# Grandediw/Unmanned_Aerial_Vehicles

Hardware: AMD Instinct MI355X
Metric: GP predictions/sec (mean+var) at N_train=65536, D=9 (higher is better)
Workload: dtype f32; 1 GPU; C3: N_train=65536, D=9, P=3, batched predict mean+var over 10000 query points per GPU per step (horizon 20 x 500 rollouts), fp32 predict on an fp64 factor; n_train=65536, features=9, outputs=3, parallelism=query-sharded x1, model replicated (every rank fits redundantly)

## Files before the change

include/gpk.h:

```cpp
#ifndef GPK_H
#define GPK_H

#include <stddef.h>
#include <stdint.h>

#ifdef __cplusplus
extern "C" {
#endif

typedef struct gpk_context* gpk_handle;

#define GPK_API __attribute__((visibility("default")))

enum { GPK_F32 = 0, GPK_F64 = 1 };
enum { GPK_OK = 0, GPK_NOT_PD = 1, GPK_BAD_ARG = 2, GPK_HIP_ERROR = 3 };
enum { GPK_TILE = 128, GPK_MAX_D = 64, GPK_MAX_D_PREDICT = 16, GPK_MAX_P = 16, GPK_MAX_BATCH = 8 };

GPK_API int gpk_create(gpk_handle* h, int device);
GPK_API void gpk_destroy(gpk_handle h);
GPK_API const char* gpk_last_error(gpk_handle h);
#define GPK_OWN_STREAM ((void*)(intptr_t)-1)
GPK_API int gpk_set_stream(gpk_handle h, void* stream);
GPK_API int gpk_synchronize(gpk_handle h);
GPK_API int64_t gpk_padded(int64_t n);

GPK_API int gpk_set_option(gpk_handle h, const char* name, int value);
GPK_API int gpk_set_option_str(gpk_handle h, const char* name, const char* value);
enum { GPK_TIMED_K5 = 1, GPK_TIMED_GRAM = 2, GPK_TIMED_GRAD = 3, GPK_TIMED_POTRF = 4, GPK_TIMED_COV = 5, GPK_TIMED_JAC = 6,
       GPK_TIMED_SPARSE_STATS = 7, GPK_TIMED_SPARSE_PASS = 8 };
GPK_API int gpk_timing(gpk_handle h, int enable);
GPK_API int gpk_kernel_times(gpk_handle h, int tag, double* ms, int max_n, int* n_out);

GPK_API int gpk_batch_begin(gpk_handle h, int count);
GPK_API int gpk_batch_buffer(gpk_handle h, const void* base, int64_t stride_bytes);
GPK_API int gpk_batch_end(gpk_handle h);
GPK_API const char* gpk_version(void);

GPK_API int gpk_gram(gpk_handle h, int dtype, const void* X, int64_t N, int D, const double* ls,
             double sf2, double diag_add, void* K, int64_t ldk);

GPK_API int gpk_gram_rows(gpk_handle h, int dtype, const void* X, int64_t N, int D, const double* ls, double sf2,
                  double diag_add, int64_t row0, int64_t nrows, void* Kslab, int64_t ldk);

GPK_API int gpk_cross_gram_t(gpk_handle h, int dtype, const void* X, int64_t N, const void* Xq,
                     int64_t M, int D, const double* ls, double sf2, void* B, int64_t ldb);

GPK_API int gpk_potrf(gpk_handle h, double* A, int64_t Np, int64_t lda, double* winv, int* info);

GPK_API int gpk_leaf_inverses(gpk_handle h, const double* L, int64_t Np, int64_t ldl, double* winv);

GPK_API int gpk_factor_to_f32(gpk_handle h, const double* L, int64_t Np, int64_t ldl, const double* winv,
                      float* Lf, int64_t ldlf, float* winvf);

GPK_API int gpk_potrs(gpk_handle h, const double* L, int64_t Np, int64_t ldl, const double* winv,
              const double* Y, int64_t N, int P, double* alpha);

GPK_API int gpk_potrs_inv(gpk_handle h, const double* W, int64_t Np, int64_t ldw, const double* Y, int64_t N,
                  int P, double* alpha);

GPK_API int gpk_trsm_lower_left(gpk_handle h, int dtype, const void* L, int64_t Np, int64_t ldl,
                        const void* winv, void* B, int64_t Mp, int64_t ldb);
GPK_API int gpk_colsumsq(gpk_handle h, int dtype, const void* B, int64_t Np, int64_t Mp, int64_t ldb,
                 double* out);

GPK_API int gpk_predict_mean(gpk_handle h, int dtype, const void* X, const void* alpha, int64_t N, int D,
                     int P, const double* ls, double sf2, const double* y_mean,
                     const double* y_std, const void* Xq, int64_t M, void* mean);

#define GPK_HOST_MAX_M 4096
GPK_API int gpk_predict_host(gpk_handle h, const double* X, const double* alpha, int64_t N, int D, int P,
                     const double* ls, double sf2, const double* y_mean, const double* y_std,
                     const double* W, int64_t Np, int64_t ldw, double kss, double floor_,
                     const double* Xq_host, int64_t M, double* mean_host, double* var_host);

GPK_API int gpk_predict_host_multi(gpk_handle h, int B, const double* const* X, const double* const* alpha, int64_t N, int D,
                           const double* ls, const double* sf2, const double* y_mean, const double* y_std,
                           const double* const* W, int64_t Np, int64_t ldw, const double* kss, double floor_,
                           const double* Xq_host, int64_t M, double* mean_host, double* var_host);

GPK_API int gpk_predict_mean_mfma(gpk_handle h, const float* X, const float* alpha, int64_t N, int D, int P,
                          const double* ls, double sf2, const double* center, const double* y_mean,
                          const double* y_std, const float* Xq, int64_t M, float* mean);

GPK_API int gpk_split3(gpk_handle h, const float* src, int64_t rows, int64_t cols, int64_t ld, void* dst);
GPK_API int gpk_predict_var_inv_split(gpk_handle h, const float* X, int64_t N, int D, const double* ls, double sf2,
                              const void* W3, int64_t Np, const float* Xq, int64_t M, double kss, double floor_,
                              float* work, void* work3, double* var);

GPK_API int gpk_split2_rows(gpk_handle h, const float* W, int64_t n, int64_t ld, float* scales, void* dst);
GPK_API int gpk_split2_rows_f64(gpk_handle h, const double* W, int64_t n, int64_t ld, float* scales, void* dst);
GPK_API int gpk_split2_rows_f64_absmax(gpk_handle h, const double* W, int64_t n, int64_t ld, float* scales, void* dst);
GPK_API int gpk_predict_var_inv_split2(gpk_handle h, const float* X, int64_t N, int D, const double* ls, double sf2,
                                       const void* W2, const float* w_scales, int64_t Np, const float* Xq, int64_t M,
                                       double kss, double floor_, void* work2, double* var);

GPK_API int gpk_predict_mean_var_split2(gpk_handle h, const float* X, const float* alpha, int64_t N, int D, int P,
                                        const double* ls, double sf2, const double* center, const double* y_mean,
                                        const double* y_std, const void* W2, const float* w_scales, int64_t Np,
                                        const float* Xq, int64_t M, double kss, double floor_, void* work2,
                                        float* mean_tmp, double recheck_below, unsigned* low_count, double* out);
GPK_API int gpk_pack_mean_var(gpk_handle h, int dtype, const void* mean, const double* var, int64_t M, int P,
                              const double* y_std, double* out);

GPK_API int gpk_predict_mean_multi(gpk_handle h, int dtype, const void* X, const void* alpha, int64_t N, int D,
                           int B, const double* ls, const double* sf2, const double* y_mean,
                           const double* y_std, const void* Xq, int64_t M, void* mean);

GPK_API int gpk_predict_var(gpk_handle h, int dtype, const void* X, int64_t N, int D, const double* ls,
                    double sf2, const void* L, int64_t Np, int64_t ldl, const void* winv,
                    const void* Xq, int64_t M, double kss, double floor, void* work,
                    double* var);

GPK_API int gpk_trtri(gpk_handle h, const double* L, int64_t Np, int64_t ldl, const double* winv, double* W,
              int64_t ldw, double* work);
GPK_API int gpk_trtri_absmax(gpk_handle h, const double* L, int64_t Np, int64_t ldl, const double* winv, double* W,
              int64_t ldw, double* work, float* block_absmax);
GPK_API int gpk_tril_to_f32(gpk_handle h, const double* A, int64_t Np, int64_t lda, float* Af, int64_t ldaf);
GPK_API int gpk_predict_var_inv(gpk_handle h, int dtype, const void* X, int64_t N, int D, const double* ls,
                        double sf2, const void* W, int64_t Np, int64_t ldw, const void* Xq, int64_t M,
                        double kss, double floor, void* work, double* var);

GPK_API int gpk_predict_cov_inv(gpk_handle h, int dtype, const void* X, int64_t N, int D, const double* ls, double sf2,
                                const void* W, int64_t Np, int64_t ldw, const void* Xq, int64_t M, double noise, void* work,
                                double* cov, int64_t ldc);
GPK_API int gpk_predict_cov(gpk_handle h, int dtype, const void* X, int64_t N, int D, const double* ls, double sf2,
                            const void* L, int64_t Np, int64_t ldl, const void* winv, const void* Xq, int64_t M, double noise,
                            void* work, double* cov, int64_t ldc);
GPK_API int gpk_predict_host_cov(gpk_handle h, const double* X, const double* alpha, int64_t N, int D, int P,
                                 const double* ls, double sf2, const double* y_mean, const double* y_std, const double* W,
                                 int64_t Np, int64_t ldw, double noise, const double* Xq_host, int64_t M, double* mean_host,
                                 double* cov_host);
GPK_API int gpk_predict_host_multi_cov(gpk_handle h, int B, const double* const* X, const double* const* alpha, int64_t N,
                                       int D, const double* ls, const double* sf2, const double* y_mean, const double* y_std,
                                       const double* const* W, int64_t Np, int64_t ldw, const double* noise,
                                       const double* Xq_host, int64_t M, double* mean_host, double* cov_host);
GPK_API int gpk_predict_batched_cov(gpk_handle h, const double* Xq, int64_t M, double* mean, double* cov);

GPK_API int gpk_predict_mean_grad(gpk_handle h, const double* X, const double* alpha, int64_t N, int D, int P, const double* ls,
                                  double sf2, const double* y_std, const double* Xq, int64_t M, double* dmean);
GPK_API int gpk_predict_var_grad_inv(gpk_handle h, const double* X, int64_t N, int D, const double* ls, double sf2,
                                     const double* W, int64_t Np, int64_t ldw, const double* Xq, int64_t M, double kss,
                                     double floor, double* work, double* var, double* dvar);
GPK_API int gpk_predict_host_grad(gpk_handle h, const double* X, const double* alpha, int64_t N, int D, int P, const double* ls,
                                  double sf2, const double* y_mean, const double* y_std, const double* W, int64_t Np,
                                  int64_t ldw, double kss, double floor, const double* Xq_host, int64_t M, double* mean_host,
                                  double* var_host, double* dmean_host, double* dvar_host);
GPK_API int gpk_predict_model_grad(gpk_handle h, const double* Xq, int64_t M, double* mean, double* var, double* dmean,
                                   double* dvar, int var_includes_noise);
GPK_API int gpk_predict_host_multi_grad(gpk_handle h, int B, const double* const* X, const double* const* alpha, int64_t N,
                                        int D, const double* ls, const double* sf2, const double* y_mean, const double* y_std,
                                        const double* const* W, int64_t Np, int64_t ldw, const double* kss, double floor,
                                        const double* Xq_host, int64_t M, double* mean_host, double* var_host,
                                        double* dmean_host, double* dvar_host);
GPK_API int gpk_predict_mean_grad_multi(gpk_handle h, const double* X, const double* alpha, int64_t N, int D, int B,
                                        const double* ls, const double* sf2, const double* y_std, const double* Xq, int64_t M,
                                        double* dmean);
GPK_API int gpk_predict_batched_grad(gpk_handle h, const double* Xq, int64_t M, double* mean, double* var, double* dmean,
                                     double* dvar, int var_includes_noise);

GPK_API int gpk_lml_terms(gpk_handle h, const double* L, int64_t N, int64_t ldl, const double* Y,
                  const double* alpha, int P, double* terms);

GPK_API int gpk_potri(gpk_handle h, const double* L, int64_t Np, int64_t ldl, const double* winv,
              double* Kinv, int64_t ldk, double* work);
GPK_API int gpk_wtw(gpk_handle h, const double* W, int64_t Np, int64_t ldw, double* Kinv, int64_t ldk);
GPK_API int gpk_lml_grad(gpk_handle h, const double* X, int64_t N, int D, const double* ls, double sf2,
                 double noise, const double* alpha, int P, const double* Kinv, int64_t ldk,
                 double* grad);

GPK_API int gpk_rbf_kernel_grad(gpk_handle h, const double* X1, int64_t n1, const double* X2, int64_t n2, int D,
                        const double* ls, double sf2, double* K, double* Q, int64_t ld);

GPK_API int gpk_lml_eval(gpk_handle h, const double* X, int64_t N, int D, const double* ls, double sf2, double diag_add,
                 double noise, const double* Yn, int P, double* K, int64_t Np, double* winv, double* W, double* work,
                 double* alpha, double* Kinv, double* terms, double* grad, int* info);

GPK_API int gpk_fit(gpk_handle h, const double* X, int64_t N, int D, const double* Y, int P, const double* ls, int n_ls,
            double sf2, double noise, double jitter, int normalize_y);
GPK_API int gpk_predict(gpk_handle h, const void* Xq, int64_t M, void* mean, void* var, int dtype, int var_includes_noise);
GPK_API int gpk_lml(gpk_handle h, const double* theta, int n_theta, double* lml, double* grad);
GPK_API int gpk_export(gpk_handle h, int64_t* N, int* D, int* P, double* L, double* alpha, double* y_mean, double* y_std,
               double* lml);
GPK_API int gpk_import(gpk_handle h, const double* X, int64_t N, int D, const double* L, const double* alpha, int P,
               const double* ls, int n_ls, double sf2, double noise, const double* y_mean, const double* y_std);
GPK_API int gpk_model_release(gpk_handle h);
GPK_API int gpk_predict_model_cov(gpk_handle h, const double* Xq, int64_t M, double* mean, double* cov);

GPK_API int gpk_fit_batched(gpk_handle h, int B, const double* X, int64_t N, int D, const double* Y, const double* ls, int n_ls,
                    const double* sf2, const double* noise, double jitter, int normalize_y, int* info);
GPK_API int gpk_predict_batched(gpk_handle h, const double* Xq, int64_t M, double* mean, double* var, int var_includes_noise);
GPK_API int gpk_lml_batched(gpk_handle h, const double* thetas, int n_theta, double* lml, double* grad);

GPK_API size_t gpk_greedy_select_bytes(int64_t n, int64_t m_max);
GPK_API int gpk_greedy_select(gpk_handle h, const double* X, int64_t n, int D, const double* ls, int n_ls, double sf2,
                              int64_t m_max, double min_var, double tol, void* work, int64_t* idx, double* trace, double* dmax,
                              int64_t* selected);
GPK_API int gpk_sparse_select(gpk_handle h, const double* X, int64_t n, int64_t m_max, double min_var, double tol, int64_t* idx,
                              double* trace, double* dmax, int64_t* selected);
GPK_API int gpk_sparse_accumulate(gpk_handle h, const double* X, const double* Yn, int64_t n, const double* Z, int64_t m, int D,
                                  int P, const double* ls, double sf2, double* S, int64_t ld);
GPK_API int gpk_sparse_grad_pass(gpk_handle h, const double* X, const double* Yn, int64_t n, const double* Z, int64_t m, int D,
                                 int P, const double* ls, double sf2, const double* Cm, int64_t ldc, double* sums);
GPK_API int gpk_sparse_zgrad_pass(gpk_handle h, const double* X, const double* Yn, int64_t n, const double* Z, int64_t m, int D,
                                  int P, const double* ls, double sf2, const double* Cm, int64_t ldc, double* R);
GPK_API int gpk_sparse_begin(gpk_handle h, const double* Z, int64_t m, int D, int P, const double* ls, int n_ls, double sf2,
                             double noise, double jitter, double jitter_uu, const double* y_mean, const double* y_std);
GPK_API int gpk_sparse_hold(gpk_handle h, const double* X, const double* Y, int64_t n);
GPK_API int gpk_sparse_eval(gpk_handle h, const double* ls, int n_ls, double sf2, double noise, double* bound, double* grad,
                            int* info);
GPK_API int gpk_sparse_eval_z(gpk_handle h, const double* Z, const double* ls, int n_ls, double sf2, double noise, double* bound,
                              double* grad, double* gradZ, int* info);
GPK_API int gpk_sparse_update(gpk_handle h, const double* X, const double* Y, int64_t n);
GPK_API int gpk_sparse_finalize(gpk_handle h, int* info);
GPK_API int gpk_sparse_predict(gpk_handle h, const double* Xq, int64_t M, double* mean, double* var, int var_includes_noise);
GPK_API int gpk_sparse_predict_grad(gpk_handle h, const double* Xq, int64_t M, double* mean, double* var, double* dmean,
                                    double* dvar, int var_includes_noise);
GPK_API int gpk_sparse_predict_cov(gpk_handle h, const double* Xq, int64_t M, double* mean, double* cov);

GPK_API int gpk_sparse_predict_multi(gpk_handle h, int B, const gpk_handle* models, const double* Xq, int64_t M, double* mean,
                                     double* var, int var_includes_noise);
GPK_API int gpk_sparse_predict_multi_grad(gpk_handle h, int B, const gpk_handle* models, const double* Xq, int64_t M, double* mean,
                                          double* var, double* dmean, double* dvar, int var_includes_noise);
GPK_API int gpk_sparse_predict_multi_cov(gpk_handle h, int B, const gpk_handle* models, const double* Xq, int64_t M, double* mean,
                                         double* cov);
GPK_API int gpk_sparse_bound(gpk_handle h, double* bound, int64_t* n_rows);
GPK_API int gpk_sparse_export(gpk_handle h, int64_t* m, int* D, int* P, int* n_ls, double* Z, double* G, double* g, double* yy,
                              int64_t* n_rows, double* ls, double* hyper, double* y_mean, double* y_std);
GPK_API int gpk_sparse_import(gpk_handle h, const double* Z, int64_t m, int D, int P, const double* ls, int n_ls, double sf2,
                              double noise, double jitter, double jitter_uu, const double* y_mean, const double* y_std,
                              const double* G, const double* g, const double* yy, int64_t n_rows);

GPK_API int gpk_gemm_tiles(gpk_handle h, int dtype, int ta, int tb, const void* A, int64_t lda, const void* B,
                   int64_t ldb, void* C, int64_t ldc, int64_t m, int64_t n, int64_t k, double alpha,
                   double beta, int lower_only);

#ifdef __cplusplus
}
#endif
#endif
```

unmanned_aerial_vehicles_amd/_lib.py:

```python
import ctypes as C
import os

import numpy as np

from ._build import LIB_PATH

GPK_F32, GPK_F64 = 0, 1
GPK_OK, GPK_NOT_PD, GPK_BAD_ARG, GPK_HIP_ERROR = 0, 1, 2, 3
GPK_TILE, GPK_MAX_D, GPK_MAX_P = 128, 64, 16
GPK_HOST_MAX_M = 4096
GPK_TIMED_K5, GPK_TIMED_GRAM, GPK_TIMED_GRAD, GPK_TIMED_POTRF = 1, 2, 3, 4
GPK_TIMED_COV = 5
GPK_TIMED_JAC = 6
GPK_TIMED_SPARSE_STATS, GPK_TIMED_SPARSE_PASS = 7, 8

_vp, _i64, _int, _dbl = C.c_void_p, C.c_int64, C.c_int, C.c_double
_dp = C.POINTER(C.c_double)

SIGNATURES = {
    "gpk_create": (_int, [C.POINTER(_vp), _int]),
    "gpk_destroy": (None, [_vp]),
    "gpk_last_error": (C.c_char_p, [_vp]),
    "gpk_set_stream": (_int, [_vp, _vp]),
    "gpk_synchronize": (_int, [_vp]),
    "gpk_padded": (_i64, [_i64]),
    "gpk_fit": (_int, [_vp, _dp, _i64, _int, _dp, _int, _dp, _int, _dbl, _dbl, _dbl, _int]),
    "gpk_predict": (_int, [_vp, _vp, _i64, _vp, _vp, _int, _int]),
    "gpk_lml": (_int, [_vp, _dp, _int, _dp, _dp]),
    "gpk_fit_batched": (_int, [_vp, _int, _dp, _i64, _int, _dp, _dp, _int, _dp, _dp, _dbl, _int, C.POINTER(C.c_int)]),
    "gpk_predict_batched": (_int, [_vp, _dp, _i64, _dp, _dp, _int]),
    "gpk_lml_batched": (_int, [_vp, _dp, _int, _dp, _dp]),
    "gpk_export": (_int, [_vp, C.POINTER(_i64), C.POINTER(_int), C.POINTER(_int), _dp, _dp, _dp, _dp, _dp]),
    "gpk_import": (_int, [_vp, _dp, _i64, _int, _dp, _dp, _int, _dp, _int, _dbl, _dbl, _dp, _dp]),
    "gpk_model_release": (_int, [_vp]),
    "gpk_split2_rows": (_int, [_vp, _vp, _i64, _i64, _vp, _vp]),
    "gpk_split2_rows_f64": (_int, [_vp, _vp, _i64, _i64, _vp, _vp]),
    "gpk_split2_rows_f64_absmax": (_int, [_vp, _vp, _i64, _i64, _vp, _vp]),
    "gpk_predict_var_inv_split2": (_int, [_vp, _vp, _i64, _int, _dp, _dbl, _vp, _vp, _i64, _vp, _i64, _dbl, _dbl, _vp, _vp]),
    "gpk_predict_mean_var_split2": (_int, [_vp, _vp, _vp, _i64, _int, _int, _dp, _dbl, _dp, _dp, _dp, _vp, _vp, _i64, _vp, _i64,
                                           _dbl, _dbl, _vp, _vp, _dbl, _vp, _vp]),
    "gpk_pack_mean_var": (_int, [_vp, _int, _vp, _vp, _i64, _int, _dp, _vp]),
    "gpk_set_option": (_int, [_vp, C.c_char_p, _int]),
    "gpk_set_option_str": (_int, [_vp, C.c_char_p, C.c_char_p]),
    "gpk_timing": (_int, [_vp, _int]),
    "gpk_kernel_times": (_int, [_vp, _int, _dp, _int, C.POINTER(_int)]),
    "gpk_batch_begin": (_int, [_vp, _int]),
    "gpk_batch_buffer": (_int, [_vp, _vp, _i64]),
    "gpk_batch_end": (_int, [_vp]),
    "gpk_version": (C.c_char_p, []),
    "gpk_gram": (_int, [_vp, _int, _vp, _i64, _int, _dp, _dbl, _dbl, _vp, _i64]),
    "gpk_gram_rows": (_int, [_vp, _int, _vp, _i64, _int, _dp, _dbl, _dbl, _i64, _i64, _vp, _i64]),
    "gpk_cross_gram_t": (_int, [_vp, _int, _vp, _i64, _vp, _i64, _int, _dp, _dbl, _vp, _i64]),
    "gpk_rbf_kernel_grad": (_int, [_vp, _vp, _i64, _vp, _i64, _int, _dp, _dbl, _vp, _vp, _i64]),
    "gpk_potrf": (_int, [_vp, _vp, _i64, _i64, _vp, C.POINTER(_int)]),
    "gpk_leaf_inverses": (_int, [_vp, _vp, _i64, _i64, _vp]),
    "gpk_factor_to_f32": (_int, [_vp, _vp, _i64, _i64, _vp, _vp, _i64, _vp]),
    "gpk_potrs": (_int, [_vp, _vp, _i64, _i64, _vp, _vp, _i64, _int, _vp]),
    "gpk_potrs_inv": (_int, [_vp, _vp, _i64, _i64, _vp, _i64, _int, _vp]),
    "gpk_wtw": (_int, [_vp, _vp, _i64, _i64, _vp, _i64]),
    "gpk_trsm_lower_left": (_int, [_vp, _int, _vp, _i64, _i64, _vp, _vp, _i64, _i64]),
    "gpk_colsumsq": (_int, [_vp, _int, _vp, _i64, _i64, _i64, _vp]),
    "gpk_predict_mean": (_int, [_vp, _int, _vp, _vp, _i64, _int, _int, _dp, _dbl, _dp, _dp, _vp, _i64, _vp]),
    "gpk_split3": (_int, [_vp, _vp, _i64, _i64, _i64, _vp]),
    "gpk_predict_var_inv_split": (_int, [_vp, _vp, _i64, _int, _dp, _dbl, _vp, _i64, _vp, _i64, _dbl, _dbl, _vp, _vp, _vp]),
    "gpk_predict_host": (_int, [_vp, _vp, _vp, _i64, _int, _int, _vp, _dbl, _vp, _vp, _vp, _i64, _i64, _dbl, _dbl, _vp,
                                _i64, _vp, _vp]),
    "gpk_predict_host_multi": (_int, [_vp, _int, _vp, _vp, _i64, _int, _vp, _vp, _vp, _vp, _vp, _i64, _i64, _vp, _dbl, _vp,
                                      _i64, _vp, _vp]),
    "gpk_predict_mean_mfma": (_int, [_vp, _vp, _vp, _i64, _int, _int, _dp, _dbl, _dp, _dp, _dp, _vp, _i64, _vp]),
    "gpk_predict_mean_multi": (_int, [_vp, _int, _vp, _vp, _i64, _int, _int, _dp, _dp, _dp, _dp, _vp, _i64, _vp]),
    "gpk_predict_var": (_int, [_vp, _int, _vp, _i64, _int, _dp, _dbl, _vp, _i64, _i64, _vp, _vp, _i64, _dbl,
                               _dbl, _vp, _vp]),
    "gpk_trtri": (_int, [_vp, _vp, _i64, _i64, _vp, _vp, _i64, _vp]),
    "gpk_trtri_absmax": (_int, [_vp, _vp, _i64, _i64, _vp, _vp, _i64, _vp, _vp]),
    "gpk_tril_to_f32": (_int, [_vp, _vp, _i64, _i64, _vp, _i64]),
    "gpk_predict_var_inv": (_int, [_vp, _int, _vp, _i64, _int, _dp, _dbl, _vp, _i64, _i64, _vp, _i64, _dbl, _dbl,
                                   _vp, _vp]),
    "gpk_predict_cov_inv": (_int, [_vp, _int, _vp, _i64, _int, _dp, _dbl, _vp, _i64, _i64, _vp, _i64, _dbl, _vp, _vp,
                                   _i64]),
    "gpk_predict_cov": (_int, [_vp, _int, _vp, _i64, _int, _dp, _dbl, _vp, _i64, _i64, _vp, _vp, _i64, _dbl, _vp, _vp,
                               _i64]),
    "gpk_predict_host_cov": (_int, [_vp, _vp, _vp, _i64, _int, _int, _vp, _dbl, _vp, _vp, _vp, _i64, _i64, _dbl, _vp, _i64,
                                    _vp, _vp]),
    "gpk_predict_model_cov": (_int, [_vp, _dp, _i64, _dp, _dp]),
    "gpk_predict_host_multi_cov": (_int, [_vp, _int, _vp, _vp, _i64, _int, _vp, _vp, _vp, _vp, _vp, _i64, _i64, _vp, _vp, _i64,
                                          _vp, _vp]),
    "gpk_predict_batched_cov": (_int, [_vp, _dp, _i64, _dp, _dp]),
    "gpk_predict_mean_grad": (_int, [_vp, _vp, _vp, _i64, _int, _int, _dp, _dbl, _dp, _vp, _i64, _vp]),
    "gpk_predict_var_grad_inv": (_int, [_vp, _vp, _i64, _int, _dp, _dbl, _vp, _i64, _i64, _vp, _i64, _dbl, _dbl, _vp, _vp, _vp]),
    "gpk_predict_host_grad": (_int, [_vp, _vp, _vp, _i64, _int, _int, _vp, _dbl, _vp, _vp, _vp, _i64, _i64, _dbl, _dbl, _vp,
                                     _i64, _vp, _vp, _vp, _vp]),
    "gpk_predict_model_grad": (_int, [_vp, _dp, _i64, _dp, _dp, _dp, _dp, _int]),
    "gpk_predict_host_multi_grad": (_int, [_vp, _int, _vp, _vp, _i64, _int, _vp, _vp, _vp, _vp, _vp, _i64, _i64, _vp, _dbl, _vp,
                                           _i64, _vp, _vp, _vp, _vp]),
    "gpk_predict_mean_grad_multi": (_int, [_vp, _vp, _vp, _i64, _int, _int, _dp, _dp, _dp, _vp, _i64, _vp]),
    "gpk_predict_batched_grad": (_int, [_vp, _dp, _i64, _dp, _dp, _dp, _dp, _int]),
    "gpk_lml_terms": (_int, [_vp, _vp, _i64, _i64, _vp, _vp, _int, _dp]),
    "gpk_potri": (_int, [_vp, _vp, _i64, _i64, _vp, _vp, _i64, _vp]),
    "gpk_lml_grad": (_int, [_vp, _vp, _i64, _int, _dp, _dbl, _dbl, _vp, _int, _vp, _i64, _dp]),
    "gpk_lml_eval": (_int, [_vp, _vp, _i64, _int, _dp, _dbl, _dbl, _dbl, _vp, _int, _vp, _i64, _vp, _vp, _vp, _vp, _vp, _dp, _dp,
                            C.POINTER(C.c_int)]),
    "gpk_sparse_accumulate": (_int, [_vp, _vp, _vp, _i64, _vp, _i64, _int, _int, _dp, _dbl, _vp, _i64]),
    "gpk_sparse_grad_pass": (_int, [_vp, _vp, _vp, _i64, _vp, _i64, _int, _int, _dp, _dbl, _vp, _i64, _vp]),
    "gpk_sparse_zgrad_pass": (_int, [_vp, _vp, _vp, _i64, _vp, _i64, _int, _int, _dp, _dbl, _vp, _i64, _vp]),
    "gpk_sparse_hold": (_int, [_vp, _dp, _dp, _i64]),
    "gpk_sparse_eval": (_int, [_vp, _dp, _int, _dbl, _dbl, _dp, _dp, C.POINTER(_int)]),
    "gpk_sparse_eval_z": (_int, [_vp, _dp, _dp, _int, _dbl, _dbl, _dp, _dp, _dp, C.POINTER(_int)]),
    "gpk_greedy_select_bytes": (C.c_size_t, [_i64, _i64]),
    "gpk_greedy_select": (_int, [_vp, _vp, _i64, _int, _dp, _int, _dbl, _i64, _dbl, _dbl, _vp, _vp, _vp, _vp, _vp]),
    "gpk_sparse_select": (_int, [_vp, _dp, _i64, _i64, _dbl, _dbl, C.POINTER(_i64), _dp, _dp, C.POINTER(_i64)]),
    "gpk_sparse_begin": (_int, [_vp, _dp, _i64, _int, _int, _dp, _int, _dbl, _dbl, _dbl, _dbl, _dp, _dp]),
    "gpk_sparse_update": (_int, [_vp, _dp, _dp, _i64]),
    "gpk_sparse_finalize": (_int, [_vp, C.POINTER(_int)]),
    "gpk_sparse_predict": (_int, [_vp, _dp, _i64, _dp, _dp, _int]),
    "gpk_sparse_predict_grad": (_int, [_vp, _dp, _i64, _dp, _dp, _dp, _dp, _int]),
    "gpk_sparse_predict_cov": (_int, [_vp, _dp, _i64, _dp, _dp]),
    "gpk_sparse_predict_multi": (_int, [_vp, _int, C.POINTER(_vp), _dp, _i64, _dp, _dp, _int]),
    "gpk_sparse_predict_multi_grad": (_int, [_vp, _int, C.POINTER(_vp), _dp, _i64, _dp, _dp, _dp, _dp, _int]),
    "gpk_sparse_predict_multi_cov": (_int, [_vp, _int, C.POINTER(_vp), _dp, _i64, _dp, _dp]),
    "gpk_sparse_bound": (_int, [_vp, _dp, C.POINTER(_i64)]),
    "gpk_sparse_export": (_int, [_vp, C.POINTER(_i64), C.POINTER(_int), C.POINTER(_int), C.POINTER(_int), _dp, _dp, _dp, _dp,
                                 C.POINTER(_i64), _dp, _dp, _dp, _dp]),
    "gpk_sparse_import": (_int, [_vp, _dp, _i64, _int, _int, _dp, _int, _dbl, _dbl, _dbl, _dbl, _dp, _dp, _dp, _dp, _dp, _i64]),
    "gpk_gemm_tiles": (_int, [_vp, _int, _int, _int, _vp, _i64, _vp, _i64, _vp, _i64, _i64, _i64, _i64, _dbl,
                              _dbl, _int]),
}

_lib = None


class GPKError(RuntimeError):
    def __init__(self, code, message):
        super().__init__(f"libgpk error {code}: {message}")
        self.code = code


class NotPositiveDefinite(np.linalg.LinAlgError):
    """Raised where the reference's LAPACK call raises `numpy.linalg.LinAlgError`
    (scipy.linalg.cholesky at sklearn/gaussian_process/_gpr.py:349)."""


def load():
    global _lib
    if _lib is not None:
        return _lib
    try:
        import torch
    except ImportError:
        pass
    path = os.environ.get("GPK_LIBRARY") or LIB_PATH
    if not os.path.exists(path):
        raise RuntimeError(
            f"{path} not found: build it with `python -c 'import __graft_entry__ as g; g.build()'` "
            "(there is no CPU fallback for the GP kernels)")
    lib = C.CDLL(path)
    for name, (res, args) in SIGNATURES.items():
        fn = getattr(lib, name)
        fn.restype = res
        fn.argtypes = args
    _lib = lib
    return lib


def dptr(a):
    a = np.ascontiguousarray(a, dtype=np.float64)
    return a, a.ctypes.data_as(_dp)
```

unmanned_aerial_vehicles_amd/csrc/gpk_api.hip:

```cpp
#include <cstdlib>

#include "gpk_internal.h"

extern "C" const char* gpk_version(void) { return "gpk 0.1 (gfx950)"; }

extern "C" int64_t gpk_padded(int64_t n) { return (n + GPK_TILE - 1) / GPK_TILE * GPK_TILE; }

extern "C" int gpk_create(gpk_handle* out, int device) {
  if (!out) return GPK_BAD_ARG;
  *out = nullptr;
  int count = 0;
  if (hipGetDeviceCount(&count) != hipSuccess || count <= 0 || device < 0 || device >= count) return GPK_HIP_ERROR;
  if (hipSetDevice(device) != hipSuccess) return GPK_HIP_ERROR;
  gpk_context* h = new gpk_context();
  h->device = device;
  if (hipStreamCreateWithFlags(&h->own_stream, hipStreamNonBlocking) != hipSuccess ||
      hipMalloc((void**)&h->d_info, GPK_MAX_BATCH * sizeof(int)) != hipSuccess ||

      hipMalloc((void**)&h->d_count, 2 * GPK_SMALL_MAX_MODELS * sizeof(unsigned)) != hipSuccess ||
      hipMemset(h->d_count, 0, 2 * GPK_SMALL_MAX_MODELS * sizeof(unsigned)) != hipSuccess ||
      hipHostMalloc((void**)&h->h_small, 4096, hipHostMallocMapped | hipHostMallocCoherent) != hipSuccess ||
      hipHostGetDevicePointer((void**)&h->d_small, h->h_small, 0) != hipSuccess) {
    delete h;
    return GPK_HIP_ERROR;
  }
  h->stream = h->own_stream;
  *out = h;
  return GPK_OK;
}

extern "C" void gpk_destroy(gpk_handle h) {
  if (!h) return;
  (void)hipSetDevice(h->device);
  (void)hipStreamSynchronize(h->stream);
  gpk_model_free(h);
  if (h->scratch) (void)hipFree(h->scratch);
  if (h->d_info) (void)hipFree(h->d_info);
  if (h->d_count) (void)hipFree(h->d_count);
  if (h->d_cov_count) (void)hipFree(h->d_cov_count);
  if (h->d_ptile) (void)hipFree(h->d_ptile);
  if (h->h_small) (void)hipHostFree(h->h_small);
  if (h->serve_dev) (void)hipFree(h->serve_dev);
  if (h->serve_host) (void)hipHostFree(h->serve_host);
  for (auto& t : h->timed) {
    if (t.e0) (void)hipEventDestroy(t.e0);
    if (t.e1) (void)hipEventDestroy(t.e1);
  }
  if (h->own_stream) (void)hipStreamDestroy(h->own_stream);
  delete h;
}

extern "C" const char* gpk_last_error(gpk_handle h) { return h ? h->err.c_str() : "null handle"; }

extern "C" int gpk_set_stream(gpk_handle h, void* stream) {
  if (!h) return GPK_BAD_ARG;
  hipStream_t want = (stream == GPK_OWN_STREAM) ? h->own_stream : (hipStream_t)stream;
  GPK_CHECK_HIP(h, hipSetDevice(h->device));
  if (want == h->stream) return GPK_OK;
  GPK_CHECK_HIP(h, hipStreamSynchronize(h->stream));
  h->stream = want;
  h->user_stream = (stream != GPK_OWN_STREAM);
  return GPK_OK;
}

extern "C" int gpk_set_option(gpk_handle h, const char* name, int value) {
  if (!h) return GPK_BAD_ARG;
  GPK_REQUIRE(h, name, "set_option: null name");
  const std::string n(name);
  if (n == "k5_split2_tile") h->k5_split2_tile = (value >= 0 && value <= 2) ? value : 0;
  else if (n == "small_path") h->small_path = value;
  else if (n == "trsm256") h->trsm256 = value;
  else if (n == "trtri_levels") h->trtri_levels = value;
  else if (n == "gemm_small_tiles") h->gemm_small_tiles = value;
  else if (n == "gemm_tiny_tiles") h->gemm_tiny_tiles = value;
  else if (n == "gemm_balanced") h->gemm_balanced = value;
  else if (n == "gemm_balanced_max_tiles") h->gemm_balanced_max_tiles = value;
  else if (n == "k3_stream_min_np") h->k3_stream_min_np = value;
  else if (n == "gemm_log") h->gemm_log = value;
  else if (n == "gram_log") h->gram_log = value;
  else if (n == "debug_fill") h->debug_fill = value ? 1 : 0;
  else if (n == "sparse_panel") h->sparse_panel = value <= 0 ? 0 : value > (1 << 20) ? (1 << 20) : value;
  else if (n == "sparse_slabs") h->sparse_slabs = value <= 0 ? 0 : value > 64 ? 64 : value;
  else if (n == "ptile") h->ptile = value;
  else if (n == "ptile_max_np") h->ptile_max_np = value;
  else if (n == "ptile_prog_max_nt") h->ptile_prog_max_nt = value;
  else if (n == "ptile_inv_max_np") h->ptile_inv_max_np = value;
  else if (n == "ptile_single_max_nt") h->ptile_single_max_nt = value;
  else if (n == "ptile_sr") h->ptile_sr = value;
  else if (n == "ptile_sr_max_nt") h->ptile_sr_max_nt = value;
  else if (n == "ptile_prog_rows") h->ptile_prog_rows = value >= 8 ? 8 : value >= 1 ? value : 1;
  else { h->err = "bad argument: unknown option " + n; return GPK_BAD_ARG; }
  return GPK_OK;
}

extern "C" int gpk_set_option_str(gpk_handle h, const char* name, const char* value) {
  if (!h) return GPK_BAD_ARG;
  GPK_REQUIRE(h, name, "set_option_str: null name");
  const std::string n(name);
  if (n == "ptile_trace_path") h->ptile_trace_request = value ? value : "";
  else { h->err = "bad argument: unknown option " + n; return GPK_BAD_ARG; }
  return GPK_OK;
}

extern "C" int gpk_timing(gpk_handle h, int enable) {
  if (!h) return GPK_BAD_ARG;
  if (enable && h->timed.empty()) {
    GPK_CHECK_HIP(h, hipSetDevice(h->device));
    h->timed.resize(GPK_TIMING_RING);
    for (auto& t : h->timed) {
      GPK_CHECK_HIP(h, hipEventCreate(&t.e0));
      GPK_CHECK_HIP(h, hipEventCreate(&t.e1));
    }
  }
  h->timing = enable ? 1 : 0;
  h->timed_count = 0;
  return GPK_OK;
}

extern "C" int gpk_kernel_times(gpk_handle h, int tag, double* ms, int max_n, int* n_out) {
  if (!h) return GPK_BAD_ARG;
  GPK_REQUIRE(h, ms && n_out && max_n >= 1, "kernel_times: null pointer");
  *n_out = 0;
  if (h->timed.empty()) return GPK_OK;
  GPK_CHECK_HIP(h, hipStreamSynchronize(h->stream));
  const long long have = h->timed_count < GPK_TIMING_RING ? h->timed_count : GPK_TIMING_RING;
  for (long long i = h->timed_count - have; i < h->timed_count && *n_out < max_n; ++i) {
    const auto& t = h->timed[(size_t)(i % GPK_TIMING_RING)];
    if (t.tag != tag) continue;
    float f = 0.f;
    GPK_CHECK_HIP(h, hipEventElapsedTime(&f, t.e0, t.e1));
    ms[(*n_out)++] = (double)f;
  }
  return GPK_OK;
}

extern "C" int gpk_batch_begin(gpk_handle h, int count) {
  if (!h) return GPK_BAD_ARG;
  GPK_REQUIRE(h, count >= 1 && count <= GPK_MAX_BATCH, "batch_begin: count must be in [1, 8]");
  GPK_REQUIRE(h, h->batch == 1 && h->bbufs.empty(), "batch_begin: a batch is already open");
  h->batch = count;
  return GPK_OK;
}

extern "C" int gpk_batch_buffer(gpk_handle h, const void* base, int64_t stride_bytes) {
  if (!h) return GPK_BAD_ARG;
  GPK_REQUIRE(h, base && stride_bytes > 0 && stride_bytes % 16 == 0, "batch_buffer: stride must be a positive multiple of 16");
  h->bbufs.push_back({(const char*)base, (long long)stride_bytes});
  return GPK_OK;
}

extern "C" int gpk_batch_end(gpk_handle h) {
  if (!h) return GPK_BAD_ARG;
  h->batch = 1;
  h->bbufs.clear();
  return GPK_OK;
}

extern "C" int gpk_synchronize(gpk_handle h) {
  if (!h) return GPK_BAD_ARG;
  GPK_CHECK_HIP(h, hipStreamSynchronize(h->stream));
  return GPK_OK;
}

int gpk_scratch(gpk_handle h, size_t bytes, void** out) {
  if (bytes > h->scratch_bytes) {
    GPK_CHECK_HIP(h, hipSetDevice(h->device));
    GPK_CHECK_HIP(h, hipStreamSynchronize(h->stream));
    if (h->scratch) GPK_CHECK_HIP(h, hipFree(h->scratch));
    h->scratch = nullptr;
    h->scratch_bytes = 0;
    const size_t want = (bytes + (1u << 20) - 1) & ~(size_t)((1u << 20) - 1);
    GPK_CHECK_HIP(h, hipMalloc(&h->scratch, want));
    h->scratch_bytes = want;
  }
  if (h->debug_fill && bytes > 0) GPK_CHECK_HIP(h, hipMemsetAsync(h->scratch, 0xFF, bytes, h->stream));
  *out = h->scratch;
  return GPK_OK;
}

extern "C" int gpk_predict_var(gpk_handle h, int dtype, const void* X, int64_t N, int D, const double* ls,
                               double sf2, const void* L, int64_t Np, int64_t ldl, const void* winv, const void* Xq,
                               int64_t M, double kss, double floor_, void* work, double* var) {
  if (!h) return GPK_BAD_ARG;
  GPK_REQUIRE(h, X && L && winv && Xq && work && var, "predict_var: null pointer");
  GPK_REQUIRE(h, N >= 1 && M >= 1 && Np == gpk_padded(N), "predict_var: Np must equal gpk_padded(N)");
  const int64_t Mp = gpk_padded(M);
  GPK_TRY(gpk_cross_gram_t(h, dtype, X, N, Xq, M, D, ls, sf2, work, Mp));
  GPK_TRY(gpk_trsm_lower_left(h, dtype, L, Np, ldl, winv, work, Mp, Mp));
  GPK_TRY(gpk_colsumsq(h, dtype, work, Np, Mp, Mp, var));
  return gpk_var_finalize(h, var, M, kss, floor_, var);
}

extern "C" int gpk_predict_var_inv(gpk_handle h, int dtype, const void* X, int64_t N, int D, const double* ls,
                                   double sf2, const void* W, int64_t Np, int64_t ldw, const void* Xq, int64_t M,
                                   double kss, double floor_, void* work, double* var) {
  if (!h) return GPK_BAD_ARG;
  GPK_REQUIRE(h, X && W && Xq && work && var, "predict_var_inv: null pointer");
  GPK_REQUIRE(h, N >= 1 && M >= 1 && Np == gpk_padded(N) && ldw >= Np, "predict_var_inv: Np must equal gpk_padded(N)");
  GPK_REQUIRE(h, dtype == GPK_F32 || dtype == GPK_F64, "predict_var_inv: bad dtype");
  const int64_t Mp = gpk_padded(M);
  GPK_TRY(gpk_cross_gram_t(h, dtype, Xq, M, X, N, D, ls, sf2, work, Np));
  GemmArgs g = gemm_args(W, ldw, 0, work, Np, 0, nullptr, Mp, (int)Np, (int)Mp, (int)Np, 1.0, 0.0);
  g.ke0 = GPK_TILE;
  g.ke_row = GPK_TILE;
  g.epilogue = 1;
  g.k_super = 1;
  g.heavy_first = 1;
  const int ntm = (int)(Np / gpk_gemm_tile(h, g));
  void* partial = nullptr;
  GPK_TRY(gpk_scratch(h, (size_t)ntm * Mp * sizeof(double), &partial));
  g.C = partial;
  gpk_time_begin(h, GPK_TIMED_K5);
  const int rc_gemm = gpk_gemm(h, dtype, g);
  gpk_time_end(h);
  GPK_TRY(rc_gemm);
  return gpk_colsum_finalize(h, (const double*)partial, ntm, Mp, M, kss, floor_, var);
}

extern "C" int gpk_gemm_tiles(gpk_handle h, int dtype, int ta, int tb, const void* A, int64_t lda, const void* B,
                              int64_t ldb, void* C, int64_t ldc, int64_t m, int64_t n, int64_t k, double alpha,
                              double beta, int lower_only) {
  if (!h) return GPK_BAD_ARG;
  GPK_REQUIRE(h, A && B && C, "gemm_tiles: null pointer");
  GPK_REQUIRE(h, dtype == GPK_F32 || dtype == GPK_F64, "gemm_tiles: bad dtype");
  GPK_REQUIRE(h, m < (1ll << 31) && n < (1ll << 31) && k < (1ll << 31), "gemm_tiles: size too large");
  GemmArgs g = gemm_args(A, lda, ta ? 1 : 0, B, ldb, tb ? 1 : 0, C, ldc, (int)m, (int)n, (int)k, alpha, beta);
  g.lower_only = lower_only ? 1 : 0;
  return gpk_gemm(h, dtype, g);
}
```

unmanned_aerial_vehicles_amd/csrc/gpk_gram.hip:

```cpp
#include <cstdlib>

#include "gpk_internal.h"
#include "gpk_math.h"

namespace {

struct LsArr { double v[GPK_MAX_D]; };
struct PArr { double v[GPK_MAX_P]; };
struct Ls16 { double v[16]; };

__device__ __forceinline__ double exp_neg(double x) { return gpk_exp_neg(x); }
__device__ __forceinline__ float exp_neg(float x) {
  const float L2E_HI = 1.44269502162933349609375f, L2E_LO = 1.925963033500011e-08f;
  const float hi = x * L2E_HI;
  const float lo = __builtin_fmaf(x, L2E_HI, -hi) + x * L2E_LO;
  const float e = __builtin_amdgcn_exp2f(hi);
  return __builtin_fmaf(e, lo * 0.693147180559945f, e);
}

__device__ __forceinline__ double fma_t(double a, double b, double c) { return __builtin_fma(a, b, c); }
__device__ __forceinline__ float fma_t(float a, float b, float c) { return __builtin_fmaf(a, b, c); }

template <typename T> struct Vec16;
template <> struct Vec16<double> { typedef double2 type; static constexpr int N = 2; };
template <> struct Vec16<float> { typedef float4 type; static constexpr int N = 4; };

__device__ __forceinline__ void st16(double* p, double a, double b, bool nt) {
  typedef double dv2 __attribute__((ext_vector_type(2)));
  dv2 v = {a, b};
  if (nt) __builtin_nontemporal_store(v, reinterpret_cast<dv2*>(p));
  else *reinterpret_cast<dv2*>(p) = v;
}
__device__ __forceinline__ void st16(float* p, float a, float b, float c, float d, bool nt) {
  typedef float fv4 __attribute__((ext_vector_type(4)));
  fv4 v = {a, b, c, d};
  if (nt) __builtin_nontemporal_store(v, reinterpret_cast<fv4*>(p));
  else *reinterpret_cast<fv4*>(p) = v;
}
__device__ __forceinline__ void store_row4(double* p, int tx, const double (&v)[4], bool nt) {
  st16(p + 2 * tx, v[0], v[1], nt);
  st16(p + 32 + 2 * tx, v[2], v[3], nt);
}
__device__ __forceinline__ void store_row4(float* p, int tx, const float (&v)[4], bool nt) {
  st16(p + 4 * tx, v[0], v[1], v[2], v[3], nt);
}

constexpr int TS = 64;

template <typename T> __device__ __forceinline__ int colof(int tx, int c);
template <> __device__ __forceinline__ int colof<double>(int tx, int c) { return (c >> 1) * 32 + 2 * tx + (c & 1); }
template <> __device__ __forceinline__ int colof<float>(int tx, int c) { return 4 * tx + c; }
constexpr int DCH = 16;

template <typename T>
__device__ __forceinline__ void stage_x(const T* __restrict__ X, long long n, int D, long long r0, int d0,
                                        int dc, const LsArr& ls, T* lds, int tid) {
  for (int e = tid; e < TS * dc; e += 256) {
    const int i = e / dc, d = e - i * dc;
    const long long gi = r0 + i;
    T v = T(0);
    if (gi < n) v = X[gi * D + d0 + d] / T(ls.v[d0 + d]);
    lds[d * TS + i] = v;
  }
}

template <typename T>
__device__ __forceinline__ void accum_d2(const T* xi, const T* xj, int dc, int ty, int tx, T (&d2)[4][4]) {
  for (int d = 0; d < dc; ++d) {
    T a[4], b[4];
#pragma unroll
    for (int r = 0; r < 4; ++r) a[r] = xi[d * TS + 4 * ty + r];
#pragma unroll
    for (int c = 0; c < 4; ++c) b[c] = xj[d * TS + colof<T>(tx, c)];
#pragma unroll
    for (int r = 0; r < 4; ++r)
#pragma unroll
      for (int c = 0; c < 4; ++c) {
        const T df = a[r] - b[c];
        d2[r][c] = fma_t(df, df, d2[r][c]);
      }
  }
}

template <typename T, bool NT>
__global__ __launch_bounds__(256) void gram_sym_kernel(const T* __restrict__ X, long long N, int D, LsArr ls,
                                                       T sf2, T diag_add, T* __restrict__ K, long long ldk) {
  __shared__ __attribute__((aligned(16))) T xi[DCH * TS];
  __shared__ __attribute__((aligned(16))) T xj[DCH * TS];
  __shared__ __attribute__((aligned(16))) T tb[TS * (TS + 1)];
  const int tid = threadIdx.x, tx = tid & 15, ty = tid >> 4;

  const long long id = blockIdx.x;
  long long ti = (long long)((__builtin_sqrt(8.0 * (double)id + 1.0) - 1.0) * 0.5);
  while ((ti + 1) * (ti + 2) / 2 <= id) ++ti;
  while (ti * (ti + 1) / 2 > id) --ti;
  const long long tj = id - ti * (ti + 1) / 2;
  const long long i0 = ti * TS, j0 = tj * TS;

  T d2[4][4];
#pragma unroll
  for (int r = 0; r < 4; ++r)
#pragma unroll
    for (int c = 0; c < 4; ++c) d2[r][c] = T(0);

  for (int dbase = 0; dbase < D; dbase += DCH) {
    const int dc = min(DCH, D - dbase);
    if (dbase) __syncthreads();
    stage_x<T>(X, N, D, i0, dbase, dc, ls, xi, tid);
    stage_x<T>(X, N, D, j0, dbase, dc, ls, xj, tid);
    __syncthreads();
    accum_d2<T>(xi, xj, dc, ty, tx, d2);
  }

  T v[4][4];
#pragma unroll
  for (int r = 0; r < 4; ++r) {
    const long long gi = i0 + 4 * ty + r;
#pragma unroll
    for (int c = 0; c < 4; ++c) {
      const long long gj = j0 + colof<T>(tx, c);
      T val = sf2 * exp_neg(T(-0.5) * d2[r][c]);
      if (gi == gj) val = sf2 + diag_add;
      if (gi >= N || gj >= N) val = (gi == gj) ? T(1) : T(0);
      v[r][c] = val;
    }
    store_row4(K + gi * ldk + j0, tx, v[r], NT);
  }
  if (ti == tj) return;

#pragma unroll
  for (int r = 0; r < 4; ++r)
#pragma unroll
    for (int c = 0; c < 4; ++c) tb[(4 * ty + r) * (TS + 1) + colof<T>(tx, c)] = v[r][c];
  __syncthreads();
  constexpr int VEC = Vec16<T>::N;
  constexpr int LPR = TS / VEC;
  constexpr int RPG = TS / (256 / LPR);
  const int lp = tid % LPR, g = tid / LPR;
#pragma unroll
  for (int rr = 0; rr < RPG; ++rr) {
    const int jj = g * RPG + rr;
    T w[VEC];
#pragma unroll
    for (int e = 0; e < VEC; ++e) w[e] = tb[(VEC * lp + e) * (TS + 1) + jj];
    T* dst = K + (j0 + jj) * ldk + i0 + VEC * lp;
    if constexpr (VEC == 2) st16(dst, w[0], w[1], NT);
    else st16(dst, w[0], w[1], w[2], w[3], NT);
  }
}

template <typename T, bool NT, int GS>
__global__ __launch_bounds__(256) void gram_strip_kernel(const T* __restrict__ X, long long N, int D, LsArr ls,
                                                         T sf2, T diag_add, T* __restrict__ K, long long ldk) {
  __shared__ __attribute__((aligned(16))) T xi[DCH * TS];
  __shared__ __attribute__((aligned(16))) T xj[DCH * TS];
  __shared__ __attribute__((aligned(16))) T tb[TS * (TS + 1)];
  const int tid = threadIdx.x, tx = tid & 15, ty = tid >> 4;
  const long long id = blockIdx.x;
  long long q = (long long)((__builtin_sqrt(1.0 + 8.0 * (double)id / GS) - 1.0) * 0.5);
  while (GS * (q + 1) * (q + 2) / 2 <= id) ++q;
  while (GS * q * (q + 1) / 2 > id) --q;
  const long long rem_id = id - GS * q * (q + 1) / 2;
  const long long ti = GS * q + rem_id / (q + 1);
  const long long g = rem_id % (q + 1);
  const long long i0 = ti * TS;
  const long long tj0 = g * GS, tj1 = min(ti, tj0 + GS - 1);

  stage_x<T>(X, N, D, i0, 0, D, ls, xi, tid);
  stage_x<T>(X, N, D, tj0 * TS, 0, D, ls, xj, tid);
  constexpr int NPF = (TS * DCH + 255) / 256;
  T pf[NPF];
  __syncthreads();
  for (long long tj = tj0; tj <= tj1; ++tj) {
    const long long j0 = tj * TS;
    const bool more = tj < tj1;
    if (more) {
#pragma unroll
      for (int p = 0; p < NPF; ++p) {
        const int e = tid + 256 * p;
        const int i = e / D, d = e - i * D;
        const long long gi = j0 + TS + i;
        pf[p] = (e < TS * D && gi < N) ? X[gi * D + d] / T(ls.v[d]) : T(0);
      }
    }
    T d2[4][4];
#pragma unroll
    for (int r = 0; r < 4; ++r)
#pragma unroll
      for (int c = 0; c < 4; ++c) d2[r][c] = T(0);
    accum_d2<T>(xi, xj, D, ty, tx, d2);
    T v[4][4];
#pragma unroll
    for (int r = 0; r < 4; ++r) {
      const long long gi = i0 + 4 * ty + r;
#pragma unroll
      for (int c = 0; c < 4; ++c) {
        const long long gj = j0 + colof<T>(tx, c);
        T val = sf2 * exp_neg(T(-0.5) * d2[r][c]);
        if (gi == gj) val = sf2 + diag_add;
        if (gi >= N || gj >= N) val = (gi == gj) ? T(1) : T(0);
        v[r][c] = val;
      }
      store_row4(K + gi * ldk + j0, tx, v[r], NT);
    }
    if (ti != tj) {
#pragma unroll
      for (int r = 0; r < 4; ++r)
#pragma unroll
        for (int c = 0; c < 4; ++c) tb[(4 * ty + r) * (TS + 1) + colof<T>(tx, c)] = v[r][c];
    }
    __syncthreads();
    if (ti != tj) {
      constexpr int VEC = Vec16<T>::N;
      constexpr int LPR = TS / VEC;
      constexpr int RPG = TS / (256 / LPR);
      const int lp = tid % LPR, gg = tid / LPR;
#pragma unroll
      for (int rr = 0; rr < RPG; ++rr) {
        const int jj = gg * RPG + rr;
        T w[VEC];
#pragma unroll
        for (int e = 0; e < VEC; ++e) w[e] = tb[(VEC * lp + e) * (TS + 1) + jj];
        T* dst = K + (j0 + jj) * ldk + i0 + VEC * lp;
        if constexpr (VEC == 2) st16(dst, w[0], w[1], NT);
        else st16(dst, w[0], w[1], w[2], w[3], NT);
      }
    }
    if (more) {
#pragma unroll
      for (int p = 0; p < NPF; ++p) {
        const int e = tid + 256 * p;
        if (e < TS * D) { const int i = e / D, d = e - i * D; xj[d * TS + i] = pf[p]; }
      }
    }
    __syncthreads();
  }
}

template <typename T>
__global__ __launch_bounds__(256) void cross_t_kernel(const T* __restrict__ X, long long N,
                                                      const T* __restrict__ Xq, long long M, int D, LsArr ls,
                                                      T sf2, T* __restrict__ B, long long ldb) {
  __shared__ __attribute__((aligned(16))) T xi[DCH * TS];
  __shared__ __attribute__((aligned(16))) T xj[DCH * TS];
  const int tid = threadIdx.x, tx = tid & 15, ty = tid >> 4;
  const long long i0 = (long long)blockIdx.y * TS, j0 = (long long)blockIdx.x * TS;
  T d2[4][4];
#pragma unroll
  for (int r = 0; r < 4; ++r)
#pragma unroll
    for (int c = 0; c < 4; ++c) d2[r][c] = T(0);
  for (int dbase = 0; dbase < D; dbase += DCH) {
    const int dc = min(DCH, D - dbase);
    if (dbase) __syncthreads();
    stage_x<T>(X, N, D, i0, dbase, dc, ls, xi, tid);
    stage_x<T>(Xq, M, D, j0, dbase, dc, ls, xj, tid);
    __syncthreads();
    accum_d2<T>(xi, xj, dc, ty, tx, d2);
  }
#pragma unroll
  for (int r = 0; r < 4; ++r) {
    const long long gi = i0 + 4 * ty + r;
    T v[4];
#pragma unroll
    for (int c = 0; c < 4; ++c) {
      const long long gj = j0 + colof<T>(tx, c);
      T val = sf2 * exp_neg(T(-0.5) * d2[r][c]);
      if (gi >= N || gj >= M) val = T(0);
      v[c] = val;
    }
    store_row4(B + gi * ldb + j0, tx, v, false);
  }
}

typedef _Float16 h8_t __attribute__((ext_vector_type(8)));
typedef unsigned int u4_t __attribute__((ext_vector_type(4)));
constexpr int CS2_QS = 4;
template <int DD>
__global__ __launch_bounds__(256) void cross_split2_kernel(const float* __restrict__ Xq, long long M,
                                                           const float* __restrict__ X, long long N, int D, LsArr ls,
                                                           float sf2, float scale, u4_t* __restrict__ dst, long long Np) {
  __shared__ __attribute__((aligned(16))) float xs[DD][128];
  const int tid = threadIdx.x, lane = tid & 63, wave = tid >> 6;
  const long long j0 = (long long)blockIdx.x * 128;
  for (int e = tid; e < 128 * DD; e += 256) {
    const int d = e >> 7, i = e & 127;
    const long long gj = j0 + i;
    xs[d][i] = (d < D && gj < N) ? X[gj * D + d] / (float)ls.v[d] : 0.f;
  }
  __syncthreads();
  const int r = lane & 31, hh = lane >> 5;
  const long long KB = Np >> 4, Mp = (M + 127) / 128 * 128;
#pragma unroll 1
  for (int qs = 0; qs < CS2_QS; ++qs) {
  const long long q0 = ((long long)blockIdx.y * CS2_QS + qs) * 64;
  if (q0 >= Mp) break;
  const long long qblk = (q0 >> 5) + (wave >> 1), q = qblk * 32 + r;
  float xq[DD];
#pragma unroll
  for (int d = 0; d < DD; ++d) xq[d] = (q < M ? Xq[q * DD + d] : 0.f) / (float)ls.v[d];
#pragma unroll
  for (int t = 0; t < 4; ++t) {
    const int kb = 4 * (wave & 1) + t, kbase = 16 * kb + 8 * hh;
    float d2[8];
#pragma unroll
    for (int i = 0; i < 8; ++i) d2[i] = 0.f;
#pragma unroll
    for (int d = 0; d < DD; ++d) {
      const float4 lo = *reinterpret_cast<const float4*>(&xs[d][kbase]), hi = *reinterpret_cast<const float4*>(&xs[d][kbase + 4]);
      const float b[8] = {lo.x, lo.y, lo.z, lo.w, hi.x, hi.y, hi.z, hi.w};
#pragma unroll
      for (int i = 0; i < 8; ++i) { const float df = xq[d] - b[i]; d2[i] = __builtin_fmaf(df, df, d2[i]); }
    }
    h8_t p0, p1;
#pragma unroll
    for (int i = 0; i < 8; ++i) {
      float val = sf2 * exp_neg(-0.5f * d2[i]);
      if (q >= M || j0 + kbase + i >= N) val = 0.f;
      const float x = val * scale;
      const _Float16 h0 = (_Float16)x;
      p0[i] = h0;
      p1[i] = (_Float16)(x - (float)h0);
    }
    u4_t* o = dst + ((qblk * KB + (j0 >> 4) + kb) * 2) * 64 + lane;
    o[0] = __builtin_bit_cast(u4_t, p0);
    o[64] = __builtin_bit_cast(u4_t, p1);
  }
  }
}

constexpr int PM_DMAX = 16, PM_PMAX = 16, PM_TJ = 128, PM_QPT = 2, PM_RS = PM_DMAX + PM_PMAX;

template <typename T> struct Quad;
template <> struct Quad<float> { typedef float4 type; };
template <> struct Quad<double> { typedef double4 type; };

template <typename T, int D4, int P4>
__global__ __launch_bounds__(256) void predict_mean_kernel(const T* __restrict__ X, const T* __restrict__ alpha,
                                                           long long N, int D, int P, Ls16 ls,
                                                           const T* __restrict__ Xq, long long M,
                                                           long long chunk, T* __restrict__ partial) {
  __shared__ __attribute__((aligned(16))) T rows[PM_TJ * PM_RS];
  typedef typename Quad<T>::type Q4;
  const int tid = threadIdx.x;
  constexpr int DD = 4 * D4, PP = 4 * P4;
  T xq[PM_QPT][DD];
  T acc[PM_QPT][PP];
  long long qm[PM_QPT];
#pragma unroll
  for (int q = 0; q < PM_QPT; ++q) {
    qm[q] = ((long long)blockIdx.x * PM_QPT + q) * 256 + tid;
#pragma unroll
    for (int d = 0; d < DD; ++d) {
      xq[q][d] = T(0);
      if (d < D && qm[q] < M) xq[q][d] = Xq[qm[q] * D + d] / T(ls.v[d]);
    }
#pragma unroll
    for (int p = 0; p < PP; ++p) acc[q][p] = T(0);
  }
  constexpr bool TWO_LEVEL = sizeof(T) == 4;
  T tot[PM_QPT][PP];
#pragma unroll
  for (int q = 0; q < PM_QPT; ++q)
#pragma unroll
    for (int p = 0; p < PP; ++p) tot[q][p] = T(0);
  const long long n0 = (long long)blockIdx.y * chunk;
  const long long n1 = min(N, n0 + chunk);
  for (long long jb = n0; jb < n1; jb += PM_TJ) {
    const int nj = (int)min((long long)PM_TJ, n1 - jb);
    if constexpr (TWO_LEVEL) {
#pragma unroll
      for (int q = 0; q < PM_QPT; ++q)
#pragma unroll
        for (int p = 0; p < PP; ++p) { tot[q][p] += acc[q][p]; acc[q][p] = T(0); }
    }
    __syncthreads();
    for (int e = tid; e < nj * (DD + PP); e += 256) {
      const int j = e / (DD + PP), c = e - j * (DD + PP);
      T v = T(0);
      if (c < DD) { if (c < D) v = X[(jb + j) * D + c] / T(ls.v[c]); }
      else if (c - DD < P) v = alpha[(jb + j) * P + (c - DD)];
      rows[j * PM_RS + (c < DD ? c : PM_DMAX + (c - DD))] = v;
    }
    __syncthreads();
#pragma unroll 2
    for (int j = 0; j < nj; ++j) {
      const Q4* row = reinterpret_cast<const Q4*>(rows + j * PM_RS);
      T xt[DD], al[PP];
#pragma unroll
      for (int g = 0; g < D4; ++g) {
        const Q4 v = row[g];
        xt[4 * g] = v.x; xt[4 * g + 1] = v.y; xt[4 * g + 2] = v.z; xt[4 * g + 3] = v.w;
      }
#pragma unroll
      for (int g = 0; g < P4; ++g) {
        const Q4 v = row[PM_DMAX / 4 + g];
        al[4 * g] = v.x; al[4 * g + 1] = v.y; al[4 * g + 2] = v.z; al[4 * g + 3] = v.w;
      }
#pragma unroll
      for (int q = 0; q < PM_QPT; ++q) {
        T d2 = T(0);
#pragma unroll
        for (int d = 0; d < DD; ++d) {
          const T df = xq[q][d] - xt[d];
          d2 = fma_t(df, df, d2);
        }
        const T e = exp_neg(T(-0.5) * d2);
#pragma unroll
        for (int p = 0; p < PP; ++p) acc[q][p] = fma_t(e, al[p], acc[q][p]);
      }
    }
  }
#pragma unroll
  for (int q = 0; q < PM_QPT; ++q) {
    if (qm[q] < M) {
#pragma unroll
      for (int p = 0; p < PP; ++p)
        if (p < P) partial[((long long)blockIdx.y * M + qm[q]) * P + p] = TWO_LEVEL ? tot[q][p] + acc[q][p] : acc[q][p];
    }
  }
}

template <typename T>
using pm_fn = void (*)(const T*, const T*, long long, int, int, Ls16, const T*, long long, long long, T*);
template <typename T, int D4>
pm_fn<T> pm_pick_p(int p4) {
  switch (p4) {
    case 1: return predict_mean_kernel<T, D4, 1>;
    case 2: return predict_mean_kernel<T, D4, 2>;
    case 3: return predict_mean_kernel<T, D4, 3>;
    default: return predict_mean_kernel<T, D4, 4>;
  }
}
template <typename T>
pm_fn<T> pm_pick(int d4, int p4) {
  switch (d4) {
    case 1: return pm_pick_p<T, 1>(p4);
    case 2: return pm_pick_p<T, 2>(p4);
    case 3: return pm_pick_p<T, 3>(p4);
    default: return pm_pick_p<T, 4>(p4);
  }
}

template <typename T, int D4, int B4>
__global__ __launch_bounds__(256) void predict_mean_multi_kernel(const T* __restrict__ X,
                                                                 const T* __restrict__ alpha, long long N, int D,
                                                                 int B, const double* __restrict__ w_dev,
                                                                 const T* __restrict__ Xq, long long M,
                                                                 long long chunk, T* __restrict__ partial) {
  __shared__ __attribute__((aligned(16))) T rows[PM_TJ * PM_RS];
  __shared__ __attribute__((aligned(16))) T wl[4 * B4 * 4 * D4];
  typedef typename Quad<T>::type Q4;
  const int tid = threadIdx.x;
  constexpr int DD = 4 * D4, BB = 4 * B4;
  for (int e = tid; e < BB * DD; e += 256) {
    const int b = e / DD, d = e - b * DD;
    wl[e] = (b < B && d < D) ? T(w_dev[b * D + d]) : T(0);
  }
  T xq[PM_QPT][DD];
  T acc[PM_QPT][BB];
  long long qm[PM_QPT];
#pragma unroll
  for (int q = 0; q < PM_QPT; ++q) {
    qm[q] = ((long long)blockIdx.x * PM_QPT + q) * 256 + tid;
#pragma unroll
    for (int d = 0; d < DD; ++d) {
      xq[q][d] = T(0);
      if (d < D && qm[q] < M) xq[q][d] = Xq[qm[q] * D + d];
    }
#pragma unroll
    for (int b = 0; b < BB; ++b) acc[q][b] = T(0);
  }
  const long long n0 = (long long)blockIdx.y * chunk;
  const long long n1 = min(N, n0 + chunk);
  for (long long jb = n0; jb < n1; jb += PM_TJ) {
    const int nj = (int)min((long long)PM_TJ, n1 - jb);
    __syncthreads();
    for (int e = tid; e < PM_TJ * (DD + BB); e += 256) {
      const int j = e / (DD + BB), c = e - j * (DD + BB);
      T v = T(0);
      if (j < nj) {
        if (c < DD) { if (c < D) v = X[(jb + j) * D + c]; }
        else if (c - DD < B) v = alpha[(jb + j) * B + (c - DD)];
      }
      rows[j * PM_RS + (c < DD ? c : PM_DMAX + (c - DD))] = v;
    }
    __syncthreads();
#pragma unroll 2
    for (int j = 0; j < PM_TJ; ++j) {
      const Q4* row = reinterpret_cast<const Q4*>(rows + j * PM_RS);
      T xt[DD], al[BB];
#pragma unroll
      for (int g = 0; g < D4; ++g) {
        const Q4 v = row[g];
        xt[4 * g] = v.x; xt[4 * g + 1] = v.y; xt[4 * g + 2] = v.z; xt[4 * g + 3] = v.w;
      }
#pragma unroll
      for (int g = 0; g < B4; ++g) {
        const Q4 v = row[PM_DMAX / 4 + g];
        al[4 * g] = v.x; al[4 * g + 1] = v.y; al[4 * g + 2] = v.z; al[4 * g + 3] = v.w;
      }
#pragma unroll
      for (int q = 0; q < PM_QPT; ++q) {
        T sq[DD];
#pragma unroll
        for (int d = 0; d < DD; ++d) { const T df = xq[q][d] - xt[d]; sq[d] = df * df; }
#pragma unroll
        for (int b = 0; b < BB; ++b) {
          T d2 = T(0);
#pragma unroll
          for (int d = 0; d < DD; ++d) d2 = fma_t(sq[d], wl[b * DD + d], d2);
          acc[q][b] = fma_t(exp_neg(T(-0.5) * d2), al[b], acc[q][b]);
        }
      }
    }
  }
#pragma unroll
  for (int q = 0; q < PM_QPT; ++q) {
    if (qm[q] < M) {
#pragma unroll
      for (int b = 0; b < BB; ++b)
        if (b < B) partial[((long long)blockIdx.y * M + qm[q]) * B + b] = acc[q][b];
    }
  }
}

template <typename T>
__global__ void mean_reduce_multi_kernel(const T* __restrict__ partial, int S, long long M, int B, PArr sf2,
                                         PArr ymean, PArr ystd, T* __restrict__ mean) {
  const long long e = (long long)blockIdx.x * blockDim.x + threadIdx.x;
  if (e >= M * B) return;
  const int b = (int)(e % B);
  T s = T(0);
  for (int k = 0; k < S; ++k) s += partial[(long long)k * M * B + e];
  mean[e] = T(ymean.v[b]) + T(ystd.v[b]) * (T(sf2.v[b]) * s);
}

template <typename T>
using pmm_fn = void (*)(const T*, const T*, long long, int, int, const double*, const T*, long long, long long, T*);
template <typename T, int D4>
pmm_fn<T> pmm_pick_b(int b4) {
  return b4 <= 1 ? predict_mean_multi_kernel<T, D4, 1> : predict_mean_multi_kernel<T, D4, 2>;
}
template <typename T>
pmm_fn<T> pmm_pick(int d4, int b4) {
  switch (d4) {
    case 1: return pmm_pick_b<T, 1>(b4);
    case 2: return pmm_pick_b<T, 2>(b4);
    case 3: return pmm_pick_b<T, 3>(b4);
    default: return pmm_pick_b<T, 4>(b4);
  }
}

template <typename T>
__global__ void mean_reduce_kernel(const T* __restrict__ partial, int S, long long M, int P, T sf2, PArr ymean,
                                   PArr ystd, T* __restrict__ mean) {
  const long long e = (long long)blockIdx.x * blockDim.x + threadIdx.x;
  if (e >= M * P) return;
  const int p = (int)(e % P);
  double s = 0.0;
  for (int k = 0; k < S; ++k) s += (double)partial[(long long)k * M * P + e];
  mean[e] = T(ymean.v[p]) + T(ystd.v[p]) * (sf2 * T(s));
}

template <typename T>
__global__ __launch_bounds__(256) void colsumsq_kernel(const T* __restrict__ B, long long rows_per, long long Np,
                                                       long long ldb, double* __restrict__ partial, long long Mp) {
  const int c = threadIdx.x & 127, hh = threadIdx.x >> 7;
  const long long m = (long long)blockIdx.x * 128 + c;
  const long long r0 = (long long)blockIdx.y * rows_per, r1 = min(Np, r0 + rows_per);
  double s0 = 0.0, s1 = 0.0;
  long long r = r0 + hh;
  for (; r + 2 < r1; r += 4) {
    const double a = (double)B[r * ldb + m], b = (double)B[(r + 2) * ldb + m];
    s0 = __builtin_fma(a, a, s0);
    s1 = __builtin_fma(b, b, s1);
  }
  if (r < r1) { const double a = (double)B[r * ldb + m]; s0 = __builtin_fma(a, a, s0); }
  partial[((long long)blockIdx.y * 2 + hh) * Mp + m] = s0 + s1;
}
__global__ void colsum_reduce_kernel(const double* __restrict__ partial, int S, long long Mp,
                                     double* __restrict__ out) {
  const long long m = (long long)blockIdx.x * blockDim.x + threadIdx.x;
  if (m >= Mp) return;
  double s = 0.0;
  for (int k = 0; k < S; ++k) s += partial[(long long)k * Mp + m];
  out[m] = s;
}
__global__ void colsum_finalize_kernel(const double* __restrict__ partial, int S, long long Mp, long long M, double kss,
                                       double floor_, double* __restrict__ var) {
  const long long m = (long long)blockIdx.x * blockDim.x + threadIdx.x;
  if (m >= M) return;
  double s = 0.0;
  for (int k = 0; k < S; ++k) s += partial[(long long)k * Mp + m];
  var[m] = fmax(kss - s, floor_);
}
__global__ void colsum_finalize_packed_kernel(const double* __restrict__ partial, int S, long long Mp, long long M, double kss,
                                              double floor_, const float* __restrict__ mean, int P, PArr ystd,
                                              double recheck_below, unsigned* __restrict__ low_count,
                                              double* __restrict__ out) {
  const long long m = (long long)blockIdx.x * blockDim.x + threadIdx.x;
  if (m >= M) return;
  double s = 0.0;
  for (int k = 0; k < S; ++k) s += partial[(long long)k * Mp + m];
  const double v = fmax(kss - s, floor_);
  if (low_count && v < recheck_below) atomicAdd(low_count, 1u);
  double* o = out + m * 2 * P;
  for (int p = 0; p < P; ++p) { o[p] = (double)mean[m * P + p]; o[P + p] = v * ystd.v[p] * ystd.v[p]; }
}
template <typename T>
__global__ void pack_mean_var_kernel(const T* __restrict__ mean, const double* __restrict__ var, long long M, int P, PArr ystd,
                                     double* __restrict__ out) {
  const long long m = (long long)blockIdx.x * blockDim.x + threadIdx.x;
  if (m >= M) return;
  double* o = out + m * 2 * P;
  const double v = var[m];
  for (int p = 0; p < P; ++p) { o[p] = (double)mean[m * P + p]; o[P + p] = v * ystd.v[p] * ystd.v[p]; }
}
__global__ void var_finalize_kernel(const double* ss, long long M, double kss, double floor_, double* var) {
  const long long m = (long long)blockIdx.x * blockDim.x + threadIdx.x;
  if (m >= M) return;
  var[m] = fmax(kss - ss[m], floor_);
}

int fill_ls(gpk_handle h, const double* ls, int D, LsArr& out) {
  GPK_REQUIRE(h, D >= 1 && D <= GPK_MAX_D, "D must be in [1, 64]");
  GPK_REQUIRE(h, ls != nullptr, "length-scale array is null");
  for (int d = 0; d < GPK_MAX_D; ++d) out.v[d] = 1.0;
  for (int d = 0; d < D; ++d) {
    GPK_REQUIRE(h, ls[d] > 0.0, "length-scales must be positive");
    out.v[d] = ls[d];
  }
  return GPK_OK;
}

}

extern "C" int gpk_gram(gpk_handle h, int dtype, const void* X, int64_t N, int D, const double* ls, double sf2,
                        double diag_add, void* K, int64_t ldk) {
  if (!h) return GPK_BAD_ARG;
  GPK_REQUIRE(h, N >= 1 && X && K, "gram: null pointer or N < 1");
  const int64_t Np = gpk_padded(N);
  GPK_REQUIRE(h, dtype == GPK_F32 || dtype == GPK_F64, "gram: bad dtype");
  GPK_REQUIRE(h, ldk >= Np && ldk % (dtype == GPK_F32 ? 4 : 2) == 0,
              "gram: ldk must be >= gpk_padded(N) and a multiple of 2 (fp64) / 4 (fp32)");
  LsArr l;
  GPK_TRY(fill_ls(h, ls, D, l));
  const int64_t nt = Np / TS;
  const int64_t tiles = nt * (nt + 1) / 2;
  GPK_REQUIRE(h, tiles < (1ll << 31), "gram: N too large");
  const bool stream_nt = Np >= 16384;
  GPK_REQUIRE(h, ((uintptr_t)K % 16) == 0, "gram: K must be 16-byte aligned");
  const dim3 block(256);
  const bool strip = D <= DCH;
  auto count = [&](int gs) { long long c = 0; for (long long r = 0; r < nt; ++r) c += r / gs + 1; return c; };
  const int gs = count(8) >= 1024 ? 8 : count(2) >= 512 ? 2 : 1;
  const long long nstrips = count(gs);
  const dim3 grid((unsigned)(strip ? nstrips : tiles));
#define GPK_GRAM_LAUNCH(T, NT)                                                                              \
  do {                                                                                                      \
    if (strip && gs == 8)                                                                                   \
      hipLaunchKernelGGL((gram_strip_kernel<T, NT, 8>), grid, block, 0, h->stream, (const T*)X, (long long)N, D, l, \
                         (T)sf2, (T)diag_add, (T*)K, (long long)ldk);                                       \
    else if (strip && gs == 2)                                                                              \
      hipLaunchKernelGGL((gram_strip_kernel<T, NT, 2>), grid, block, 0, h->stream, (const T*)X, (long long)N, D, l, \
                         (T)sf2, (T)diag_add, (T*)K, (long long)ldk);                                       \
    else if (strip)                                                                                         \
      hipLaunchKernelGGL((gram_strip_kernel<T, NT, 1>), grid, block, 0, h->stream, (const T*)X, (long long)N, D, l, \
                         (T)sf2, (T)diag_add, (T*)K, (long long)ldk);                                       \
    else                                                                                                    \
      hipLaunchKernelGGL((gram_sym_kernel<T, NT>), grid, block, 0, h->stream, (const T*)X, (long long)N, D, l,  \
                         (T)sf2, (T)diag_add, (T*)K, (long long)ldk);                                       \
  } while (0)
  if (h->gram_log)
    fprintf(stderr, "GPKGRAM %s %lld %lld %d %s gs%d nt%lld grid%u\n", dtype == GPK_F64 ? "f64" : "f32", (long long)N, (long long)Np, D,
            strip ? "strip" : "sym", strip ? gs : 0, (long long)nt, grid.x);
  gpk_time_begin(h, GPK_TIMED_GRAM);
  if (dtype == GPK_F64) { if (stream_nt) GPK_GRAM_LAUNCH(double, true); else GPK_GRAM_LAUNCH(double, false); }
  else { if (stream_nt) GPK_GRAM_LAUNCH(float, true); else GPK_GRAM_LAUNCH(float, false); }
  gpk_time_end(h);
#undef GPK_GRAM_LAUNCH
  GPK_LAUNCH_CHECK(h);
  return GPK_OK;
}

int gpk_cross_split2(gpk_handle h, const float* Xq, int64_t M, const float* X, int64_t N, int D, const double* ls,
                     double sf2, double scale, void* dst) {
  GPK_REQUIRE(h, Xq && X && dst && M >= 1 && N >= 1 && D >= 1 && D <= DCH, "cross_split2: bad argument");
  const int64_t Np = gpk_padded(N), Mp = gpk_padded(M);
  LsArr l;
  GPK_TRY(fill_ls(h, ls, D, l));
  GPK_REQUIRE(h, Mp / 64 < 65536, "cross_split2: at most 2^22 queries per call");
  const dim3 grid((unsigned)(Np / 128), (unsigned)((Mp / 64 + CS2_QS - 1) / CS2_QS));
#define GPK_CS2(DD) case DD: hipLaunchKernelGGL(cross_split2_kernel<DD>, grid, dim3(256), 0, h->stream, Xq, (long long)M, X, (long long)N, D, \
                                                l, (float)sf2, (float)scale, (u4_t*)dst, (long long)Np); break
  switch (D) {
    GPK_CS2(1); GPK_CS2(2); GPK_CS2(3); GPK_CS2(4); GPK_CS2(5); GPK_CS2(6); GPK_CS2(7); GPK_CS2(8);
    GPK_CS2(9); GPK_CS2(10); GPK_CS2(11); GPK_CS2(12); GPK_CS2(13); GPK_CS2(14); GPK_CS2(15); GPK_CS2(16);
  }
#undef GPK_CS2
  GPK_LAUNCH_CHECK(h);
  return GPK_OK;
}

extern "C" int gpk_cross_gram_t(gpk_handle h, int dtype, const void* X, int64_t N, const void* Xq, int64_t M,
                                int D, const double* ls, double sf2, void* B, int64_t ldb) {
  if (!h) return GPK_BAD_ARG;
  GPK_REQUIRE(h, N >= 1 && M >= 1 && X && Xq && B, "cross_gram: null pointer or empty input");
  const int64_t Np = gpk_padded(N), Mp = gpk_padded(M);
  GPK_REQUIRE(h, ldb >= Mp && ldb % 4 == 0, "cross_gram: ldb must be >= gpk_padded(M)");
  GPK_REQUIRE(h, dtype == GPK_F32 || dtype == GPK_F64, "cross_gram: bad dtype");
  LsArr l;
  GPK_TRY(fill_ls(h, ls, D, l));
  dim3 grid((unsigned)(Mp / TS), (unsigned)(Np / TS));
  GPK_REQUIRE(h, Np / TS < 65536, "cross_gram: N too large");
  if (dtype == GPK_F64)
    hipLaunchKernelGGL(cross_t_kernel<double>, grid, dim3(256), 0, h->stream, (const double*)X, (long long)N,
                       (const double*)Xq, (long long)M, D, l, sf2, (double*)B, (long long)ldb);
  else
    hipLaunchKernelGGL(cross_t_kernel<float>, grid, dim3(256), 0, h->stream, (const float*)X, (long long)N,
                       (const float*)Xq, (long long)M, D, l, (float)sf2, (float*)B, (long long)ldb);
  GPK_LAUNCH_CHECK(h);
  return GPK_OK;
}

namespace {
template <typename T>
__global__ void slab_diag_kernel(T* __restrict__ K, long long ldk, long long row0, long long nrows_p, long long N,
                                 long long Np, T dval) {
  const long long r = (long long)blockIdx.x * 256 + threadIdx.x;
  if (r >= nrows_p) return;
  const long long i = row0 + r;
  if (i < Np) K[r * ldk + i] = i < N ? dval : T(1);
}
}

extern "C" int gpk_gram_rows(gpk_handle h, int dtype, const void* X, int64_t N, int D, const double* ls, double sf2,
                             double diag_add, int64_t row0, int64_t nrows, void* Kslab, int64_t ldk) {
  if (!h) return GPK_BAD_ARG;
  GPK_REQUIRE(h, X && Kslab && N >= 1, "gram_rows: null pointer or empty input");
  const int64_t Np = gpk_padded(N), nrp = gpk_padded(nrows);
  GPK_REQUIRE(h, row0 >= 0 && row0 % GPK_TILE == 0 && nrows >= 1 && row0 + nrp <= Np,
              "gram_rows: row0 must be a multiple of 128 and the slab must lie inside the padded matrix");
  GPK_REQUIRE(h, ldk >= Np && ldk % 4 == 0, "gram_rows: ldk must be >= gpk_padded(N)");
  GPK_REQUIRE(h, dtype == GPK_F32 || dtype == GPK_F64, "gram_rows: bad dtype");
  const size_t es = dtype == GPK_F64 ? 8 : 4;
  const int64_t valid = row0 >= N ? 0 : (N - row0 < nrp ? N - row0 : nrp);
  if (valid > 0) {
    GPK_TRY(gpk_cross_gram_t(h, dtype, (const char*)X + (size_t)row0 * D * es, valid, X, N, D, ls, sf2, Kslab, ldk));
    if (gpk_padded(valid) < nrp)
      GPK_CHECK_HIP(h, hipMemsetAsync((char*)Kslab + (size_t)gpk_padded(valid) * ldk * es, 0,
                                      (size_t)(nrp - gpk_padded(valid)) * ldk * es, h->stream));
  } else {
    GPK_CHECK_HIP(h, hipMemsetAsync(Kslab, 0, (size_t)nrp * ldk * es, h->stream));
  }
  const unsigned nb = (unsigned)((nrp + 255) / 256);
  if (dtype == GPK_F64)
    hipLaunchKernelGGL(slab_diag_kernel<double>, dim3(nb), dim3(256), 0, h->stream, (double*)Kslab, (long long)ldk,
                       (long long)row0, (long long)nrp, (long long)N, (long long)Np, sf2 + diag_add);
  else
    hipLaunchKernelGGL(slab_diag_kernel<float>, dim3(nb), dim3(256), 0, h->stream, (float*)Kslab, (long long)ldk,
                       (long long)row0, (long long)nrp, (long long)N, (long long)Np, (float)sf2 + (float)diag_add);
  GPK_LAUNCH_CHECK(h);
  return GPK_OK;
}

extern "C" int gpk_predict_mean(gpk_handle h, int dtype, const void* X, const void* alpha, int64_t N, int D, int P,
                                const double* ls, double sf2, const double* y_mean, const double* y_std,
                                const void* Xq, int64_t M, void* mean) {
  if (!h) return GPK_BAD_ARG;
  GPK_REQUIRE(h, X && alpha && Xq && mean && y_mean && y_std, "predict_mean: null pointer");
  GPK_REQUIRE(h, N >= 1 && M >= 1, "predict_mean: empty input");
  GPK_REQUIRE(h, D >= 1 && D <= PM_DMAX, "predict_mean: D must be in [1, 16]");
  GPK_REQUIRE(h, P >= 1 && P <= PM_PMAX, "predict_mean: P must be in [1, 16]");
  GPK_REQUIRE(h, dtype == GPK_F32 || dtype == GPK_F64, "predict_mean: bad dtype");
  LsArr l;
  GPK_TRY(fill_ls(h, ls, D, l));
  PArr ym{}, ys{};
  for (int p = 0; p < P; ++p) { ym.v[p] = y_mean[p]; ys.v[p] = y_std[p]; }
  Ls16 l16;
  for (int d = 0; d < 16; ++d) l16.v[d] = l.v[d];
  const int64_t nqb = (M + 256 * PM_QPT - 1) / (256 * PM_QPT);
  const int64_t gran = (M <= 512 && N <= 16384) ? 32 : PM_TJ;
  int64_t S = (2048 + nqb - 1) / nqb;
  if (dtype == GPK_F32 && S < (N + 2047) / 2048) S = (N + 2047) / 2048;
  const int64_t maxS = (N + gran - 1) / gran;
  if (S > maxS) S = maxS;
  if (S < 1) S = 1;
  if (S > 65535) S = 65535;
  int64_t chunk = (N + S - 1) / S;
  chunk = (chunk + gran - 1) / gran * gran;
  S = (N + chunk - 1) / chunk;
  const size_t es = dtype == GPK_F64 ? 8 : 4;
  void* partial = nullptr;
  GPK_TRY(gpk_scratch(h, (size_t)S * M * P * es, &partial));
  dim3 grid((unsigned)nqb, (unsigned)S);
  const int64_t tot = M * P;
  const int d4 = (D + 3) / 4, p4 = (P + 3) / 4;
  if (h->gram_log)
    fprintf(stderr, "GPKMEAN %s %lld %lld %d P%d d%d p%d gran%lld s%lld chunk%lld\n", dtype == GPK_F64 ? "f64" : "f32", (long long)N,
            (long long)M, D, P, d4, p4, (long long)gran, (long long)S, (long long)chunk);
  if (dtype == GPK_F64) {
    hipLaunchKernelGGL(pm_pick<double>(d4, p4), grid, dim3(256), 0, h->stream, (const double*)X,
                       (const double*)alpha, (long long)N, D, P, l16, (const double*)Xq, (long long)M,
                       (long long)chunk, (double*)partial);
    GPK_LAUNCH_CHECK(h);
    hipLaunchKernelGGL(mean_reduce_kernel<double>, dim3((unsigned)((tot + 255) / 256)), dim3(256), 0, h->stream,
                       (const double*)partial, (int)S, (long long)M, P, sf2, ym, ys, (double*)mean);
  } else {
    hipLaunchKernelGGL(pm_pick<float>(d4, p4), grid, dim3(256), 0, h->stream, (const float*)X,
                       (const float*)alpha, (long long)N, D, P, l16, (const float*)Xq, (long long)M,
                       (long long)chunk, (float*)partial);
    GPK_LAUNCH_CHECK(h);
    hipLaunchKernelGGL(mean_reduce_kernel<float>, dim3((unsigned)((tot + 255) / 256)), dim3(256), 0, h->stream,
                       (const float*)partial, (int)S, (long long)M, P, (float)sf2, ym, ys, (float*)mean);
  }
  GPK_LAUNCH_CHECK(h);
  return GPK_OK;
}

extern "C" int gpk_predict_mean_multi(gpk_handle h, int dtype, const void* X, const void* alpha, int64_t N, int D,
                                      int B, const double* ls, const double* sf2, const double* y_mean,
                                      const double* y_std, const void* Xq, int64_t M, void* mean) {
  if (!h) return GPK_BAD_ARG;
  GPK_REQUIRE(h, X && alpha && Xq && mean && ls && sf2 && y_mean && y_std, "predict_mean_multi: null pointer");
  GPK_REQUIRE(h, N >= 1 && M >= 1, "predict_mean_multi: empty input");
  GPK_REQUIRE(h, D >= 1 && D <= PM_DMAX, "predict_mean_multi: D must be in [1, 16]");
  GPK_REQUIRE(h, B >= 1 && B <= 8, "predict_mean_multi: B must be in [1, 8]");
  GPK_REQUIRE(h, dtype == GPK_F32 || dtype == GPK_F64, "predict_mean_multi: bad dtype");
  PArr ym{}, ys{}, sf{};
  double w[8 * PM_DMAX];
  for (int b = 0; b < B; ++b) {
    ym.v[b] = y_mean[b]; ys.v[b] = y_std[b]; sf.v[b] = sf2[b];
    for (int d = 0; d < D; ++d) {
      GPK_REQUIRE(h, ls[b * D + d] > 0.0, "predict_mean_multi: length-scales must be positive");
      w[b * D + d] = 1.0 / (ls[b * D + d] * ls[b * D + d]);
    }
  }
  const int64_t nqb = (M + 256 * PM_QPT - 1) / (256 * PM_QPT);
  int64_t S = (2048 + nqb - 1) / nqb;
  const int64_t maxS = (N + PM_TJ - 1) / PM_TJ;
  if (S > maxS) S = maxS;
  if (S < 1) S = 1;
  if (S > 65535) S = 65535;
  int64_t chunk = (N + S - 1) / S;
  chunk = (chunk + PM_TJ - 1) / PM_TJ * PM_TJ;
  S = (N + chunk - 1) / chunk;
  const size_t es = dtype == GPK_F64 ? 8 : 4;
  const size_t wbytes = 8 * PM_DMAX * sizeof(double);
  void* ws = nullptr;
  GPK_TRY(gpk_scratch(h, wbytes + (size_t)S * M * B * es, &ws));
  double* w_dev = (double*)ws;
  void* partial = (char*)ws + wbytes;
  GPK_CHECK_HIP(h, hipStreamSynchronize(h->stream));
  memcpy(h->h_small, w, (size_t)B * D * sizeof(double));
  GPK_CHECK_HIP(h, hipMemcpyAsync(w_dev, h->h_small, (size_t)B * D * sizeof(double), hipMemcpyHostToDevice, h->stream));
  dim3 grid((unsigned)nqb, (unsigned)S);
  const int64_t tot = M * B;
  const int d4 = (D + 3) / 4, b4 = (B + 3) / 4;
  if (h->gram_log)
    fprintf(stderr, "GPKMEAN %s %lld %lld %d B%d d%d p%d gran%d s%lld chunk%lld\n", dtype == GPK_F64 ? "f64" : "f32", (long long)N,
            (long long)M, D, B, d4, b4 <= 1 ? 1 : 2, PM_TJ, (long long)S, (long long)chunk);
  if (dtype == GPK_F64) {
    hipLaunchKernelGGL(pmm_pick<double>(d4, b4), grid, dim3(256), 0, h->stream, (const double*)X,
                       (const double*)alpha, (long long)N, D, B, (const double*)w_dev, (const double*)Xq,
                       (long long)M, (long long)chunk, (double*)partial);
    GPK_LAUNCH_CHECK(h);
    hipLaunchKernelGGL(mean_reduce_multi_kernel<double>, dim3((unsigned)((tot + 255) / 256)), dim3(256), 0, h->stream,
                       (const double*)partial, (int)S, (long long)M, B, sf, ym, ys, (double*)mean);
  } else {
    hipLaunchKernelGGL(pmm_pick<float>(d4, b4), grid, dim3(256), 0, h->stream, (const float*)X,
                       (const float*)alpha, (long long)N, D, B, (const double*)w_dev, (const float*)Xq,
                       (long long)M, (long long)chunk, (float*)partial);
    GPK_LAUNCH_CHECK(h);
    hipLaunchKernelGGL(mean_reduce_multi_kernel<float>, dim3((unsigned)((tot + 255) / 256)), dim3(256), 0, h->stream,
                       (const float*)partial, (int)S, (long long)M, B, sf, ym, ys, (float*)mean);
  }
  GPK_LAUNCH_CHECK(h);
  return GPK_OK;
}

extern "C" int gpk_colsumsq(gpk_handle h, int dtype, const void* B, int64_t Np, int64_t Mp, int64_t ldb,
                            double* out) {
  if (!h) return GPK_BAD_ARG;
  GPK_REQUIRE(h, B && out, "colsumsq: null pointer");
  GPK_REQUIRE(h, Np > 0 && Mp > 0 && Mp % 128 == 0 && ldb >= Mp, "colsumsq: Mp must be a multiple of 128");
  GPK_REQUIRE(h, dtype == GPK_F32 || dtype == GPK_F64, "colsumsq: bad dtype");
  const int64_t nmb = Mp / 128;
  int64_t S = (2048 + nmb - 1) / nmb;
  if (S > Np / 64) S = Np / 64;
  if (S < 1) S = 1;
  if (S > 32768) S = 32768;
  const int64_t rows_per = (Np + S - 1) / S;
  S = (Np + rows_per - 1) / rows_per;
  void* partial = nullptr;
  GPK_TRY(gpk_scratch(h, (size_t)2 * S * Mp * sizeof(double), &partial));
  dim3 grid((unsigned)nmb, (unsigned)S);
  if (dtype == GPK_F64)
    hipLaunchKernelGGL(colsumsq_kernel<double>, grid, dim3(256), 0, h->stream, (const double*)B,
                       (long long)rows_per, (long long)Np, (long long)ldb, (double*)partial, (long long)Mp);
  else
    hipLaunchKernelGGL(colsumsq_kernel<float>, grid, dim3(256), 0, h->stream, (const float*)B, (long long)rows_per,
                       (long long)Np, (long long)ldb, (double*)partial, (long long)Mp);
  GPK_LAUNCH_CHECK(h);
  hipLaunchKernelGGL(colsum_reduce_kernel, dim3((unsigned)((Mp + 255) / 256)), dim3(256), 0, h->stream,
                     (const double*)partial, (int)(2 * S), (long long)Mp, out);
  GPK_LAUNCH_CHECK(h);
  return GPK_OK;
}

int gpk_colsum_finalize(gpk_handle h, const double* partial, int S, int64_t Mp, int64_t M, double kss, double floor_,
                        double* var) {
  hipLaunchKernelGGL(colsum_finalize_kernel, dim3((unsigned)((M + 255) / 256)), dim3(256), 0, h->stream, partial, S,
                     (long long)Mp, (long long)M, kss, floor_, var);
  GPK_LAUNCH_CHECK(h);
  return GPK_OK;
}
int gpk_colsum_finalize_packed(gpk_handle h, const double* partial, int S, int64_t Mp, int64_t M, double kss, double floor_,
                               const float* mean, int P, const double* y_std, double recheck_below, unsigned* low_count,
                               double* out) {
  PArr ys{};
  for (int p = 0; p < P; ++p) ys.v[p] = y_std[p];
  hipLaunchKernelGGL(colsum_finalize_packed_kernel, dim3((unsigned)((M + 255) / 256)), dim3(256), 0, h->stream, partial, S,
                     (long long)Mp, (long long)M, kss, floor_, mean, P, ys, recheck_below, low_count, out);
  GPK_LAUNCH_CHECK(h);
  return GPK_OK;
}
extern "C" int gpk_pack_mean_var(gpk_handle h, int dtype, const void* mean, const double* var, int64_t M, int P,
                                 const double* y_std, double* out) {
  if (!h) return GPK_BAD_ARG;
  GPK_REQUIRE(h, mean && var && y_std && out && M >= 1 && P >= 1 && P <= GPK_MAX_P, "pack_mean_var: bad argument");
  GPK_REQUIRE(h, dtype == GPK_F32 || dtype == GPK_F64, "pack_mean_var: bad dtype");
  PArr ys{};
  for (int p = 0; p < P; ++p) ys.v[p] = y_std[p];
  const dim3 grid((unsigned)((M + 255) / 256));
  if (dtype == GPK_F32)
    hipLaunchKernelGGL(pack_mean_var_kernel<float>, grid, dim3(256), 0, h->stream, (const float*)mean, var, (long long)M, P, ys, out);
  else
    hipLaunchKernelGGL(pack_mean_var_kernel<double>, grid, dim3(256), 0, h->stream, (const double*)mean, var, (long long)M, P, ys, out);
  GPK_LAUNCH_CHECK(h);
  return GPK_OK;
}
int gpk_colsum_reduce(gpk_handle h, const double* partial, int S, int64_t Mp, double* out) {
  hipLaunchKernelGGL(colsum_reduce_kernel, dim3((unsigned)((Mp + 255) / 256)), dim3(256), 0, h->stream, partial, S,
                     (long long)Mp, out);
  GPK_LAUNCH_CHECK(h);
  return GPK_OK;
}

int gpk_var_finalize(gpk_handle h, const double* ss, int64_t M, double kss, double floor_, double* var) {
  hipLaunchKernelGGL(var_finalize_kernel, dim3((unsigned)((M + 255) / 256)), dim3(256), 0, h->stream, ss,
                     (long long)M, kss, floor_, var);
  GPK_LAUNCH_CHECK(h);
  return GPK_OK;
}
```

unmanned_aerial_vehicles_amd/csrc/gpk_internal.h:

```cpp
#pragma once
#include <hip/hip_runtime.h>

#include <cstdint>
#include <cstdio>
#include <cstring>
#include <string>
#include <vector>

#include "../../include/gpk.h"

struct gpk_model;
struct gpk_bmodel;
struct gpk_sparse;

struct gpk_context {
  int device = 0;
  gpk_model* model = nullptr;
  gpk_bmodel* bmodel = nullptr;
  gpk_sparse* sparse = nullptr;
  hipStream_t stream = nullptr;
  hipStream_t own_stream = nullptr;
  bool user_stream = false;
  std::string err;
  void* scratch = nullptr;
  size_t scratch_bytes = 0;
  int* d_info = nullptr;
  double* h_small = nullptr;
  double* d_small = nullptr;
  unsigned* d_count = nullptr;
  unsigned* d_cov_count = nullptr;
  void* serve_dev = nullptr;
  size_t serve_dev_bytes = 0;
  void* serve_host = nullptr;
  size_t serve_host_bytes = 0;
  int gemm_small_tiles = 1024;
  int gemm_tiny_tiles = 320;
  int gemm_balanced = 1;
  long long gemm_balanced_max_tiles = 32768;
  int cus = 0;
  int trtri_levels = 1;
  int trsm256 = 1;
  int small_path = 1;
  int k3_stream_min_np = 512;
  int k5_split2_tile = 0;
  int ptile = 1;
  int ptile_max_np = 24576;
  int ptile_prog_max_nt = 128;
  int ptile_inv_max_np = 4608;
  int ptile_prog_rows = 8;
  int* d_ptile = nullptr;
  int ptile_slots = 512;
  int ptile_sr = 1, ptile_sr_max_nt = 36;
  int ptile_single_max_nt = 96;
  int ptile_launches = 0;
  std::string ptile_trace_request;
  std::string ptile_trace_path;
  long long ptile_trace_n = 0;
  int sparse_panel = 0;
  int sparse_slabs = 0;
  int debug_fill = 0;
  int gemm_log = 0;
  int gram_log = 0;
  struct TimedLaunch { hipEvent_t e0 = nullptr, e1 = nullptr; int tag = 0; };
  int timing = 0;
  std::vector<TimedLaunch> timed;
  long long timed_count = 0;
  struct BatchBuf { const char* base; long long stride; };
  int batch = 1;
  std::vector<BatchBuf> bbufs;
};

#define GPK_CHECK_HIP(h, call)                                                          \
  do {                                                                                  \
    hipError_t e_ = (call);                                                             \
    if (e_ != hipSuccess) {                                                             \
      (h)->err = std::string(#call) + ": " + hipGetErrorString(e_);                     \
      return GPK_HIP_ERROR;                                                             \
    }                                                                                   \
  } while (0)

#define GPK_REQUIRE(h, cond, msg)                                                       \
  do {                                                                                  \
    if (!(cond)) {                                                                      \
      (h)->err = std::string("bad argument: ") + (msg);                                 \
      return GPK_BAD_ARG;                                                               \
    }                                                                                   \
  } while (0)

#define GPK_LAUNCH_CHECK(h)                                                             \
  do {                                                                                  \
    hipError_t e_ = hipGetLastError();                                                  \
    if (e_ != hipSuccess) {                                                             \
      (h)->err = std::string("kernel launch: ") + hipGetErrorString(e_);                \
      return GPK_HIP_ERROR;                                                             \
    }                                                                                   \
  } while (0)

#define GPK_TRY(expr)                                                                   \
  do {                                                                                  \
    int rc_ = (expr);                                                                   \
    if (rc_ != GPK_OK) return rc_;                                                      \
  } while (0)

int gpk_scratch(gpk_handle h, size_t bytes, void** out);

constexpr size_t GPK_PTILE_CTRL_INTS = 16 + 8 * 512 + 1024 + 10 * 8 * 512;
int gpk_potrf_ptile(gpk_handle h, double* A, int64_t Np, int64_t lda, double* winv, int row0, int* used, double* wt = nullptr,
                    double* wband = nullptr, int64_t ldw = 0, int zero_info = 0);
int gpk_potrf_ptile_check(gpk_handle h, int gave_up = -1);
void gpk_model_free(gpk_handle h);
void gpk_bmodel_free(gpk_handle h);
void gpk_sparse_free(gpk_handle h);
int gpk_potrf_enqueue(gpk_handle h, double* A, int64_t Np, int64_t lda, double* winv);
int gpk_potrf_finish(gpk_handle h, const int* hinfo_all, int* info, int gave_up = -1);
constexpr int GPK_STATUS_OFF = 480;
int gpk_tril_block_absmax_f64_enqueue(gpk_handle h, const double* W, int64_t n, int64_t ld, unsigned* out);
int gpk_potrf_trtri_enqueue(gpk_handle h, double* A, int64_t Np, int64_t lda, double* winv, double* W, int64_t ldw, double* wt,
                            int* used);
int gpk_lml_terms_enqueue(gpk_handle h, const double* L, int64_t N, int64_t ldl, const double* Y, const double* alpha, int P,
                          double* dout, int with_status = 0);
int gpk_lml_grad_enqueue(gpk_handle h, const double* X, int64_t N, int D, const double* ls, double sf2, const double* alpha,
                         int P, const double* Kinv, int64_t ldk, double* dout);
int gpk_lml_chain_batched(gpk_handle h, int B, const double* X, int64_t N, int D, const double* ls , const double* sf2,
                          const double* noise, const double* Yn, int64_t Ne, double* K, int64_t Np, double* winv, double* W,
                          double* T, size_t tsz, double* alpha, double* Kinv, double* terms, double* grads, int* info);

constexpr int GPK_TIMING_RING = 64;
inline void gpk_time_begin(gpk_handle h, int tag) {
  if (!h->timing) return;
  auto& t = h->timed[(size_t)(h->timed_count % GPK_TIMING_RING)];
  t.tag = tag;
  (void)hipEventRecord(t.e0, h->stream);
}
inline void gpk_time_end(gpk_handle h) {
  if (!h->timing) return;
  auto& t = h->timed[(size_t)(h->timed_count % GPK_TIMING_RING)];
  (void)hipEventRecord(t.e1, h->stream);
  ++h->timed_count;
}

inline long long gpk_bstride(gpk_handle h, const void* p) {
  if (h->batch <= 1) return 0;
  const char* c = (const char*)p;
  for (const auto& b : h->bbufs)
    if (c >= b.base && c < b.base + b.stride) return b.stride;
  return 0;
}

constexpr int GPK_ZERO_BAND_TILES = 16;

constexpr int GPK_GRAD_W = 17;

struct GemmArgs {
  const void* A;
  const void* B;
  void* C;
  int64_t lda, ldb, ldc;
  int m, n, k;
  int ta, tb;
  double alpha, beta;
  int lower_only;
  int kb0, kb_row, kb_col, ke0, ke_row, ke_col;
  int heavy_first;
  int k_super;
  int epilogue;
  unsigned* amax;
  const void* amax_base;
  const double* cov_q;
  double cov_sf2, cov_noise;
  int cov_d, cov_m;
  const double* grad_x;
  const double* grad_z;
  int grad_n, grad_m, grad_d;
  double grad_ls[16];
  int nbatch;
  long long sA, sB, sC;
};
inline GemmArgs gemm_args(const void* A, int64_t lda, int ta, const void* B, int64_t ldb, int tb,
                          void* C, int64_t ldc, int m, int n, int k, double alpha, double beta) {
  GemmArgs g{};
  g.A = A; g.B = B; g.C = C; g.lda = lda; g.ldb = ldb; g.ldc = ldc;
  g.m = m; g.n = n; g.k = k; g.ta = ta; g.tb = tb; g.alpha = alpha; g.beta = beta;
  g.lower_only = 0; g.kb0 = 0; g.kb_row = 0; g.kb_col = 0; g.ke0 = -1; g.ke_row = 0; g.ke_col = 0; g.epilogue = 0; g.heavy_first = 0; g.k_super = 0;
  g.nbatch = 0; g.sA = 0; g.sB = 0; g.sC = 0; g.amax = nullptr; g.amax_base = nullptr;
  g.cov_q = nullptr; g.cov_sf2 = 0.0; g.cov_noise = 0.0; g.cov_d = 0; g.cov_m = 0;
  return g;
}
int gpk_gemm(gpk_handle h, int dtype, const GemmArgs& g);
int gpk_gemm_tile(gpk_handle h, const GemmArgs& g);

constexpr int GPK_SMALL_MAX_M = 32;
constexpr int64_t GPK_SMALL_MAX_NP = 16384;
constexpr int GPK_SMALL_MAX_MODELS = 8;
constexpr int GPK_SMALL_COV_COUNTERS = GPK_SMALL_MAX_MODELS * 129 + GPK_SMALL_MAX_MODELS;
bool gpk_small_ok(int64_t Np, int D, int P, int64_t M);
enum { GPK_SMALL_PREDICT, GPK_SMALL_COV, GPK_SMALL_GRAD };
size_t gpk_small_work_doubles(int call, int64_t Np, int B, int64_t M, int D, int P, int F = 1);
int gpk_small_predict(gpk_handle h, int B, const double* const* X, const double* const* alpha, int64_t N, int D, int P,
                      const double* ls, const double* sf2, const double* y_mean, const double* y_std,
                      const double* const* W, int64_t Np, int64_t ldw, const double* kss, double floor_,
                      const double* Xq, int64_t M, double* work, double* mean_out, double* var_out);
int gpk_small_cov_multi(gpk_handle h, int B, const double* const* X, const double* const* alpha, int64_t N, int D, int P,
                        const double* ls, const double* sf2, const double* y_mean, const double* y_std, const double* const* W,
                        int64_t Np, int64_t ldw, const double* noise, const double* Xq, int64_t M, double* work,
                        double* mean_out, double* cov_out);
int gpk_small_grad_multi(gpk_handle h, int B, const double* const* X, const double* const* alpha, int64_t N, int D, int P,
                         const double* ls, const double* sf2, const double* y_mean, const double* y_std, const double* const* W,
                         int64_t Np, int64_t ldw, const double* kss, double floor_, const double* Xq, int64_t M, double* work,
                         double* mean_out, double* var_out, double* dmean_out, double* dvar_out);
int gpk_small_two(gpk_handle h, int call, const double* X, const double* alpha, int64_t N, int D, int P, const double* ls,
                  double sf2, const double* y_mean, const double* y_std, const double* W0, const double* W1, int64_t Np,
                  int64_t ldw, double kss, double floor_, double noise, const double* Xq, int64_t M, double* work,
                  double* mean_out, double* var_out, double* dmean_out, double* dvar_out, double* cov_out);
int gpk_small_two_multi(gpk_handle h, int call, int B, const double* const* X, const double* const* alpha, int64_t N, int D, int P,
                        const double* ls, const double* sf2, const double* y_mean, const double* y_std, const double* const* W0,
                        const double* const* W1, int64_t Np, int64_t ldw, const double* kss, double floor_, const double* noise,
                        const double* Xq, int64_t M, double* work, double* mean_out, double* var_out, double* dmean_out,
                        double* dvar_out, double* cov_out);
int gpk_serve_two(gpk_handle h, int call, const double* X, const double* alpha, int64_t N, int D, int P, const double* ls,
                  double sf2, const double* y_mean, const double* y_std, const double* W0, const double* W1, int64_t Np,
                  int64_t ldw, double kss, double floor_, double noise, const double* Xq_host, int64_t M, double* mean_host,
                  double* var_host, double* dmean_host, double* dvar_host, double* cov_host);
int gpk_serve_two_multi(gpk_handle h, int call, int B, const double* const* X, const double* const* alpha, int64_t N, int D, int P,
                        const double* ls, const double* sf2, const double* y_mean, const double* y_std, const double* const* W0,
                        const double* const* W1, int64_t Np, int64_t ldw, const double* kss, double floor_, const double* noise,
                        const double* Xq_host, int64_t M, double* mean_host, double* var_host, double* dmean_host, double* dvar_host,
                        double* cov_host);
int gpk_cov_from_v(gpk_handle h, const double* VA, const double* VB, int64_t rows, const double* Xq, int64_t M, int D,
                   const double* ls, double sf2, double noise, double* cov, int64_t ldc);

int gpk_cross_split2(gpk_handle h, const float* Xq, int64_t M, const float* X, int64_t N, int D, const double* ls,
                     double sf2, double scale, void* dst);
int gpk_var_finalize(gpk_handle h, const double* ss, int64_t M, double kss, double floor_, double* var);
int gpk_colsum_reduce(gpk_handle h, const double* partial, int S, int64_t Mp, double* out);
int gpk_colsum_finalize(gpk_handle h, const double* partial, int S, int64_t Mp, int64_t M, double kss, double floor_,
                        double* var);
int gpk_colsum_finalize_packed(gpk_handle h, const double* partial, int S, int64_t Mp, int64_t M, double kss, double floor_,
                               const float* mean, int P, const double* y_std, double recheck_below, unsigned* low_count,
                               double* out);
```

unmanned_aerial_vehicles_amd/csrc/gpk_k5split.hip:

```cpp
#include <cmath>

#include "gpk_internal.h"

namespace {

typedef __bf16 bf16x8 __attribute__((ext_vector_type(8)));
typedef unsigned int V16 __attribute__((ext_vector_type(4)));
typedef float f16v __attribute__((ext_vector_type(16)));
template <int V> struct IntC { static constexpr int value = V; };

constexpr int ROWB = 384;
constexpr int LROW = 112;
typedef _Float16 f16x8 __attribute__((ext_vector_type(8)));

__device__ __forceinline__ unsigned bf16_rn_bits(float x) {
  const unsigned u = __float_as_uint(x);
  return (u + 0x7fffu + ((u >> 16) & 1u)) & 0xffff0000u;
}
__device__ __forceinline__ void split3(float x, unsigned& h0, unsigned& h1, unsigned& h2) {
  h0 = bf16_rn_bits(x);
  const float r1 = x - __uint_as_float(h0);
  h1 = bf16_rn_bits(r1);
  const float r2 = r1 - __uint_as_float(h1);
  h2 = __float_as_uint(r2);
}

__global__ __launch_bounds__(256) void split3_kernel(const float* __restrict__ src, long long rows, long long cols,
                                                     long long ld, V16* __restrict__ dst) {
  const long long hc = cols / 8;
  const long long e = (long long)blockIdx.x * 256 + threadIdx.x;
  if (e >= rows * hc) return;
  const long long row = e / hc, hb = e - row * hc;
  const float4* s4 = reinterpret_cast<const float4*>(src + row * ld + hb * 8);
  const float4 lo = s4[0], hi = s4[1];
  const float v[8] = {lo.x, lo.y, lo.z, lo.w, hi.x, hi.y, hi.z, hi.w};
  V16 f[3];
#pragma unroll
  for (int j = 0; j < 4; ++j) {
    unsigned a0, a1, a2, b0, b1, b2;
    split3(v[2 * j], a0, a1, a2);
    split3(v[2 * j + 1], b0, b1, b2);
    f[0][j] = (a0 >> 16) | b0;
    f[1][j] = (a1 >> 16) | b1;
    f[2][j] = (a2 >> 16) | (b2 & 0xffff0000u);
  }
  V16* d = dst + (((row >> 2) * (hc >> 1) + (hb >> 1)) * 4 + (row & 3)) * 6 + (hb & 1) * 3;
  d[0] = f[0]; d[1] = f[1]; d[2] = f[2];
}

struct SParams {
  const char* A;
  const char* B;
  double* out;
  long long rsa, rsb;
  long long Mp;
  int ntm, ntn, nst;
};

template <int WR>
__global__ __launch_bounds__(WR * 128, 2) void k5_split_kernel(SParams p) {
  constexpr int TMR = 64 * WR;
  constexpr int SSZ = (TMR + 128) * LROW;
  constexpr int BOFF = TMR * LROW;
  __shared__ __attribute__((aligned(16))) char lds[2 * SSZ];
  constexpr int NT = WR * 128, NCH = (TMR + 128) * 6, NQ = (NCH + NT - 1) / NT;
  constexpr int GSZ = WR == 2 ? 64 : 32;
  constexpr int BH = 1024 / TMR;
  const int tid = threadIdx.x, lane = tid & 63, wave = __builtin_amdgcn_readfirstlane(tid >> 6);
  const int wm = wave >> 1, wn = wave & 1;
  const int row_w = wm * 64, col_w = wn * 64;

  const int ntm = p.ntm * 128 / TMR;
  const int xcd = blockIdx.x & 7, j = blockIdx.x >> 3;
  const int grp = j / GSZ, slot = j - grp * GSZ;
  const int st = grp * 8 + ((grp & 1) ? 7 - xcd : xcd);
  if (st >= p.nst) return;
  const int per = BH * p.ntn, nfull = ntm / BH, hlast = ntm - nfull * BH, total = ntm * p.ntn;
  const int t = st * GSZ + slot;
  if (t >= total) return;
  int tm, tn;
  {
    const int band = min(t / per, nfull);
    const int idx = t - band * per, hh = band < nfull ? BH : hlast;
    tn = idx / hh;
    tm = band * BH + (idx - tn * hh);
  }
  const int band0 = min(st * GSZ / per, nfull), band1 = min(min(st * GSZ + GSZ - 1, total - 1) / per, nfull);
  tm = ntm - 1 - tm;
  const int rhi = (band1 - band0 <= 1) ? ntm - 1 - band0 * BH : tm;
  const int nkt = (rhi + 1) * (TMR / 16);

  const int row0 = tm * TMR, col0 = tn * 128;
  f16v acc[2][2];
#pragma unroll
  for (int a = 0; a < 2; ++a)
#pragma unroll
    for (int b = 0; b < 2; ++b)
#pragma unroll
      for (int i = 0; i < 16; ++i) acc[a][b][i] = 0.f;

  unsigned goff[NQ], lofs[NQ];
  bool isb[NQ], live[NQ];
#pragma unroll
  for (int q = 0; q < NQ; ++q) {
    const int g = tid + NT * q;
    live[q] = __builtin_amdgcn_readfirstlane(g < NCH ? 1 : 0) != 0;
    isb[q] = __builtin_amdgcn_readfirstlane(g >= TMR * 6 ? 1 : 0) != 0;
    const int c = live[q] ? (isb[q] ? g - TMR * 6 : g) : 0, row = c / 6, w = c - row * 6;
    goff[q] = (unsigned)((long long)(row >> 2) * p.rsa + ((row & 3) * 6 + w) * 16);
    lofs[q] = (isb[q] ? BOFF : 0) + row * LROW + w * 16;
  }
  const char* ua = p.A + (long long)(row0 >> 2) * p.rsa;
  const char* ub = p.B + (long long)(col0 >> 2) * p.rsb;
  V16 rr[2][NQ];
  auto fetch = [&](int tile, auto slotc) {
    constexpr int sl = decltype(slotc)::value;
    const long long ko = (long long)min(tile, nkt - 1) * ROWB;
#pragma unroll
    for (int q = 0; q < NQ; ++q) {
      if (NCH % NT != 0 && !live[q]) continue;
      const __amdgpu_buffer_rsrc_t rs =
          __builtin_amdgcn_make_buffer_rsrc(const_cast<char*>((isb[q] ? ub : ua) + ko), 0, 0x7fffffff, 0x00020000);
      rr[sl][q] = __builtin_amdgcn_raw_buffer_load_b128(rs, goff[q], 0, 0);
    }
  };
  auto stage = [&](auto bufc, auto slotc) {
    constexpr int sl = decltype(slotc)::value, bi = decltype(bufc)::value;
    char* buf = lds + bi * SSZ;
#pragma unroll
    for (int q = 0; q < NQ; ++q)
      if (NCH % NT == 0 || live[q]) *reinterpret_cast<V16*>(buf + lofs[q]) = rr[sl][q];
  };
  const int fr = lane & 31, fh = lane >> 5;
  auto mfmas = [&](const bf16x8 (&af)[2][3], const bf16x8 (&bf)[2][3]) {
#pragma unroll
    for (int a = 0; a < 2; ++a)
#pragma unroll
      for (int b = 0; b < 2; ++b) {
        f16v c = acc[a][b];
        c = __builtin_amdgcn_mfma_f32_32x32x16_bf16(af[a][2], bf[b][0], c, 0, 0, 0);
        c = __builtin_amdgcn_mfma_f32_32x32x16_bf16(af[a][0], bf[b][2], c, 0, 0, 0);
        c = __builtin_amdgcn_mfma_f32_32x32x16_bf16(af[a][1], bf[b][1], c, 0, 0, 0);
        c = __builtin_amdgcn_mfma_f32_32x32x16_bf16(af[a][1], bf[b][0], c, 0, 0, 0);
        c = __builtin_amdgcn_mfma_f32_32x32x16_bf16(af[a][0], bf[b][1], c, 0, 0, 0);
        c = __builtin_amdgcn_mfma_f32_32x32x16_bf16(af[a][0], bf[b][0], c, 0, 0, 0);
        acc[a][b] = c;
      }
  };
  auto frags = [&](auto bufc, bf16x8 (&af)[2][3], bf16x8 (&bf)[2][3]) {
    constexpr int bi = decltype(bufc)::value;
#pragma unroll
    for (int a = 0; a < 2; ++a)
#pragma unroll
      for (int s = 0; s < 3; ++s)
        af[a][s] = __builtin_bit_cast(bf16x8, *reinterpret_cast<const V16*>(lds + bi * SSZ + (row_w + 32 * a + fr) * LROW + (fh * 3 + s) * 16));
#pragma unroll
    for (int b = 0; b < 2; ++b)
#pragma unroll
      for (int s = 0; s < 3; ++s)
        bf[b][s] = __builtin_bit_cast(bf16x8, *reinterpret_cast<const V16*>(lds + bi * SSZ + BOFF + (col_w + 32 * b + fr) * LROW + (fh * 3 + s) * 16));
  };
  bf16x8 FA[2][2][3], FB[2][2][3];
  fetch(0, IntC<0>{});
  stage(IntC<0>{}, IntC<0>{});
  fetch(1, IntC<1>{});
  stage(IntC<1>{}, IntC<1>{});
  fetch(2, IntC<0>{});
  fetch(3, IntC<1>{});
  __syncthreads();
  frags(IntC<0>{}, FA[0], FB[0]);
  __syncthreads();
  auto body = [&](int kt, auto ksc) {
    constexpr int cur = decltype(ksc)::value & 1;
    stage(IntC<cur>{}, IntC<cur>{});
    fetch(kt + 4, IntC<cur>{});
    frags(IntC<(cur ^ 1)>{}, FA[cur ^ 1], FB[cur ^ 1]);
    mfmas(FA[cur], FB[cur]);
    constexpr int NMF = 24, NRD = 12;
    __builtin_amdgcn_sched_group_barrier(0x200, NQ, 0);
#pragma unroll
    for (int g = 0; g < NQ; ++g) {
      __builtin_amdgcn_sched_group_barrier(0x008, (NMF + NQ - 1) / NQ, 0);
      __builtin_amdgcn_sched_group_barrier(0x100, (NRD + NQ - 1) / NQ, 0);
      __builtin_amdgcn_sched_group_barrier(0x020, 1, 0);
    }
    __syncthreads();
  };
  for (int kt = 0; kt + 3 < nkt; kt += 4) {
    body(kt, IntC<0>{});
    body(kt + 1, IntC<1>{});
    body(kt + 2, IntC<2>{});
    body(kt + 3, IntC<3>{});
  }

  double* red = reinterpret_cast<double*>(lds);
#pragma unroll
  for (int b = 0; b < 2; ++b) {
    float s = 0.f;
#pragma unroll
    for (int a = 0; a < 2; ++a)
#pragma unroll
      for (int i = 0; i < 16; ++i) { const float v = acc[a][b][i]; s = __builtin_fmaf(v, v, s); }
    s += __shfl_xor(s, 32, 64);
    if (lane < 32) red[wm * 128 + col_w + 32 * b + lane] = (double)s;
  }
  __syncthreads();
  if (tid < 128) {
    double t2 = 0.0;
#pragma unroll
    for (int w = 0; w < WR; ++w) t2 += red[w * 128 + tid];
    p.out[(long long)tm * p.Mp + col0 + tid] = t2;
  }
}

struct DParams {
  const char* A;
  const char* B;
  double* out;
  const float* wscale;
  long long rba, rbb;
  long long Mp;
  float kscale;
  int ntm, ntn, nst;
  int per_pad;
};

template <int AB>
__global__ __launch_bounds__(256, 1) void k5_direct_kernel(DParams p) {
  constexpr int TMR = 128 * AB, GSZ = 32, BH = 1024 / TMR;
  const int tid = threadIdx.x, lane = tid & 63, wave = __builtin_amdgcn_readfirstlane(tid >> 6);
  const int ntm = p.ntm * 128 / TMR;
  const int xcd = blockIdx.x & 7, j = blockIdx.x >> 3;
  const int grp = j / GSZ, slot = j - grp * GSZ;
  const int st = grp * 8 + ((grp & 1) ? 7 - xcd : xcd);
  if (st >= p.nst) return;
  const int nfull = ntm / BH, hlast = ntm - nfull * BH;
  const int t = st * GSZ + slot;
  int tm, tn;
  {
    const int band = min(t / p.per_pad, nfull);
    const int idx = t - band * p.per_pad, hh = band < nfull ? BH : hlast;
    if (idx >= hh * p.ntn) return;
    tn = idx / hh;
    tm = band * BH + (idx - tn * hh);
  }
  tm = ntm - 1 - tm;
  const int row0 = tm * TMR, col0 = tn * 128;
  const int nkt = (row0 + 32 * AB * (wave + 1)) / 16;

  f16v acc[AB][4];
#pragma unroll
  for (int a = 0; a < AB; ++a)
#pragma unroll
    for (int b = 0; b < 4; ++b)
#pragma unroll
      for (int i = 0; i < 16; ++i) acc[a][b][i] = 0.f;

  const unsigned vo = lane * 16;
  const char* ua = p.A + (long long)((row0 >> 5) + AB * wave) * p.rba;
  const char* ub = p.B + (long long)(col0 >> 5) * p.rbb;
  const int rba = (int)p.rba, rbb = (int)p.rbb;
  V16 FA[3][AB][2], FB[3][4][2];
  auto rsrc_at = [&](const char* base, int tile) {
    return __builtin_amdgcn_make_buffer_rsrc(const_cast<char*>(base + (long long)min(tile, nkt - 1) * 2048), 0, 0x7fffffff, 0x00020000);
  };
  auto ldf = [&](const __amdgpu_buffer_rsrc_t rs, int blk_off, V16 (&f)[2]) {
    f[0] = __builtin_amdgcn_raw_buffer_load_b128(rs, vo, blk_off, 0);
    f[1] = __builtin_amdgcn_raw_buffer_load_b128(rs, vo, blk_off + 1024, 0);
  };
  auto fill = [&](int tile, auto slc) {
    constexpr int S = decltype(slc)::value;
    const __amdgpu_buffer_rsrc_t ra = rsrc_at(ua, tile), rb = rsrc_at(ub, tile);
    ldf(ra, 0, FA[S][0]);
#pragma unroll
    for (int b = 0; b < 4; ++b) ldf(rb, b * rbb, FB[S][b]);
#pragma unroll
    for (int a = 1; a < AB; ++a) ldf(ra, a * rba, FA[S][a]);
  };
  auto mm = [&](f16v& c, const V16 (&fa)[2], const V16 (&fb)[2]) {
    const f16x8 a0 = __builtin_bit_cast(f16x8, fa[0]), a1 = __builtin_bit_cast(f16x8, fa[1]);
    const f16x8 b0 = __builtin_bit_cast(f16x8, fb[0]), b1 = __builtin_bit_cast(f16x8, fb[1]);
    c = __builtin_amdgcn_mfma_f32_32x32x16_f16(a1, b0, c, 0, 0, 0);
    c = __builtin_amdgcn_mfma_f32_32x32x16_f16(a0, b1, c, 0, 0, 0);
    c = __builtin_amdgcn_mfma_f32_32x32x16_f16(a0, b0, c, 0, 0, 0);
  };
  fill(0, IntC<0>{});
  fill(1, IntC<1>{});
  fill(2, IntC<2>{});
  auto body = [&](int kt, auto slc) {
    constexpr int S = decltype(slc)::value;
    const __amdgpu_buffer_rsrc_t ra = rsrc_at(ua, kt + 3), rb = rsrc_at(ub, kt + 3);
#pragma unroll
    for (int a = 0; a < AB; ++a) {
#pragma unroll
      for (int b = 0; b < 4; ++b) {
        mm(acc[a][b], FA[S][a], FB[S][b]);
        if (a == AB - 1) ldf(rb, b * rbb, FB[S][b]);
        __builtin_amdgcn_sched_barrier(0);
      }
      ldf(ra, a * rba, FA[S][a]);
      __builtin_amdgcn_sched_barrier(0);
    }
  };
  int kt = 0;
  for (; kt + 3 <= nkt; kt += 3) {
    body(kt, IntC<0>{});
    body(kt + 1, IntC<1>{});
    body(kt + 2, IntC<2>{});
  }
  if (kt < nkt) {
    body(kt, IntC<0>{});
    if (kt + 1 < nkt) body(kt + 1, IntC<1>{});
  }

  __shared__ double red[4 * 128];
  const float alpha = (1.0f / p.wscale[(row0 + 32 * AB * wave) >> 7]) * (1.0f / p.kscale);
#pragma unroll
  for (int b = 0; b < 4; ++b) {
    float s = 0.f;
#pragma unroll
    for (int a = 0; a < AB; ++a)
#pragma unroll
      for (int i = 0; i < 16; ++i) { const float v = alpha * acc[a][b][i]; s = __builtin_fmaf(v, v, s); }
    s += __shfl_xor(s, 32, 64);
    if (lane < 32) red[wave * 128 + 32 * b + lane] = (double)s;
  }
  __syncthreads();
  if (tid < 128) p.out[(long long)tm * p.Mp + col0 + tid] = (red[tid] + red[128 + tid]) + (red[256 + tid] + red[384 + tid]);
}

__global__ __launch_bounds__(256) void split2_kernel(const float* __restrict__ src, long long rows, long long cols,
                                                      long long ld, const float* __restrict__ scales,
                                                      V16* __restrict__ dst) {
  const int lane = threadIdx.x & 63, wave = threadIdx.x >> 6;
  const long long KB = cols >> 4;
  const long long kb = (long long)blockIdx.x * 4 + wave, rb = blockIdx.y;
  if (kb >= KB) return;
  const int r = lane & 31, h = lane >> 5;
  const long long row = rb * 32 + r;
  const float sc = scales[row >> 7];
  const float4* s4 = reinterpret_cast<const float4*>(src + row * ld + kb * 16 + h * 8);
  const float4 lo = s4[0], hi = s4[1];
  const float v[8] = {lo.x, lo.y, lo.z, lo.w, hi.x, hi.y, hi.z, hi.w};
  f16x8 p0, p1;
#pragma unroll
  for (int j = 0; j < 8; ++j) {
    const float x = v[j] * sc;
    const _Float16 h0 = (_Float16)x;
    p0[j] = h0;
    p1[j] = (_Float16)(x - (float)h0);
  }
  V16* d = dst + ((rb * KB + kb) * 2) * 64 + lane;
  d[0] = __builtin_bit_cast(V16, p0);
  d[64] = __builtin_bit_cast(V16, p1);
}

__global__ __launch_bounds__(256) void tril_block_absmax_kernel(const float* __restrict__ A, long long n, long long lda,
                                                                unsigned* __restrict__ out) {
  const long long i = blockIdx.x;
  float m = 0.f;
  for (long long jj = threadIdx.x; jj <= i; jj += 256) m = fmaxf(m, fabsf(A[i * lda + jj]));
  for (int off = 32; off > 0; off >>= 1) m = fmaxf(m, __shfl_xor(m, off, 64));
  if ((threadIdx.x & 63) == 0) atomicMax(out + (i >> 7), __float_as_uint(m));
}
__global__ __launch_bounds__(256) void tril_block_absmax_f64_kernel(const double* __restrict__ A, long long n, long long lda,
                                                                    unsigned* __restrict__ out) {
  const long long i = blockIdx.x;
  float m = 0.f;
  for (long long jj = threadIdx.x; jj <= i; jj += 256) m = fmaxf(m, fabsf((float)A[i * lda + jj]));
  for (int off = 32; off > 0; off >>= 1) m = fmaxf(m, __shfl_xor(m, off, 64));
  if ((threadIdx.x & 63) == 0) atomicMax(out + (i >> 7), __float_as_uint(m));
}
__global__ __launch_bounds__(256) void split2_f64_kernel(const double* __restrict__ src, long long n, long long ld,
                                                          const float* __restrict__ scales, V16* __restrict__ dst) {
  typedef double dv2 __attribute__((ext_vector_type(2)));
  const int lane = threadIdx.x & 63, wave = threadIdx.x >> 6;
  const long long KB = n >> 4;
  const long long kb = (long long)blockIdx.x * 4 + wave, rb = blockIdx.y;
  if (kb >= KB || kb * 16 >= ((rb * 32) / 128 + 1) * 128) return;
  const int r = lane & 31, h = lane >> 5;
  const long long row = rb * 32 + r, col0 = kb * 16 + h * 8;
  const float sc = scales[row >> 7];
  const dv2* s2 = reinterpret_cast<const dv2*>(src + row * ld + col0);
  const dv2 a = s2[0], b = s2[1], c = s2[2], d = s2[3];
  const double v[8] = {a.x, a.y, b.x, b.y, c.x, c.y, d.x, d.y};
  f16x8 p0, p1;
#pragma unroll
  for (int j = 0; j < 8; ++j) {
    const float x = (col0 + j <= row ? (float)v[j] : 0.f) * sc;
    const _Float16 h0 = (_Float16)x;
    p0[j] = h0;
    p1[j] = (_Float16)(x - (float)h0);
  }
  V16* o = dst + ((rb * KB + kb) * 2) * 64 + lane;
  o[0] = __builtin_bit_cast(V16, p0);
  o[64] = __builtin_bit_cast(V16, p1);
}
__global__ void absmax_to_scale_kernel(unsigned* __restrict__ io, int nblk) {
  const int b = blockIdx.x * blockDim.x + threadIdx.x;
  if (b >= nblk) return;
  const unsigned u = io[b];
  const int e = (int)(u >> 23) - 127;
  float s = 1.f;
  if (u != 0u && u < 0x7f800000u) {
    const int se = ((u & 0x7fffffu) == 0u ? 15 : 14) - e;
    s = __uint_as_float((unsigned)(min(max(se, -126), 100) + 127) << 23);
  }
  reinterpret_cast<float*>(io)[b] = s;
}

}

extern "C" int gpk_split3(gpk_handle h, const float* src, int64_t rows, int64_t cols, int64_t ld, void* dst) {
  if (!h) return GPK_BAD_ARG;
  GPK_REQUIRE(h, src && dst, "split3: null pointer");
  GPK_REQUIRE(h, rows >= 4 && rows % 4 == 0 && cols >= 16 && cols % 16 == 0 && ld >= cols && ld % 4 == 0,
              "split3: rows must be a multiple of 4 and cols a multiple of 16");
  GPK_REQUIRE(h, ((uintptr_t)src % 16) == 0 && ((uintptr_t)dst % 16) == 0, "split3: buffers must be 16-byte aligned");
  const long long n = rows * (cols / 8);
  hipLaunchKernelGGL(split3_kernel, dim3((unsigned)((n + 255) / 256)), dim3(256), 0, h->stream, src, (long long)rows,
                     (long long)cols, (long long)ld, (V16*)dst);
  GPK_LAUNCH_CHECK(h);
  return GPK_OK;
}

extern "C" int gpk_split2_rows(gpk_handle h, const float* W, int64_t n, int64_t ld, float* scales, void* dst) {
  if (!h) return GPK_BAD_ARG;
  GPK_REQUIRE(h, W && scales && dst, "split2_rows: null pointer");
  GPK_REQUIRE(h, n >= 128 && n % 128 == 0 && ld >= n && ld % 4 == 0 && n < (1ll << 24), "split2_rows: n must be a multiple of 128");
  GPK_REQUIRE(h, ((uintptr_t)W % 16) == 0 && ((uintptr_t)dst % 16) == 0, "split2_rows: buffers must be 16-byte aligned");
  const int nblk = (int)(n / 128);
  GPK_CHECK_HIP(h, hipMemsetAsync(scales, 0, nblk * sizeof(float), h->stream));
  hipLaunchKernelGGL(tril_block_absmax_kernel, dim3((unsigned)n), dim3(256), 0, h->stream, W, (long long)n, (long long)ld,
                     reinterpret_cast<unsigned*>(scales));
  GPK_LAUNCH_CHECK(h);
  hipLaunchKernelGGL(absmax_to_scale_kernel, dim3((unsigned)((nblk + 255) / 256)), dim3(256), 0, h->stream,
                     reinterpret_cast<unsigned*>(scales), nblk);
  GPK_LAUNCH_CHECK(h);
  hipLaunchKernelGGL(split2_kernel, dim3((unsigned)((n / 16 + 3) / 4), (unsigned)(n / 32)), dim3(256), 0, h->stream, W,
                     (long long)n, (long long)n, (long long)ld, (const float*)scales, (V16*)dst);
  GPK_LAUNCH_CHECK(h);
  return GPK_OK;
}

int gpk_tril_block_absmax_f64_enqueue(gpk_handle h, const double* W, int64_t n, int64_t ld, unsigned* out) {
  GPK_CHECK_HIP(h, hipMemsetAsync(out, 0, (n / 128) * sizeof(unsigned), h->stream));
  hipLaunchKernelGGL(tril_block_absmax_f64_kernel, dim3((unsigned)n), dim3(256), 0, h->stream, W, (long long)n, (long long)ld, out);
  GPK_LAUNCH_CHECK(h);
  return GPK_OK;
}

static int split2_rows_f64_impl(gpk_handle h, const double* W, int64_t n, int64_t ld, float* scales, void* dst, bool have_absmax) {
  GPK_REQUIRE(h, W && scales && dst, "split2_rows_f64: null pointer");
  GPK_REQUIRE(h, n >= 128 && n % 128 == 0 && ld >= n && ld % 2 == 0 && n < (1ll << 24), "split2_rows_f64: n must be a multiple of 128");
  GPK_REQUIRE(h, ((uintptr_t)W % 16) == 0 && ((uintptr_t)dst % 16) == 0, "split2_rows_f64: buffers must be 16-byte aligned");
  const int nblk = (int)(n / 128);
  if (!have_absmax) GPK_TRY(gpk_tril_block_absmax_f64_enqueue(h, W, n, ld, reinterpret_cast<unsigned*>(scales)));
  hipLaunchKernelGGL(absmax_to_scale_kernel, dim3((unsigned)((nblk + 255) / 256)), dim3(256), 0, h->stream,
                     reinterpret_cast<unsigned*>(scales), nblk);
  GPK_LAUNCH_CHECK(h);
  hipLaunchKernelGGL(split2_f64_kernel, dim3((unsigned)((n / 16 + 3) / 4), (unsigned)(n / 32)), dim3(256), 0, h->stream, W,
                     (long long)n, (long long)ld, (const float*)scales, (V16*)dst);
  GPK_LAUNCH_CHECK(h);
  return GPK_OK;
}

extern "C" int gpk_split2_rows_f64(gpk_handle h, const double* W, int64_t n, int64_t ld, float* scales, void* dst) {
  if (!h) return GPK_BAD_ARG;
  return split2_rows_f64_impl(h, W, n, ld, scales, dst, false);
}

extern "C" int gpk_split2_rows_f64_absmax(gpk_handle h, const double* W, int64_t n, int64_t ld, float* scales, void* dst) {
  if (!h) return GPK_BAD_ARG;
  return split2_rows_f64_impl(h, W, n, ld, scales, dst, true);
}

namespace {
int split2_launch(gpk_handle h, const char* who, const float* X, int64_t N, int D, const double* ls, double sf2, const void* W2,
                  const float* w_scales, int64_t Np, const float* Xq, int64_t M, void* work2, void** partial, int* S) {
  GPK_REQUIRE(h, X && W2 && w_scales && Xq && work2, (std::string(who) + ": null pointer").c_str());
  GPK_REQUIRE(h, N >= 1 && M >= 1 && Np == gpk_padded(N), (std::string(who) + ": Np must equal gpk_padded(N)").c_str());
  GPK_REQUIRE(h, h->batch == 1, (std::string(who) + ": not available in batched mode").c_str());
  GPK_REQUIRE(h, sf2 > 0.0 && D >= 1 && D <= 16, (std::string(who) + ": sf2 must be positive and D <= 16").c_str());
  const int64_t Mp = gpk_padded(M);
  const int ntm = (int)(Np / 128), ntn = (int)(Mp / 128);
  GPK_REQUIRE(h, (long long)ntm * ntn < (1ll << 30) && Np * 128 * 4 < (1ll << 31) && Mp / 64 < 65536,
              (std::string(who) + ": size too large").c_str());
  const double k_scale = std::ldexp(1.0, 14 - (int)std::floor(std::log2(sf2)));
  GPK_TRY(gpk_cross_split2(h, Xq, M, X, N, D, ls, sf2, k_scale, work2));
  int ab = 1;
  if (Np % 512 == 0 && (h->k5_split2_tile == 2 || (Np / 512) * (long long)ntn >= 512)) ab = 4;
  else if (Np % 256 == 0 && (Np / 256) * (long long)ntn >= 512) ab = 2;
  if (h->k5_split2_tile == 1) ab = 1;
  const int ntmT = (int)(Np / (128 * ab)), gsz = 32;
  GPK_TRY(gpk_scratch(h, (size_t)ntmT * Mp * sizeof(double), partial));
  DParams p;
  p.A = (const char*)W2; p.B = (const char*)work2; p.out = (double*)*partial; p.wscale = w_scales;
  p.rba = p.rbb = Np * 128;
  p.Mp = Mp;
  p.kscale = (float)k_scale;
  p.ntm = ntm; p.ntn = ntn;
  {
    const int bh = 1024 / (128 * ab), per = bh * ntn, pad = (per + gsz - 1) / gsz * gsz;
    p.per_pad = (pad - per) * 8 <= per ? pad : per;
    const int nfull = ntmT / bh, hlast = ntmT - nfull * bh;
    p.nst = (int)(((long long)nfull * p.per_pad + (long long)hlast * ntn + gsz - 1) / gsz);
  }
  const long long nblocks = (long long)((p.nst + 7) / 8) * 8 * gsz;
  gpk_time_begin(h, GPK_TIMED_K5);
  if (ab == 4) hipLaunchKernelGGL(k5_direct_kernel<4>, dim3((unsigned)nblocks), dim3(256), 0, h->stream, p);
  else if (ab == 2) hipLaunchKernelGGL(k5_direct_kernel<2>, dim3((unsigned)nblocks), dim3(256), 0, h->stream, p);
  else hipLaunchKernelGGL(k5_direct_kernel<1>, dim3((unsigned)nblocks), dim3(256), 0, h->stream, p);
  gpk_time_end(h);
  GPK_LAUNCH_CHECK(h);
  *S = ntmT;
  return GPK_OK;
}
}

extern "C" int gpk_predict_var_inv_split2(gpk_handle h, const float* X, int64_t N, int D, const double* ls, double sf2,
                                          const void* W2, const float* w_scales, int64_t Np, const float* Xq, int64_t M,
                                          double kss, double floor_, void* work2, double* var) {
  if (!h) return GPK_BAD_ARG;
  GPK_REQUIRE(h, var, "predict_var_inv_split2: null pointer");
  void* partial = nullptr;
  int S = 0;
  GPK_TRY(split2_launch(h, "predict_var_inv_split2", X, N, D, ls, sf2, W2, w_scales, Np, Xq, M, work2, &partial, &S));
  return gpk_colsum_finalize(h, (const double*)partial, S, gpk_padded(M), M, kss, floor_, var);
}

extern "C" int gpk_predict_mean_var_split2(gpk_handle h, const float* X, const float* alpha, int64_t N, int D, int P,
                                           const double* ls, double sf2, const double* center, const double* y_mean,
                                           const double* y_std, const void* W2, const float* w_scales, int64_t Np,
                                           const float* Xq, int64_t M, double kss, double floor_, void* work2,
                                           float* mean_tmp, double recheck_below, unsigned* low_count, double* out) {
  if (!h) return GPK_BAD_ARG;
  GPK_REQUIRE(h, alpha && y_mean && y_std && mean_tmp && out && P >= 1 && P <= GPK_MAX_P, "predict_mean_var_split2: bad argument");
  if (center) GPK_TRY(gpk_predict_mean_mfma(h, X, alpha, N, D, P, ls, sf2, center, y_mean, y_std, Xq, M, mean_tmp));
  else GPK_TRY(gpk_predict_mean(h, GPK_F32, X, alpha, N, D, P, ls, sf2, y_mean, y_std, Xq, M, mean_tmp));
  void* partial = nullptr;
  int S = 0;
  GPK_TRY(split2_launch(h, "predict_mean_var_split2", X, N, D, ls, sf2, W2, w_scales, Np, Xq, M, work2, &partial, &S));
  return gpk_colsum_finalize_packed(h, (const double*)partial, S, gpk_padded(M), M, kss, floor_, mean_tmp, P, y_std,
                                    recheck_below, low_count, out);
}

extern "C" int gpk_predict_var_inv_split(gpk_handle h, const float* X, int64_t N, int D, const double* ls, double sf2,
                                         const void* W3, int64_t Np, const float* Xq, int64_t M, double kss,
                                         double floor_, float* work, void* work3, double* var) {
  if (!h) return GPK_BAD_ARG;
  GPK_REQUIRE(h, X && W3 && Xq && work && work3 && var, "predict_var_inv_split: null pointer");
  GPK_REQUIRE(h, N >= 1 && M >= 1 && Np == gpk_padded(N), "predict_var_inv_split: Np must equal gpk_padded(N)");
  GPK_REQUIRE(h, h->batch == 1, "predict_var_inv_split: not available in batched mode");
  const int64_t Mp = gpk_padded(M);
  const int ntm = (int)(Np / 128), ntn = (int)(Mp / 128);
  GPK_REQUIRE(h, (long long)ntm * ntn < (1ll << 30) && Np * 24 * 64 < (1ll << 31), "predict_var_inv_split: size too large");
  GPK_TRY(gpk_cross_gram_t(h, GPK_F32, Xq, M, X, N, D, ls, sf2, work, Np));
  GPK_TRY(gpk_split3(h, work, Mp, Np, Np, work3));
  const int wr = (Np % 256 == 0) ? 4 : 2;
  const int ntmT = (int)(Np / (64 * wr)), gsz = wr == 2 ? 64 : 32;
  void* partial = nullptr;
  GPK_TRY(gpk_scratch(h, (size_t)ntmT * Mp * sizeof(double), &partial));
  SParams p;
  p.A = (const char*)W3; p.B = (const char*)work3; p.out = (double*)partial;
  p.rsa = Np * 24; p.rsb = Np * 24; p.Mp = Mp;
  p.ntm = ntm; p.ntn = ntn;
  p.nst = (int)(((long long)ntmT * ntn + gsz - 1) / gsz);
  const long long nblocks = (long long)((p.nst + 7) / 8) * 8 * gsz;
  gpk_time_begin(h, GPK_TIMED_K5);
  if (wr == 4) hipLaunchKernelGGL(k5_split_kernel<4>, dim3((unsigned)nblocks), dim3(512), 0, h->stream, p);
  else hipLaunchKernelGGL(k5_split_kernel<2>, dim3((unsigned)nblocks), dim3(256), 0, h->stream, p);
  gpk_time_end(h);
  GPK_LAUNCH_CHECK(h);
  return gpk_colsum_finalize(h, (const double*)partial, ntmT, Mp, M, kss, floor_, var);
}
```

unmanned_aerial_vehicles_amd/device.py:

```python
from __future__ import annotations

import ctypes as C
import os
import threading

import numpy as np

from . import _lib
from ._lib import GPK_F32, GPK_F64, GPKError, NotPositiveDefinite

_backends = {}
_backends_lock = threading.Lock()


def _torch():
    import torch
    return torch


class Backend:

    def __init__(self, device_index=0):
        torch = _torch()
        self.lib = _lib.load()
        if not torch.cuda.is_available():
            raise RuntimeError("no HIP device visible: the GP kernels need an MI355X (there is no CPU fallback)")
        self.device_index = int(device_index)
        self.device = torch.device("cuda", self.device_index)
        torch.cuda.set_device(self.device)
        h = C.c_void_p()
        rc = self.lib.gpk_create(C.byref(h), self.device_index)
        if rc != _lib.GPK_OK:
            raise GPKError(rc, "gpk_create failed")
        self.h = h
        self.lock = threading.RLock()
        if os.environ.get("GPK_DEBUG_FILL"):
            self.check(self.lib.gpk_set_option(self.h, b"debug_fill", 1))
        self.bind_stream()
        self.low_count = torch.zeros((1,), dtype=torch.int32, device=self.device)
        self.low_seen = 0

    def bind_stream(self):
        torch = _torch()
        s = torch.cuda.current_stream(self.device).cuda_stream
        self.check(self.lib.gpk_set_stream(self.h, C.c_void_p(s)))

    def check(self, rc):
        if rc == _lib.GPK_OK:
            return
        msg = self.lib.gpk_last_error(self.h).decode()
        if rc == _lib.GPK_NOT_PD:
            raise NotPositiveDefinite(msg)
        raise GPKError(rc, msg)

    def sync(self):
        self.check(self.lib.gpk_synchronize(self.h))

    def set_options(self, **opts):
        for k, v in opts.items():
            if isinstance(v, str):
                self.check(self.lib.gpk_set_option_str(self.h, k.encode(), v.encode()))
            else:
                self.check(self.lib.gpk_set_option(self.h, k.encode(), int(v)))
        return self

    def empty(self, shape, dtype):
        t = _torch().empty(shape, dtype=dtype, device=self.device)
        if os.environ.get("GPK_DEBUG_FILL"):
            t.fill_(float(os.environ["GPK_DEBUG_FILL"]) if t.is_floating_point() else 255)
        return t

    def upload(self, a, dtype=None):
        torch = _torch()
        t = torch.from_numpy(np.ascontiguousarray(a))
        if dtype is not None:
            t = t.to(dtype)
        return t.to(self.device)


def get_backend(device_index=None) -> Backend:
    torch = _torch()
    if isinstance(device_index, Backend):
        return device_index
    if device_index is None:
        device_index = torch.cuda.current_device() if torch.cuda.is_available() else 0
    with _backends_lock:
        b = _backends.get(device_index)
        if b is None:
            b = _backends[device_index] = Backend(device_index)
        return b


_workers = {}


def worker_backends(device_index, n):
    torch = _torch()
    main = get_backend(device_index)
    with _backends_lock:
        pool = _workers.setdefault(main.device_index, [])
        while len(pool) < n:
            pool.append((Backend(main.device_index), torch.cuda.Stream(device=main.device)))
        return pool[:n]


def padded(n):
    return (int(n) + 127) // 128 * 128


def _p(t):
    return C.c_void_p(t.data_ptr())


class DeviceGP:

    VAR_PANEL_BYTES = 6 << 30
    VAR_PANEL_MAX = 16384
    INVERSE_EAGER_NP = 32768
    FUSED_INVERSE_NP = 4608
    MAX_FEATURES = 16

    def __init__(self, X, Yn, backend: Backend | None = None):
        torch = _torch()
        self.be = backend or get_backend()
        X = np.ascontiguousarray(X, dtype=np.float64)
        Yn = np.ascontiguousarray(Yn, dtype=np.float64)
        if X.ndim != 2 or Yn.ndim != 2 or X.shape[0] != Yn.shape[0]:
            raise ValueError("X must be (N, D) and Y (N, P)")
        self.N, self.D = X.shape
        self.P = Yn.shape[1]
        if not (1 <= self.D <= self.MAX_FEATURES):
            raise ValueError(f"D must be in [1, {self.MAX_FEATURES}] on the MI355X path (got {self.D})")
        if not (1 <= self.P <= _lib.GPK_MAX_P):
            raise ValueError(f"P must be in [1, {_lib.GPK_MAX_P}]")
        self.Np = padded(self.N)
        self._Xh = X
        self._xc = X.mean(axis=0)
        self._r2 = {}
        self.X = self.be.upload(X)
        self.Yn = self.be.upload(Yn)
        self.K = None
        self.winv = None
        self.alpha = self.be.empty((self.N, self.P), torch.float64)
        self.factored = False
        self.ls = None
        self.sf2 = None
        self._f32 = None
        self._Winv = {}
        self._host_args = None
        self._amp = self._alpha_sq = None
        self._Kinv = None
        self.replica = False

    def _ensure_K(self):
        torch = _torch()
        if self.K is None:
            self.K = self.be.empty((self.Np, self.Np), torch.float64)
            self.winv = self.be.empty((self.Np, 128), torch.float64)

    def gram(self, ls, sf2, diag_add):
        self._ensure_K()
        ls = np.ascontiguousarray(np.broadcast_to(np.asarray(ls, dtype=np.float64), (self.D,)))
        be = self.be
        with be.lock:
            be.bind_stream()
            be.check(be.lib.gpk_gram(be.h, GPK_F64, _p(self.X), self.N, self.D, ls.ctypes.data_as(_lib._dp),
                                     float(sf2), float(diag_add), _p(self.K), self.Np))
        self.ls, self.sf2 = ls, float(sf2)
        self.factored = False
        self._f32 = None
        self._Winv = {}

    def factorize(self, ls, sf2, diag_add):
        self.gram(ls, sf2, diag_add)
        be = self.be
        info = C.c_int(0)
        with be.lock:
            be.check(be.lib.gpk_potrf(be.h, _p(self.K), self.Np, self.Np, _p(self.winv), C.byref(info)))
        self.factored = True

    def load_factor(self, L, ls, sf2):
        torch = _torch()
        self._ensure_K()
        L = np.asarray(L, dtype=np.float64)
        Kh = torch.eye(self.Np, dtype=torch.float64)
        Kh[: self.N, : self.N] = torch.from_numpy(np.tril(L))
        self.K.copy_(Kh)
        be = self.be
        with be.lock:
            be.bind_stream()
            be.check(be.lib.gpk_leaf_inverses(be.h, _p(self.K), self.Np, self.Np, _p(self.winv)))
        self.ls = np.ascontiguousarray(np.broadcast_to(np.asarray(ls, dtype=np.float64), (self.D,)))
        self.sf2 = float(sf2)
        self.factored = True
        self._f32 = None
        self._Winv = {}

    def solve_alpha(self, method="auto"):
        assert self.factored
        be = self.be
        if method == "auto":
            method = "inverse" if ("f64" in self._Winv or self.Np <= self.INVERSE_EAGER_NP) else "chain"
        if method == "inverse":
            W = self.inverse_factor(False)
            with be.lock:
                be.bind_stream()
                be.check(be.lib.gpk_potrs_inv(be.h, _p(W), self.Np, self.Np, _p(self.Yn), self.N, self.P,
                                              _p(self.alpha)))
        else:
            with be.lock:
                be.bind_stream()
                be.check(be.lib.gpk_potrs(be.h, _p(self.K), self.Np, self.Np, _p(self.winv), _p(self.Yn), self.N,
                                          self.P, _p(self.alpha)))
        self._amp = self._alpha_sq = None
        if self._f32:
            self._f32.pop("alpha", None)

    def set_alpha(self, alpha):
        self.alpha.copy_(self.be.upload(np.asarray(alpha, dtype=np.float64).reshape(self.N, self.P)))
        self._amp = self._alpha_sq = None
        if self._f32:
            self._f32.pop("alpha", None)

    def lml_terms(self):
        be = self.be
        out = np.zeros(1 + self.P)
        with be.lock:
            be.bind_stream()
            be.check(be.lib.gpk_lml_terms(be.h, _p(self.K), self.N, self.Np, _p(self.Yn), _p(self.alpha), self.P,
                                          out.ctypes.data_as(_lib._dp)))
        return out[0], out[1:]

    def lml_grad(self, noise, logdet_weight=None):
        torch = _torch()
        assert self.factored
        if self.D > 16:
            raise ValueError("analytic LML gradients support D <= 16")
        if self._Kinv is None:
            self._Kinv = self.be.empty((self.Np, self.Np), torch.float64)
        W = self.inverse_factor(False)
        be = self.be
        g = np.zeros(self.D + 2)
        ratio = 1.0 if logdet_weight is None else self.P / float(logdet_weight)
        if not ratio > 0.0:
            raise ValueError("logdet_weight must be positive")
        alpha = self.alpha if ratio == 1.0 else self.alpha * float(np.sqrt(ratio))
        with be.lock:
            be.bind_stream()
            be.check(be.lib.gpk_wtw(be.h, _p(W), self.Np, self.Np, _p(self._Kinv), self.Np))
            be.check(be.lib.gpk_lml_grad(be.h, _p(self.X), self.N, self.D, self.ls.ctypes.data_as(_lib._dp),
                                         self.sf2, float(noise), _p(alpha), self.P, _p(self._Kinv), self.Np,
                                         g.ctypes.data_as(_lib._dp)))
        return g if ratio == 1.0 else g / ratio

    def lml_eval(self, ls, sf2, diag_add, noise, eval_gradient=True):
        torch = _torch()
        if eval_gradient and self.D > 16:
            raise ValueError("analytic LML gradients support D <= 16")
        self._ensure_K()
        ls = np.ascontiguousarray(np.broadcast_to(np.asarray(ls, dtype=np.float64), (self.D,)))
        be = self.be
        self._f32 = None
        self._Winv = {}
        self.factored = False
        W = be.empty((self.Np, self.Np), torch.float64)
        work = be.empty(((self.Np // 2 + 128) ** 2,), torch.float64)
        want_kinv = eval_gradient or self.Np <= self.FUSED_INVERSE_NP
        if want_kinv and self._Kinv is None:
            self._Kinv = be.empty((self.Np, self.Np), torch.float64)
        terms = np.zeros(1 + self.P)
        g = np.zeros(self.D + 2) if eval_gradient else None
        info = C.c_int(0)
        with be.lock:
            be.bind_stream()
            self.ls, self.sf2 = ls, float(sf2)
            be.check(be.lib.gpk_lml_eval(
                be.h, _p(self.X), self.N, self.D, ls.ctypes.data_as(_lib._dp), float(sf2), float(diag_add), float(noise),
                _p(self.Yn), self.P, _p(self.K), self.Np, _p(self.winv), _p(W), _p(work), _p(self.alpha),
                _p(self._Kinv) if want_kinv else None, terms.ctypes.data_as(_lib._dp),
                g.ctypes.data_as(_lib._dp) if eval_gradient else None, C.byref(info)))
        self.factored = True
        self._Winv["f64"] = W
        self._amp = self._alpha_sq = None
        return terms[0], terms[1:], g

    def release_grad_buffers(self):
        self._Kinv = None

    def L_host(self):
        return np.tril(self.K[: self.N, : self.N].cpu().numpy())

    def alpha_host(self):
        return self.alpha.cpu().numpy()

    def _f32_data(self):
        torch = _torch()
        if self._f32 is None:
            self._f32 = {}
        if "X" not in self._f32:
            self._f32["X"] = self.X.to(torch.float32)
        if "alpha" not in self._f32:
            self._f32["alpha"] = self.alpha.to(torch.float32)
        return self._f32

    def _f32_factor(self):
        torch = _torch()
        c = self._f32_data()
        if "L" not in c:
            assert self.factored
            be = self.be
            Lf = be.empty((self.Np, self.Np), torch.float32)
            wf = be.empty((self.Np, 128), torch.float32)
            with be.lock:
                be.bind_stream()
                be.check(be.lib.gpk_factor_to_f32(be.h, _p(self.K), self.Np, self.Np, _p(self.winv), _p(Lf),
                                                  self.Np, _p(wf)))
            c["L"], c["winv"] = Lf, wf
        return c

    def _as_queries(self, Xq, tdtype):
        torch = _torch()
        if isinstance(Xq, torch.Tensor):
            q = Xq.to(device=self.be.device, dtype=tdtype).contiguous()
        else:
            q = self.be.upload(np.ascontiguousarray(Xq, dtype=np.float64), tdtype)
        if q.ndim != 2 or q.shape[1] != self.D:
            raise ValueError(f"queries must be (M, {self.D})")
        return q

    def timing(self, enable=True):
        be = self.be
        with be.lock:
            be.bind_stream()
            be.check(be.lib.gpk_timing(be.h, 1 if enable else 0))

    def kernel_times(self, tag, max_n=64):
        be = self.be
        ms = np.zeros(max_n)
        n = C.c_int(0)
        with be.lock:
            be.check(be.lib.gpk_kernel_times(be.h, int(tag), ms.ctypes.data_as(_lib._dp), max_n, C.byref(n)))
        return ms[: n.value].copy()

    MFMA_MEAN_R2_MAX = 64.0

    def mean_kernel_choice(self):
        key = self.ls.tobytes()
        if key not in self._r2:
            u = (self._Xh - self._xc) / self.ls
            self._r2 = {key: 0.5 * np.log2(np.e) * float(np.max(np.einsum("ij,ij->i", u, u)))}
        return "mfma" if (self.P <= 8 and self._r2[key] <= self.MFMA_MEAN_R2_MAX) else "valu"

    def predict_mean_dev(self, Xq, y_mean, y_std, dtype="float64", kernel="auto", _alpha=None, _kernel=None):
        torch = _torch()
        f32 = dtype in ("float32", np.float32, torch.float32)
        if kernel == "auto":
            kernel = self.mean_kernel_choice() if f32 else "valu"
        if kernel not in ("valu", "mfma") or (kernel == "mfma" and not f32):
            raise ValueError("kernel must be 'auto', 'valu' or 'mfma' (mfma: float32 only)")
        tdt = torch.float32 if f32 else torch.float64
        q = self._as_queries(Xq, tdt)
        M = q.shape[0]
        out = self.be.empty((M, self.P), tdt)
        if M == 0:
            return out
        if f32:
            c = self._f32_data()
            Xd, ad = c["X"], c["alpha"]
        else:
            Xd, ad = self.X, (self.alpha if _alpha is None else _alpha)
        ym = np.ascontiguousarray(np.broadcast_to(np.asarray(y_mean, dtype=np.float64), (self.P,)))
        ys = np.ascontiguousarray(np.broadcast_to(np.asarray(y_std, dtype=np.float64), (self.P,)))
        be = self.be
        ls_, sf2_ = (self.ls, self.sf2) if _kernel is None else (np.ascontiguousarray(_kernel[0]), float(_kernel[1]))
        if kernel == "mfma":
            with be.lock:
                be.bind_stream()
                be.check(be.lib.gpk_predict_mean_mfma(be.h, _p(Xd), _p(ad), self.N, self.D, self.P,
                                                      self.ls.ctypes.data_as(_lib._dp), self.sf2,
                                                      self._xc.ctypes.data_as(_lib._dp), ym.ctypes.data_as(_lib._dp),
                                                      ys.ctypes.data_as(_lib._dp), _p(q), M, _p(out)))
            return out
        with be.lock:
            be.bind_stream()
            be.check(be.lib.gpk_predict_mean(be.h, GPK_F32 if f32 else GPK_F64, _p(Xd), _p(ad), self.N, self.D,
                                             self.P, ls_.ctypes.data_as(_lib._dp), sf2_,
                                             ym.ctypes.data_as(_lib._dp), ys.ctypes.data_as(_lib._dp), _p(q), M,
                                             _p(out)))
        return out

    HOST_PATH_MAX_M = 256

    def host_path_ok(self, M, want_var):
        if not (1 <= M <= self.HOST_PATH_MAX_M and self.D <= 16):
            return False
        return (not want_var) or ("f64" in self._Winv) or self.Np <= self.INVERSE_EAGER_NP

    def _host_call_args(self, y_mean, y_std):
        c = self._host_args
        if (c is None or c[0] is not self.X or c[1] is not self.alpha or c[2] is not self.ls or c[3] is not y_mean
                or c[4] is not y_std):
            ym = np.ascontiguousarray(np.broadcast_to(np.asarray(y_mean, dtype=np.float64), (self.P,)))
            ys = np.ascontiguousarray(np.broadcast_to(np.asarray(y_std, dtype=np.float64), (self.P,)))
            c = self._host_args = (self.X, self.alpha, self.ls, y_mean, y_std, ym, ys, self.X.data_ptr(),
                                   self.alpha.data_ptr(), self.ls.ctypes.data, ym.ctypes.data, ys.ctypes.data)
        return c

    def predict_host(self, Xq, y_mean, y_std, kss=None, floor=0.0):
        assert self.factored or kss is None
        Xq = np.ascontiguousarray(Xq, dtype=np.float64)
        M = Xq.shape[0]
        if Xq.ndim != 2 or Xq.shape[1] != self.D:
            raise ValueError(f"queries must be (M, {self.D})")
        mean = np.empty((M, self.P))
        var = np.empty((M,)) if kss is not None else None
        W = self.inverse_factor(False) if kss is not None else None
        be = self.be
        c = self._host_call_args(y_mean, y_std)
        with be.lock:
            be.bind_stream()
            be.check(be.lib.gpk_predict_host(be.h, c[7], c[8], self.N, self.D, self.P, c[9], self.sf2, c[10], c[11],
                                             W.data_ptr() if W is not None else None, self.Np, self.Np,
                                             float(kss) if kss is not None else 0.0, float(floor),
                                             Xq.ctypes.data, M, mean.ctypes.data,
                                             var.ctypes.data if var is not None else None))
        return mean, var

    def inverse_factor(self, f32):
        torch = _torch()
        assert self.factored
        key = "f32" if f32 else "f64"
        if key not in self._Winv:
            be = self.be
            W = self._Winv.get("f64")
            if W is None:
                W = be.empty((self.Np, self.Np), torch.float64)
                work = be.empty(((self.Np // 2 + 128) ** 2,), torch.float64)
                absmax = be.empty((self.Np // 128,), torch.float32)
                with be.lock:
                    be.bind_stream()
                    be.check(be.lib.gpk_trtri_absmax(be.h, _p(self.K), self.Np, self.Np, _p(self.winv), _p(W), self.Np,
                                                     _p(work), _p(absmax)))
                self._Winv["absmax"] = absmax
                del work
            if f32:
                Wf = be.empty((self.Np, self.Np), torch.float32)
                with be.lock:
                    be.bind_stream()
                    be.check(be.lib.gpk_tril_to_f32(be.h, _p(W), self.Np, self.Np, _p(Wf), self.Np))
                self._Winv["f32"] = Wf
            else:
                self._Winv["f64"] = W
        return self._Winv[key]

    def split_inverse_factor(self):
        torch = _torch()
        if "split" not in self._Winv:
            had_f32 = "f32" in self._Winv
            Wf = self.inverse_factor(True)
            be = self.be
            W3 = be.empty((self.Np * self.Np * 6,), torch.uint8)
            with be.lock:
                be.bind_stream()
                be.check(be.lib.gpk_split3(be.h, _p(Wf), self.Np, self.Np, self.Np, _p(W3)))
            self._Winv["split"] = W3
            if not had_f32:
                self._Winv.pop("f32", None)
        return self._Winv["split"]

    def split2_inverse_factor(self):
        torch = _torch()
        if "split2" not in self._Winv:
            be = self.be
            scales = be.empty((self.Np // 128,), torch.float32)
            W2 = be.empty((self.Np * self.Np * 4,), torch.uint8)
            if "f32" in self._Winv:
                with be.lock:
                    be.bind_stream()
                    be.check(be.lib.gpk_split2_rows(be.h, _p(self._Winv["f32"]), self.Np, self.Np, _p(scales), _p(W2)))
            else:
                W = self.inverse_factor(False)
                absmax = self._Winv.pop("absmax", None)
                with be.lock:
                    be.bind_stream()
                    if absmax is not None:
                        scales = absmax
                        be.check(be.lib.gpk_split2_rows_f64_absmax(be.h, _p(W), self.Np, self.Np, _p(scales), _p(W2)))
                    else:
                        be.check(be.lib.gpk_split2_rows_f64(be.h, _p(W), self.Np, self.Np, _p(scales), _p(W2)))
            self._Winv["split2"] = (W2, scales)
        return self._Winv["split2"]

    SERVING_TENSORS = ("X", "alpha", "W2", "w_scales")

    def serving_state(self):
        assert self.factored and not self.replica
        W2, w_scales = self.split2_inverse_factor()
        meta = {"N": self.N, "D": self.D, "P": self.P, "Np": self.Np, "ls": np.asarray(self.ls, dtype=np.float64).tolist(),
                "sf2": float(self.sf2), "shapes": {"X": (self.N, self.D), "alpha": (self.N, self.P),
                                                   "W2": (self.Np * self.Np * 4,), "w_scales": (self.Np // 128,)},
                "dtypes": {"X": "float64", "alpha": "float64", "W2": "uint8", "w_scales": "float32"}}
        return meta, {"X": self.X, "alpha": self.alpha, "W2": W2, "w_scales": w_scales}

    @classmethod
    def from_serving_state(cls, meta, tensors, backend=None):
        torch = _torch()
        self = cls.__new__(cls)
        self.be = backend or get_backend()
        self.N, self.D, self.P, self.Np = int(meta["N"]), int(meta["D"]), int(meta["P"]), int(meta["Np"])
        self.X = tensors["X"]
        self._Xh = self.X.cpu().numpy()
        self._xc = self._Xh.mean(axis=0)
        self._r2 = {}
        self.Yn = None
        self.K = self.winv = None
        self.alpha = tensors["alpha"]
        self.factored = True
        self.ls = np.ascontiguousarray(meta["ls"], dtype=np.float64)
        self.sf2 = float(meta["sf2"])
        self._f32 = None
        self._Winv = {"split2": (tensors["W2"], tensors["w_scales"])}
        self._host_args = None
        self._amp = self._alpha_sq = None
        self._Kinv = None
        self.replica = True
        return self

    FP32_MEAN_ERR_PER_AMP = {"mfma": 7.0e-7, "valu": 1.1e-6}
    FP32_MEAN_TOL = 1e-4
    FP32_BATCH_GATE_ROWS = 1024
    FP32_BATCH_GATE_MARGIN = 1.3
    FP32_VAR_RECHECK_FRACTION = 1e-2

    def _amplification_at(self, q64):
        zeros, ones = np.zeros(self.P), np.ones(self.P)
        sq = getattr(self, "_alpha_sq", None)
        if sq is None:
            sq = self._alpha_sq = self.alpha ** 2
        b = self.predict_mean_dev(q64, zeros, ones, "float64", "valu").abs().amax(dim=0)
        a2 = self.predict_mean_dev(q64, zeros, ones, "float64", "valu", _alpha=sq,
                                   _kernel=(self.ls / np.sqrt(2.0), self.sf2 ** 2)).amax(dim=0).sqrt()
        return float((a2 / b.clamp_min(1e-300)).max())

    def fp32_mean_amplification(self):
        torch = _torch()
        c = getattr(self, "_amp", None)
        if c is not None and c[0] is self.ls:
            return c[1]
        idx = torch.linspace(0, self.N - 1, min(self.N, 1024), device=self.be.device).round().long()
        amp = self._amplification_at(self.X[idx].contiguous())
        self._amp = (self.ls, amp)
        return amp

    def fp32_mean_ok(self, q=None):
        torch = _torch()
        c = self.FP32_MEAN_ERR_PER_AMP[self.mean_kernel_choice()]
        if c * self.fp32_mean_amplification() <= self.FP32_MEAN_TOL:
            return True
        if q is None or len(q) == 0:
            return False
        M = len(q)
        if isinstance(q, torch.Tensor):
            idx = torch.linspace(0, M - 1, min(M, self.FP32_BATCH_GATE_ROWS), device=q.device).round().long()
            qs = q[idx].to(device=self.be.device, dtype=torch.float64).contiguous()
        else:
            idx = np.round(np.linspace(0, M - 1, min(M, self.FP32_BATCH_GATE_ROWS))).astype(np.int64)
            qs = self.be.upload(np.ascontiguousarray(np.asarray(q, dtype=np.float64)[idx]))
        return c * self.FP32_BATCH_GATE_MARGIN * self._amplification_at(qs) <= self.FP32_MEAN_TOL

    def predict_var_dev(self, Xq, kss, floor=0.0, dtype="float64", method="auto"):
        torch = _torch()
        assert self.factored
        f32 = dtype in ("float32", np.float32, torch.float32)
        if method == "auto":
            method = "inverse_split2" if f32 else "inverse"
        if method not in ("solve", "inverse", "inverse_split", "inverse_split2"):
            raise ValueError("method must be 'auto', 'solve', 'inverse', 'inverse_split' or 'inverse_split2'")
        if method in ("inverse_split", "inverse_split2") and not f32:
            raise ValueError("inverse_split / inverse_split2 are fp32 serving forms (bf16x3 / fp16x2 operand splits)")
        tdt = torch.float32 if f32 else torch.float64
        es = 4 if f32 else 8
        code = GPK_F32 if f32 else GPK_F64
        q = self._as_queries(Xq, tdt)
        M = q.shape[0]
        out = self.be.empty((M,), torch.float64)
        if M == 0:
            return out
        Xd = self._f32_data()["X"] if f32 else self.X
        if method == "inverse_split":
            W3 = self.split_inverse_factor()
        elif method == "inverse_split2":
            W2, w_scales = self.split2_inverse_factor()
        elif method == "inverse":
            Wd = self.inverse_factor(f32)
        elif f32:
            c = self._f32_factor()
            Ld, wd = c["L"], c["winv"]
        else:
            Ld, wd = self.K, self.winv
        panel = max(128, min(self.VAR_PANEL_MAX, (self.VAR_PANEL_BYTES // (self.Np * es)) // 128 * 128))
        panel = min(panel, padded(M))
        work = self.be.empty((self.Np * panel,), tdt) if method != "inverse_split2" else None
        work3 = (self.be.empty((self.Np * panel * (6 if method == "inverse_split" else 4),), torch.uint8)
                 if method in ("inverse_split", "inverse_split2") else None)
        var = self.be.empty((panel,), torch.float64)
        be = self.be
        lsp = self.ls.ctypes.data_as(_lib._dp)
        with be.lock:
            be.bind_stream()
            for m0 in range(0, M, panel):
                m1 = min(M, m0 + panel)
                if method == "inverse_split":
                    be.check(be.lib.gpk_predict_var_inv_split(be.h, _p(Xd), self.N, self.D, lsp, self.sf2, _p(W3),
                                                              self.Np, _p(q[m0:m1]), m1 - m0, float(kss), float(floor),
                                                              _p(work), _p(work3), _p(var)))
                elif method == "inverse_split2":
                    be.check(be.lib.gpk_predict_var_inv_split2(be.h, _p(Xd), self.N, self.D, lsp, self.sf2, _p(W2),
                                                               _p(w_scales), self.Np, _p(q[m0:m1]), m1 - m0, float(kss),
                                                               float(floor), _p(work3), _p(var)))
                elif method == "inverse":
                    be.check(be.lib.gpk_predict_var_inv(be.h, code, _p(Xd), self.N, self.D, lsp, self.sf2, _p(Wd),
                                                        self.Np, self.Np, _p(q[m0:m1]), m1 - m0, float(kss),
                                                        float(floor), _p(work), _p(var)))
                else:
                    be.check(be.lib.gpk_predict_var(be.h, code, _p(Xd), self.N, self.D, lsp, self.sf2, _p(Ld),
                                                    self.Np, self.Np, _p(wd), _p(q[m0:m1]), m1 - m0, float(kss),
                                                    float(floor), _p(work), _p(var)))
                out[m0:m1].copy_(var[: m1 - m0])
        return out

    def cov_panel_check(self, M):
        if M > self.VAR_PANEL_MAX:
            raise ValueError(f"return_cov: at most VAR_PANEL_MAX = {self.VAR_PANEL_MAX} queries per call (got {M})")
        need = self.Np * padded(M) * 8
        if need > self.VAR_PANEL_BYTES:
            raise ValueError(f"return_cov: V = L^-1 K*^T would take {need} bytes, more than VAR_PANEL_BYTES = "
                             f"{self.VAR_PANEL_BYTES} (N = {self.N}, M = {M}): pass fewer queries per call")

    def predict_cov_dev(self, Xq, noise, method="auto"):
        torch = _torch()
        assert self.factored
        if method == "auto":
            method = self._fp64_var_method()
        if method not in ("inverse", "solve"):
            raise ValueError("method must be 'auto', 'inverse' or 'solve'")
        if self.replica:
            raise RuntimeError("a serving replica holds no factor: covariances are computed on the rank that fitted the model")
        q = self._as_queries(Xq, torch.float64)
        M = q.shape[0]
        if M == 0:
            return self.be.empty((0, 0), torch.float64)
        self.cov_panel_check(M)
        Mp = padded(M)
        work = self.be.empty((self.Np * Mp,), torch.float64)
        cov = self.be.empty((Mp, Mp), torch.float64)
        be = self.be
        lsp = self.ls.ctypes.data_as(_lib._dp)
        if method == "inverse":
            W = self.inverse_factor(False)
            with be.lock:
                be.bind_stream()
                be.check(be.lib.gpk_predict_cov_inv(be.h, GPK_F64, _p(self.X), self.N, self.D, lsp, self.sf2, _p(W), self.Np,
                                                    self.Np, _p(q), M, float(noise), _p(work), _p(cov), Mp))
        else:
            with be.lock:
                be.bind_stream()
                be.check(be.lib.gpk_predict_cov(be.h, GPK_F64, _p(self.X), self.N, self.D, lsp, self.sf2, _p(self.K), self.Np,
                                                self.Np, _p(self.winv), _p(q), M, float(noise), _p(work), _p(cov), Mp))
        del work
        return cov[:M, :M]

    def predict_cov_host(self, Xq, y_mean, y_std, noise):
        assert self.factored
        Xq = np.ascontiguousarray(Xq, dtype=np.float64)
        if Xq.ndim != 2 or Xq.shape[1] != self.D:
            raise ValueError(f"queries must be (M, {self.D})")
        M = Xq.shape[0]
        mean = np.empty((M, self.P))
        cov = np.empty((M, M))
        W = self.inverse_factor(False)
        be = self.be
        c = self._host_call_args(y_mean, y_std)
        with be.lock:
            be.bind_stream()
            be.check(be.lib.gpk_predict_host_cov(be.h, c[7], c[8], self.N, self.D, self.P, c[9], self.sf2, c[10], c[11],
                                                 W.data_ptr(), self.Np, self.Np, float(noise), Xq.ctypes.data, M,
                                                 mean.ctypes.data, cov.ctypes.data))
        return mean, cov

    def predict_grad_dev(self, Xq, y_std, kss=None, floor=0.0):
        torch = _torch()
        if kss is not None and self.replica:
            raise RuntimeError("a serving replica holds no fp64 inverse factor: variance gradients are computed on the rank "
                               "that fitted the model (the mean Jacobian is served here: kss=None)")
        q = self._as_queries(Xq, torch.float64)
        dmean = self.predict_mean_grad_dev(q, y_std)
        if kss is None:
            return dmean, None, None
        var, dvar = self.predict_var_grad_dev(q, kss, floor)
        return dmean, var, dvar

    def predict_mean_grad_dev(self, Xq, y_std):
        torch = _torch()
        assert self.factored
        q = self._as_queries(Xq, torch.float64)
        M = q.shape[0]
        dmean = self.be.empty((M, self.P, self.D), torch.float64)
        if M == 0:
            return dmean
        ys = np.ascontiguousarray(np.broadcast_to(np.asarray(y_std, dtype=np.float64), (self.P,)))
        be = self.be
        with be.lock:
            be.bind_stream()
            be.check(be.lib.gpk_predict_mean_grad(be.h, _p(self.X), _p(self.alpha), self.N, self.D, self.P,
                                                  self.ls.ctypes.data_as(_lib._dp), self.sf2, ys.ctypes.data_as(_lib._dp),
                                                  _p(q), M, _p(dmean)))
        return dmean

    def predict_var_grad_dev(self, Xq, kss, floor=0.0):
        torch = _torch()
        assert self.factored
        if self.replica:
            raise RuntimeError("a serving replica holds no fp64 inverse factor: variance gradients are computed on the rank "
                               "that fitted the model (the mean Jacobian is served here: kss=None)")
        q = self._as_queries(Xq, torch.float64)
        M = q.shape[0]
        var = self.be.empty((M,), torch.float64)
        dvar = self.be.empty((M, self.D), torch.float64)
        if M == 0:
            return var, dvar
        W = self.inverse_factor(False)
        panel = max(128, min(self.VAR_PANEL_MAX, (self.VAR_PANEL_BYTES // (3 * self.Np * 8)) // 128 * 128))
        panel = min(panel, padded(M))
        work = self.be.empty((3 * self.Np * panel,), torch.float64)
        be = self.be
        lsp = self.ls.ctypes.data_as(_lib._dp)
        with be.lock:
            be.bind_stream()
            for m0 in range(0, M, panel):
                m1 = min(M, m0 + panel)
                be.check(be.lib.gpk_predict_var_grad_inv(be.h, _p(self.X), self.N, self.D, lsp, self.sf2, _p(W), self.Np,
                                                         self.Np, _p(q[m0:m1]), m1 - m0, float(kss), float(floor),
                                                         _p(work), _p(var[m0:m1]), _p(dvar[m0:m1])))
        del work
        return var, dvar

    def predict_grad_host(self, Xq, y_mean, y_std, kss=None, floor=0.0):
        assert self.factored
        Xq = np.ascontiguousarray(Xq, dtype=np.float64)
        if Xq.ndim != 2 or Xq.shape[1] != self.D:
            raise ValueError(f"queries must be (M, {self.D})")
        if kss is not None and self.replica:
            raise RuntimeError("a serving replica holds no fp64 inverse factor: variance gradients are computed on the rank "
                               "that fitted the model (the mean Jacobian is served here: kss=None)")
        M = Xq.shape[0]
        mean = np.empty((M, self.P))
        dmean = np.empty((M, self.P, self.D))
        var = np.empty((M,)) if kss is not None else None
        dvar = np.empty((M, self.D)) if kss is not None else None
        W = self.inverse_factor(False) if kss is not None else None
        be = self.be
        c = self._host_call_args(y_mean, y_std)
        with be.lock:
            be.bind_stream()
            be.check(be.lib.gpk_predict_host_grad(be.h, c[7], c[8], self.N, self.D, self.P, c[9], self.sf2, c[10], c[11],
                                                  W.data_ptr() if W is not None else None, self.Np, self.Np,
                                                  float(kss) if kss is not None else 0.0, float(floor), Xq.ctypes.data, M,
                                                  mean.ctypes.data, var.ctypes.data if var is not None else None,
                                                  dmean.ctypes.data, dvar.ctypes.data if dvar is not None else None))
        return mean, var, dmean, dvar

    def _rows64(self, Xq, q, rows):
        torch = _torch()
        if isinstance(Xq, torch.Tensor):
            return Xq[rows.to(Xq.device)].to(device=self.be.device, dtype=torch.float64).contiguous()
        return self.be.upload(np.ascontiguousarray(np.asarray(Xq, dtype=np.float64)[rows.cpu().numpy()]))

    def _fp64_var_method(self):
        if self.replica:
            raise RuntimeError("a serving replica holds no factor: fp64 variances are computed on the rank that fitted the model")
        return "inverse" if ("f64" in self._Winv or self.Np <= self.INVERSE_EAGER_NP) else "solve"

    def _gate_mean(self, dtype, var_method, gated, q=None, mean_gate=None):
        torch = _torch()
        f32 = dtype in ("float32", np.float32, torch.float32)
        if f32 and gated and not (self.fp32_mean_ok(q) if mean_gate is None else mean_gate):
            return "float64", ("auto" if var_method in ("inverse_split", "inverse_split2") else var_method)
        return ("float32" if f32 else "float64"), var_method

    def predict_gated_dev(self, Xq, y_mean, y_std, kss=None, floor=0.0, dtype="float64", var_method="auto", gated=True,
                          mean_gate=None):
        torch = _torch()
        pd, vm = self._gate_mean(dtype, var_method, gated, Xq, mean_gate)
        q = self._as_queries(Xq, torch.float32 if pd == "float32" else torch.float64)
        mean = self.predict_mean_dev(q, y_mean, y_std, pd)
        if kss is None:
            return mean, None
        var = self.predict_var_dev(q, kss, floor, pd, vm)
        if gated and pd == "float32" and q.shape[0]:
            low = torch.nonzero(var < self.FP32_VAR_RECHECK_FRACTION * kss).ravel()
            if low.numel():
                var[low] = self.predict_var_dev(self._rows64(Xq, q, low), kss, floor, "float64", self._fp64_var_method())
        return mean, var

    def predict_packed_dev(self, Xq, y_mean, y_std, kss, floor=0.0, dtype="float32", var_method="auto", gated=True,
                           mean_gate=None):
        torch = _torch()
        pd, vm = self._gate_mean(dtype, var_method, gated, Xq, mean_gate)
        f32 = pd == "float32"
        if vm == "auto":
            vm = "inverse_split2" if f32 else "inverse"
        q = self._as_queries(Xq, torch.float32 if f32 else torch.float64)
        M = q.shape[0]
        out = self.be.empty((M, 2 * self.P), torch.float64)
        if M == 0:
            return out
        ym = np.ascontiguousarray(np.broadcast_to(np.asarray(y_mean, dtype=np.float64), (self.P,)))
        ys = np.ascontiguousarray(np.broadcast_to(np.asarray(y_std, dtype=np.float64), (self.P,)))
        be = self.be
        if not (f32 and vm == "inverse_split2"):
            mean = self.predict_mean_dev(q, ym, ys, pd)
            var = self.predict_var_dev(q, kss, floor, pd, vm)
            if gated and f32:
                low = torch.nonzero(var < self.FP32_VAR_RECHECK_FRACTION * kss).ravel()
                if low.numel():
                    var[low] = self.predict_var_dev(self._rows64(Xq, q, low), kss, floor, "float64", self._fp64_var_method())
            with be.lock:
                be.bind_stream()
                be.check(be.lib.gpk_pack_mean_var(be.h, GPK_F32 if f32 else GPK_F64, _p(mean), _p(var), M, self.P,
                                                  ys.ctypes.data_as(_lib._dp), _p(out)))
            return out
        c = self._f32_data()
        W2, w_scales = self.split2_inverse_factor()
        center = self._xc.ctypes.data_as(_lib._dp) if self.mean_kernel_choice() == "mfma" else None
        panel = max(128, min(self.VAR_PANEL_MAX, (self.VAR_PANEL_BYTES // (self.Np * 4)) // 128 * 128))
        panel = min(panel, padded(M))
        work2 = be.empty((self.Np * panel * 4,), torch.uint8)
        mean_tmp = be.empty((panel * self.P,), torch.float32)
        thr = self.FP32_VAR_RECHECK_FRACTION * kss if gated else 0.0
        nlow = 0
        with be.lock:
            be.bind_stream()
            try:
                for m0 in range(0, M, panel):
                    m1 = min(M, m0 + panel)
                    be.check(be.lib.gpk_predict_mean_var_split2(
                        be.h, _p(c["X"]), _p(c["alpha"]), self.N, self.D, self.P, self.ls.ctypes.data_as(_lib._dp), self.sf2,
                        center, ym.ctypes.data_as(_lib._dp), ys.ctypes.data_as(_lib._dp), _p(W2), _p(w_scales), self.Np,
                        _p(q[m0:m1]), m1 - m0, float(kss), float(floor), _p(work2), _p(mean_tmp), float(thr),
                        _p(be.low_count) if gated else None, _p(out[m0:m1])))
            finally:
                if gated:
                    seen = int(be.low_count.item()) & 0xFFFFFFFF
                    nlow = (seen - be.low_seen) & 0xFFFFFFFF
                    be.low_seen = seen
        if nlow and not self.replica:
            ys2 = torch.as_tensor(ys ** 2, device=be.device)
            low = torch.nonzero(out[:, self.P] <= thr * float(ys[0] ** 2) * (1.0 + 1e-12)).ravel()
            v64 = self.predict_var_dev(self._rows64(Xq, q, low), kss, floor, "float64", self._fp64_var_method())
            out[low, self.P:] = v64[:, None] * ys2[None, :]
        return out

    def gram_host(self, ls, sf2, diag_add):
        self.gram(ls, sf2, diag_add)
        return self.K[: self.N, : self.N].cpu().numpy()


def prior_cov(X, ls, sf2, noise, device=None):
    torch = _torch()
    be = get_backend(device)
    X = np.ascontiguousarray(X, dtype=np.float64)
    M, D = X.shape
    if M == 0:
        return np.zeros((0, 0))
    if not 1 <= D <= _lib.GPK_MAX_D:
        raise ValueError(f"D must be in [1, {_lib.GPK_MAX_D}]")
    Mp = padded(M)
    ls = np.ascontiguousarray(np.broadcast_to(np.asarray(ls, dtype=np.float64), (D,)))
    q = be.upload(X)
    K = be.empty((Mp, Mp), torch.float64)
    with be.lock:
        be.bind_stream()
        be.check(be.lib.gpk_gram(be.h, GPK_F64, _p(q), M, D, ls.ctypes.data_as(_lib._dp), float(sf2), float(noise), _p(K), Mp))
    return K[:M, :M].cpu().numpy()
```

Before: 101,300 predictions/s.

## Fuse fp32 mean-accuracy gate into the packed predict call on device

Adds a device-side fp64 mean-amplification kernel that reduces across blocks with ticket counters, and a gated split2 predict entry point. The fp32-accuracy gate is now evaluated in the same call as the first panel instead of in a separate host-synchronising check. The low-variance count is published to mapped host memory by the finalize kernel, so the .item() readback is no longer needed. This cuts host round-trips and syncs per predict call, at the cost of more complex atomic-ticket logic and a fallback path if the gate fails.

```diff
diff --git a/include/gpk.h b/include/gpk.h
--- a/include/gpk.h
+++ b/include/gpk.h
@@ -99,6 +99,17 @@
                                         const double* y_std, const void* W2, const float* w_scales, int64_t Np,
                                         const float* Xq, int64_t M, double kss, double floor_, void* work2,
                                         float* mean_tmp, double recheck_below, unsigned* low_count, double* out);
+GPK_API int gpk_mean_amplification(gpk_handle h, const double* X, const double* alpha, int64_t N, int D, int P,
+                                   const double* ls, double sf2, int q_dtype, const void* Xq, int64_t M,
+                                   const int64_t* idx, int64_t R, double* a2);
+GPK_API int gpk_predict_mean_var_split2_gated(gpk_handle h, const float* X, const float* alpha, int64_t N, int D, int P,
+                                              const double* ls, double sf2, const double* center, const double* y_mean,
+                                              const double* y_std, const void* W2, const float* w_scales, int64_t Np,
+                                              const float* Xq, int64_t M, double kss, double floor_, void* work2,
+                                              float* mean_tmp, double recheck_below, double* out, const double* X64,
+                                              const double* alpha64, int gate_dtype, const void* gate_Xq, int64_t gate_M,
+                                              const int64_t* gate_idx, int64_t gate_R, double gate_factor, double gate_tol,
+                                              int* served, double* a2, unsigned* low_total);
 GPK_API int gpk_pack_mean_var(gpk_handle h, int dtype, const void* mean, const double* var, int64_t M, int P,
                               const double* y_std, double* out);
 
diff --git a/unmanned_aerial_vehicles_amd/_lib.py b/unmanned_aerial_vehicles_amd/_lib.py
--- a/unmanned_aerial_vehicles_amd/_lib.py
+++ b/unmanned_aerial_vehicles_amd/_lib.py
@@ -39,6 +39,10 @@
     "gpk_predict_var_inv_split2": (_int, [_vp, _vp, _i64, _int, _dp, _dbl, _vp, _vp, _i64, _vp, _i64, _dbl, _dbl, _vp, _vp]),
     "gpk_predict_mean_var_split2": (_int, [_vp, _vp, _vp, _i64, _int, _int, _dp, _dbl, _dp, _dp, _dp, _vp, _vp, _i64, _vp, _i64,
                                            _dbl, _dbl, _vp, _vp, _dbl, _vp, _vp]),
+    "gpk_mean_amplification": (_int, [_vp, _vp, _vp, _i64, _int, _int, _dp, _dbl, _int, _vp, _i64, _vp, _i64, _dp]),
+    "gpk_predict_mean_var_split2_gated": (_int, [_vp, _vp, _vp, _i64, _int, _int, _dp, _dbl, _dp, _dp, _dp, _vp, _vp, _i64, _vp,
+                                                 _i64, _dbl, _dbl, _vp, _vp, _dbl, _vp, _vp, _vp, _int, _vp, _i64, _vp, _i64,
+                                                 _dbl, _dbl, C.POINTER(_int), _dp, C.POINTER(C.c_uint)]),
     "gpk_pack_mean_var": (_int, [_vp, _int, _vp, _vp, _i64, _int, _dp, _vp]),
     "gpk_set_option": (_int, [_vp, C.c_char_p, _int]),
     "gpk_set_option_str": (_int, [_vp, C.c_char_p, C.c_char_p]),
diff --git a/unmanned_aerial_vehicles_amd/csrc/gpk_api.hip b/unmanned_aerial_vehicles_amd/csrc/gpk_api.hip
--- a/unmanned_aerial_vehicles_amd/csrc/gpk_api.hip
+++ b/unmanned_aerial_vehicles_amd/csrc/gpk_api.hip
@@ -17,14 +17,15 @@
   if (hipStreamCreateWithFlags(&h->own_stream, hipStreamNonBlocking) != hipSuccess ||
       hipMalloc((void**)&h->d_info, GPK_MAX_BATCH * sizeof(int)) != hipSuccess ||
 
-      hipMalloc((void**)&h->d_count, 2 * GPK_SMALL_MAX_MODELS * sizeof(unsigned)) != hipSuccess ||
-      hipMemset(h->d_count, 0, 2 * GPK_SMALL_MAX_MODELS * sizeof(unsigned)) != hipSuccess ||
+      hipMalloc((void**)&h->d_count, GPK_COUNT_WORDS * sizeof(unsigned)) != hipSuccess ||
+      hipMemset(h->d_count, 0, GPK_COUNT_WORDS * sizeof(unsigned)) != hipSuccess ||
       hipHostMalloc((void**)&h->h_small, 4096, hipHostMallocMapped | hipHostMallocCoherent) != hipSuccess ||
       hipHostGetDevicePointer((void**)&h->d_small, h->h_small, 0) != hipSuccess) {
     delete h;
     return GPK_HIP_ERROR;
   }
   h->stream = h->own_stream;
+  memset(h->h_small + GPK_SERVE_LOW_OFF, 0, sizeof(double));
   *out = h;
   return GPK_OK;
 }
@@ -46,6 +47,7 @@
     if (t.e0) (void)hipEventDestroy(t.e0);
     if (t.e1) (void)hipEventDestroy(t.e1);
   }
+  if (h->gate_event) (void)hipEventDestroy(h->gate_event);
   if (h->own_stream) (void)hipStreamDestroy(h->own_stream);
   delete h;
 }
diff --git a/unmanned_aerial_vehicles_amd/csrc/gpk_gram.hip b/unmanned_aerial_vehicles_amd/csrc/gpk_gram.hip
--- a/unmanned_aerial_vehicles_amd/csrc/gpk_gram.hip
+++ b/unmanned_aerial_vehicles_amd/csrc/gpk_gram.hip
@@ -563,6 +563,140 @@
   mean[e] = T(ymean.v[p]) + T(ystd.v[p]) * (sf2 * T(s));
 }
 
+__device__ __forceinline__ bool amp_last_of(unsigned* counter, unsigned count, int tid) {
+  __shared__ int is_last;
+  __syncthreads();
+  if (tid == 0) {
+    const unsigned t = __hip_atomic_fetch_add(counter, 1u, __ATOMIC_ACQ_REL, __HIP_MEMORY_SCOPE_AGENT);
+    is_last = (t == count - 1);
+    if (is_last) __hip_atomic_store(counter, 0u, __ATOMIC_RELAXED, __HIP_MEMORY_SCOPE_AGENT);
+  }
+  __syncthreads();
+  return is_last != 0;
+}
+
+template <int D4, int P4>
+__global__ __launch_bounds__(256) void mean_amp_kernel(const double* __restrict__ X, const double* __restrict__ alpha,
+                                                       long long N, int D, int P, Ls16 ls, double sf2,
+                                                       const void* __restrict__ Xq, int q_f32, long long M,
+                                                       const long long* __restrict__ idx, int R, long long chunk,
+                                                       double* __restrict__ partial, double* __restrict__ blockmax,
+                                                       unsigned* __restrict__ tickets, unsigned* __restrict__ top_ticket,
+                                                       double* __restrict__ a2_out) {
+  __shared__ __attribute__((aligned(16))) double rows[PM_TJ * PM_RS];
+  constexpr int DD = 4 * D4, PP = 4 * P4;
+  const int tid = threadIdx.x;
+  const int r = blockIdx.x * 256 + tid;
+  const long long Rp = (long long)gridDim.x * 256;
+  double xq[DD], a1[PP], a2[PP];
+  {
+    long long m = r < R ? (idx ? idx[r] : (long long)r) : 0;
+    m = min(max(m, 0ll), M - 1);
+#pragma unroll
+    for (int d = 0; d < DD; ++d) {
+      xq[d] = 0.0;
+      if (d < D && r < R)
+        xq[d] = (q_f32 ? (double)static_cast<const float*>(Xq)[m * D + d] : static_cast<const double*>(Xq)[m * D + d]) / ls.v[d];
+    }
+  }
+#pragma unroll
+  for (int p = 0; p < PP; ++p) { a1[p] = 0.0; a2[p] = 0.0; }
+  const long long n0 = (long long)blockIdx.y * chunk;
+  const long long n1 = min(N, n0 + chunk);
+  for (long long jb = n0; jb < n1; jb += PM_TJ) {
+    const int nj = (int)min((long long)PM_TJ, n1 - jb);
+    __syncthreads();
+    for (int e = tid; e < nj * (DD + PP); e += 256) {
+      const int j = e / (DD + PP), c = e - j * (DD + PP);
+      double v = 0.0;
+      if (c < DD) { if (c < D) v = X[(jb + j) * D + c] / ls.v[c]; }
+      else if (c - DD < P) v = alpha[(jb + j) * P + (c - DD)];
+      rows[j * PM_RS + (c < DD ? c : PM_DMAX + (c - DD))] = v;
+    }
+    __syncthreads();
+#pragma unroll 2
+    for (int j = 0; j < nj; ++j) {
+      const double4* row = reinterpret_cast<const double4*>(rows + j * PM_RS);
+      double xt[DD], al[PP];
+#pragma unroll
+      for (int g = 0; g < D4; ++g) {
+        const double4 v = row[g];
+        xt[4 * g] = v.x; xt[4 * g + 1] = v.y; xt[4 * g + 2] = v.z; xt[4 * g + 3] = v.w;
+      }
+#pragma unroll
+      for (int g = 0; g < P4; ++g) {
+        const double4 v = row[PM_DMAX / 4 + g];
+        al[4 * g] = v.x; al[4 * g + 1] = v.y; al[4 * g + 2] = v.z; al[4 * g + 3] = v.w;
+      }
+      double d2 = 0.0;
+#pragma unroll
+      for (int d = 0; d < DD; ++d) {
+        const double df = xq[d] - xt[d];
+        d2 = __builtin_fma(df, df, d2);
+      }
+      const double e = exp_neg(-0.5 * d2);
+#pragma unroll
+      for (int p = 0; p < PP; ++p) {
+        const double t = e * al[p];
+        a1[p] += t;
+        a2[p] = __builtin_fma(t, t, a2[p]);
+      }
+    }
+  }
+#pragma unroll
+  for (int p = 0; p < PP; ++p)
+    if (p < P) {
+      partial[(((long long)blockIdx.y * 2) * P + p) * Rp + r] = r < R ? a1[p] : 0.0;
+      partial[(((long long)blockIdx.y * 2 + 1) * P + p) * Rp + r] = r < R ? a2[p] : 0.0;
+    }
+  if (!amp_last_of(tickets + blockIdx.x, gridDim.y, tid)) return;
+  double* red = rows;
+  const int lane = tid & 63, wave = tid >> 6;
+  for (int w = 0; w < 2 * P; ++w) {
+    double s = 0.0;
+    for (unsigned k = 0; k < gridDim.y; ++k) s += partial[((long long)k * 2 * P + w) * Rp + r];
+    s = w < P ? fabs(sf2 * s) : sf2 * sf2 * s;
+    for (int off = 32; off > 0; off >>= 1) s = fmax(s, __shfl_xor(s, off, 64));
+    if (lane == 0) red[w * 4 + wave] = s;
+  }
+  __syncthreads();
+  if (tid < 2 * P) blockmax[(long long)blockIdx.x * 2 * P + tid] = fmax(fmax(red[tid * 4], red[tid * 4 + 1]), fmax(red[tid * 4 + 2], red[tid * 4 + 3]));
+  if (!amp_last_of(top_ticket, gridDim.x, tid)) return;
+  if (tid == 0) {
+    double best = 0.0;
+    for (int p = 0; p < P; ++p) {
+      double m1 = 0.0, m2 = 0.0;
+      for (unsigned b = 0; b < gridDim.x; ++b) {
+        m1 = fmax(m1, blockmax[(long long)b * 2 * P + p]);
+        m2 = fmax(m2, blockmax[(long long)b * 2 * P + P + p]);
+      }
+      const double a = sqrt(m2) / fmax(m1, 1e-300);
+      best = (a > best || a != a) ? a : best;
+    }
+    *a2_out = best;
+  }
+}
+
+using amp_fn = void (*)(const double*, const double*, long long, int, int, Ls16, double, const void*, int, long long,
+                        const long long*, int, long long, double*, double*, unsigned*, unsigned*, double*);
+template <int D4>
+amp_fn amp_pick_p(int p4) {
+  switch (p4) {
+    case 1: return mean_amp_kernel<D4, 1>;
+    case 2: return mean_amp_kernel<D4, 2>;
+    case 3: return mean_amp_kernel<D4, 3>;
+    default: return mean_amp_kernel<D4, 4>;
+  }
+}
+amp_fn amp_pick(int d4, int p4) {
+  switch (d4) {
+    case 1: return amp_pick_p<1>(p4);
+    case 2: return amp_pick_p<2>(p4);
+    case 3: return amp_pick_p<3>(p4);
+    default: return amp_pick_p<4>(p4);
+  }
+}
+
 template <typename T>
 __global__ __launch_bounds__(256) void colsumsq_kernel(const T* __restrict__ B, long long rows_per, long long Np,
                                                        long long ldb, double* __restrict__ partial, long long Mp) {
@@ -598,15 +732,19 @@
 __global__ void colsum_finalize_packed_kernel(const double* __restrict__ partial, int S, long long Mp, long long M, double kss,
                                               double floor_, const float* __restrict__ mean, int P, PArr ystd,
                                               double recheck_below, unsigned* __restrict__ low_count,
-                                              double* __restrict__ out) {
+                                              double* __restrict__ out, unsigned* __restrict__ ticket,
+                                              unsigned* __restrict__ published) {
   const long long m = (long long)blockIdx.x * blockDim.x + threadIdx.x;
-  if (m >= M) return;
-  double s = 0.0;
-  for (int k = 0; k < S; ++k) s += partial[(long long)k * Mp + m];
-  const double v = fmax(kss - s, floor_);
-  if (low_count && v < recheck_below) atomicAdd(low_count, 1u);
-  double* o = out + m * 2 * P;
-  for (int p = 0; p < P; ++p) { o[p] = (double)mean[m * P + p]; o[P + p] = v * ystd.v[p] * ystd.v[p]; }
+  if (m < M) {
+    double s = 0.0;
+    for (int k = 0; k < S; ++k) s += partial[(long long)k * Mp + m];
+    const double v = fmax(kss - s, floor_);
+    if (low_count && v < recheck_below) atomicAdd(low_count, 1u);
+    double* o = out + m * 2 * P;
+    for (int p = 0; p < P; ++p) { o[p] = (double)mean[m * P + p]; o[P + p] = v * ystd.v[p] * ystd.v[p]; }
+  }
+  if (ticket && amp_last_of(ticket, gridDim.x, threadIdx.x) && threadIdx.x == 0)
+    *published = __hip_atomic_load(low_count, __ATOMIC_RELAXED, __HIP_MEMORY_SCOPE_AGENT);
 }
 template <typename T>
 __global__ void pack_mean_var_kernel(const T* __restrict__ mean, const double* __restrict__ var, long long M, int P, PArr ystd,
@@ -880,6 +1018,49 @@
   return GPK_OK;
 }
 
+int gpk_mean_amp_enqueue(gpk_handle h, const double* X, const double* alpha, int64_t N, int D, int P, const double* ls,
+                         double sf2, int q_dtype, const void* Xq, int64_t M, const int64_t* idx, int64_t R, double* d_out) {
+  GPK_REQUIRE(h, X && alpha && Xq && ls && d_out, "mean_amplification: null pointer");
+  GPK_REQUIRE(h, N >= 1 && M >= 1 && R >= 1 && R <= GPK_GATE_MAX_ROWS, "mean_amplification: 1 <= R <= 1024 rows");
+  GPK_REQUIRE(h, idx || R <= M, "mean_amplification: more rows than the batch holds");
+  GPK_REQUIRE(h, D >= 1 && D <= PM_DMAX && P >= 1 && P <= PM_PMAX, "mean_amplification: D and P must be in [1, 16]");
+  GPK_REQUIRE(h, q_dtype == GPK_F32 || q_dtype == GPK_F64, "mean_amplification: bad dtype");
+  GPK_REQUIRE(h, h->batch == 1, "mean_amplification: not available in batched mode");
+  LsArr l;
+  GPK_TRY(fill_ls(h, ls, D, l));
+  Ls16 l16;
+  for (int d = 0; d < 16; ++d) l16.v[d] = l.v[d];
+  const int64_t nqb = (R + 255) / 256;
+  int64_t S = (512 + nqb - 1) / nqb;
+  if (S > 256) S = 256;
+  const int64_t maxS = (N + PM_TJ - 1) / PM_TJ;
+  if (S > maxS) S = maxS;
+  int64_t chunk = (N + S - 1) / S;
+  chunk = (chunk + PM_TJ - 1) / PM_TJ * PM_TJ;
+  S = (N + chunk - 1) / chunk;
+  const size_t nshare = (size_t)S * 2 * P * nqb * 256;
+  void* ws = nullptr;
+  GPK_TRY(gpk_scratch(h, (nshare + (size_t)nqb * 2 * P) * sizeof(double), &ws));
+  double* partial = (double*)ws;
+  hipLaunchKernelGGL(amp_pick((D + 3) / 4, (P + 3) / 4), dim3((unsigned)nqb, (unsigned)S), dim3(256), 0, h->stream, X, alpha,
+                     (long long)N, D, P, l16, sf2, Xq, q_dtype == GPK_F32 ? 1 : 0, (long long)M, (const long long*)idx, (int)R,
+                     (long long)chunk, partial, partial + nshare, h->d_count + GPK_SERVE_GATE_TICKETS,
+                     h->d_count + GPK_SERVE_GATE_TOP, d_out);
+  GPK_LAUNCH_CHECK(h);
+  return GPK_OK;
+}
+
+extern "C" int gpk_mean_amplification(gpk_handle h, const double* X, const double* alpha, int64_t N, int D, int P,
+                                      const double* ls, double sf2, int q_dtype, const void* Xq, int64_t M,
+                                      const int64_t* idx, int64_t R, double* a2) {
+  if (!h) return GPK_BAD_ARG;
+  GPK_REQUIRE(h, a2, "mean_amplification: null pointer");
+  GPK_TRY(gpk_mean_amp_enqueue(h, X, alpha, N, D, P, ls, sf2, q_dtype, Xq, M, idx, R, h->d_small + GPK_SERVE_A2_OFF));
+  GPK_CHECK_HIP(h, hipStreamSynchronize(h->stream));
+  *a2 = h->h_small[GPK_SERVE_A2_OFF];
+  return GPK_OK;
+}
+
 extern "C" int gpk_colsumsq(gpk_handle h, int dtype, const void* B, int64_t Np, int64_t Mp, int64_t ldb,
                             double* out) {
   if (!h) return GPK_BAD_ARG;
@@ -918,11 +1099,13 @@
 }
 int gpk_colsum_finalize_packed(gpk_handle h, const double* partial, int S, int64_t Mp, int64_t M, double kss, double floor_,
                                const float* mean, int P, const double* y_std, double recheck_below, unsigned* low_count,
-                               double* out) {
+                               double* out, int publish) {
   PArr ys{};
   for (int p = 0; p < P; ++p) ys.v[p] = y_std[p];
+  unsigned* ticket = publish ? h->d_count + GPK_SERVE_FIN_TICKET : nullptr;
+  unsigned* published = publish ? reinterpret_cast<unsigned*>(h->d_small + GPK_SERVE_LOW_OFF) : nullptr;
   hipLaunchKernelGGL(colsum_finalize_packed_kernel, dim3((unsigned)((M + 255) / 256)), dim3(256), 0, h->stream, partial, S,
-                     (long long)Mp, (long long)M, kss, floor_, mean, P, ys, recheck_below, low_count, out);
+                     (long long)Mp, (long long)M, kss, floor_, mean, P, ys, recheck_below, low_count, out, ticket, published);
   GPK_LAUNCH_CHECK(h);
   return GPK_OK;
 }
diff --git a/unmanned_aerial_vehicles_amd/csrc/gpk_internal.h b/unmanned_aerial_vehicles_amd/csrc/gpk_internal.h
--- a/unmanned_aerial_vehicles_amd/csrc/gpk_internal.h
+++ b/unmanned_aerial_vehicles_amd/csrc/gpk_internal.h
@@ -28,6 +28,7 @@
   double* h_small = nullptr;
   double* d_small = nullptr;
   unsigned* d_count = nullptr;
+  hipEvent_t gate_event = nullptr;
   unsigned* d_cov_count = nullptr;
   void* serve_dev = nullptr;
   size_t serve_dev_bytes = 0;
@@ -114,6 +115,10 @@
 int gpk_potrf_enqueue(gpk_handle h, double* A, int64_t Np, int64_t lda, double* winv);
 int gpk_potrf_finish(gpk_handle h, const int* hinfo_all, int* info, int gave_up = -1);
 constexpr int GPK_STATUS_OFF = 480;
+constexpr int GPK_SERVE_A2_OFF = 448, GPK_SERVE_LOW_OFF = 449;
+constexpr int GPK_COUNT_WORDS = 2 * 8 + 8;
+constexpr int GPK_SERVE_GATE_TICKETS = 16, GPK_SERVE_GATE_TOP = 20, GPK_SERVE_FIN_TICKET = 21, GPK_SERVE_LOW_COUNT = 22;
+constexpr int GPK_GATE_MAX_ROWS = 1024;
 int gpk_tril_block_absmax_f64_enqueue(gpk_handle h, const double* W, int64_t n, int64_t ld, unsigned* out);
 int gpk_potrf_trtri_enqueue(gpk_handle h, double* A, int64_t Np, int64_t lda, double* winv, double* W, int64_t ldw, double* wt,
                             int* used);
@@ -237,4 +242,6 @@
                         double* var);
 int gpk_colsum_finalize_packed(gpk_handle h, const double* partial, int S, int64_t Mp, int64_t M, double kss, double floor_,
                                const float* mean, int P, const double* y_std, double recheck_below, unsigned* low_count,
-                               double* out);
+                               double* out, int publish = 0);
+int gpk_mean_amp_enqueue(gpk_handle h, const double* X, const double* alpha, int64_t N, int D, int P, const double* ls,
+                         double sf2, int q_dtype, const void* Xq, int64_t M, const int64_t* idx, int64_t R, double* d_out);
diff --git a/unmanned_aerial_vehicles_amd/csrc/gpk_k5split.hip b/unmanned_aerial_vehicles_amd/csrc/gpk_k5split.hip
--- a/unmanned_aerial_vehicles_amd/csrc/gpk_k5split.hip
+++ b/unmanned_aerial_vehicles_amd/csrc/gpk_k5split.hip
@@ -476,8 +476,8 @@
 }
 
 namespace {
-int split2_launch(gpk_handle h, const char* who, const float* X, int64_t N, int D, const double* ls, double sf2, const void* W2,
-                  const float* w_scales, int64_t Np, const float* Xq, int64_t M, void* work2, void** partial, int* S) {
+int split2_kstar(gpk_handle h, const char* who, const float* X, int64_t N, int D, const double* ls, double sf2, const void* W2,
+                 const float* w_scales, int64_t Np, const float* Xq, int64_t M, void* work2, double* k_scale_out) {
   GPK_REQUIRE(h, X && W2 && w_scales && Xq && work2, (std::string(who) + ": null pointer").c_str());
   GPK_REQUIRE(h, N >= 1 && M >= 1 && Np == gpk_padded(N), (std::string(who) + ": Np must equal gpk_padded(N)").c_str());
   GPK_REQUIRE(h, h->batch == 1, (std::string(who) + ": not available in batched mode").c_str());
@@ -488,6 +488,13 @@
               (std::string(who) + ": size too large").c_str());
   const double k_scale = std::ldexp(1.0, 14 - (int)std::floor(std::log2(sf2)));
   GPK_TRY(gpk_cross_split2(h, Xq, M, X, N, D, ls, sf2, k_scale, work2));
+  *k_scale_out = k_scale;
+  return GPK_OK;
+}
+int split2_variance(gpk_handle h, const void* W2, const float* w_scales, int64_t Np, int64_t M, const void* work2, double k_scale,
+                    void** partial, int* S) {
+  const int64_t Mp = gpk_padded(M);
+  const int ntm = (int)(Np / 128), ntn = (int)(Mp / 128);
   int ab = 1;
   if (Np % 512 == 0 && (h->k5_split2_tile == 2 || (Np / 512) * (long long)ntn >= 512)) ab = 4;
   else if (Np % 256 == 0 && (Np / 256) * (long long)ntn >= 512) ab = 2;
@@ -516,6 +523,12 @@
   *S = ntmT;
   return GPK_OK;
 }
+int split2_launch(gpk_handle h, const char* who, const float* X, int64_t N, int D, const double* ls, double sf2, const void* W2,
+                  const float* w_scales, int64_t Np, const float* Xq, int64_t M, void* work2, void** partial, int* S) {
+  double k_scale = 0.0;
+  GPK_TRY(split2_kstar(h, who, X, N, D, ls, sf2, W2, w_scales, Np, Xq, M, work2, &k_scale));
+  return split2_variance(h, W2, w_scales, Np, M, work2, k_scale, partial, S);
+}
 }
 
 extern "C" int gpk_predict_var_inv_split2(gpk_handle h, const float* X, int64_t N, int D, const double* ls, double sf2,
@@ -543,6 +556,49 @@
   GPK_TRY(split2_launch(h, "predict_mean_var_split2", X, N, D, ls, sf2, W2, w_scales, Np, Xq, M, work2, &partial, &S));
   return gpk_colsum_finalize_packed(h, (const double*)partial, S, gpk_padded(M), M, kss, floor_, mean_tmp, P, y_std,
                                     recheck_below, low_count, out);
+}
+
+extern "C" int gpk_predict_mean_var_split2_gated(gpk_handle h, const float* X, const float* alpha, int64_t N, int D, int P,
+                                                 const double* ls, double sf2, const double* center, const double* y_mean,
+                                                 const double* y_std, const void* W2, const float* w_scales, int64_t Np,
+                                                 const float* Xq, int64_t M, double kss, double floor_, void* work2,
+                                                 float* mean_tmp, double recheck_below, double* out, const double* X64,
+                                                 const double* alpha64, int gate_dtype, const void* gate_Xq, int64_t gate_M,
+                                                 const int64_t* gate_idx, int64_t gate_R, double gate_factor, double gate_tol,
+                                                 int* served, double* a2, unsigned* low_total) {
+  if (!h) return GPK_BAD_ARG;
+  GPK_REQUIRE(h, alpha && y_mean && y_std && mean_tmp && out && served && P >= 1 && P <= GPK_MAX_P,
+              "predict_mean_var_split2_gated: bad argument");
+  *served = 0;
+  const bool gate = X64 != nullptr;
+  if (gate) {
+    GPK_REQUIRE(h, alpha64 && gate_Xq && a2, "predict_mean_var_split2_gated: the gate needs the fp64 model, the batch and a2");
+    if (!h->gate_event) GPK_CHECK_HIP(h, hipEventCreateWithFlags(&h->gate_event, hipEventDisableTiming));
+    GPK_TRY(gpk_mean_amp_enqueue(h, X64, alpha64, N, D, P, ls, sf2, gate_dtype, gate_Xq, gate_M, gate_idx, gate_R,
+                                 h->d_small + GPK_SERVE_A2_OFF));
+    GPK_CHECK_HIP(h, hipEventRecord(h->gate_event, h->stream));
+  }
+  if (center) GPK_TRY(gpk_predict_mean_mfma(h, X, alpha, N, D, P, ls, sf2, center, y_mean, y_std, Xq, M, mean_tmp));
+  else GPK_TRY(gpk_predict_mean(h, GPK_F32, X, alpha, N, D, P, ls, sf2, y_mean, y_std, Xq, M, mean_tmp));
+  double k_scale = 0.0;
+  GPK_TRY(split2_kstar(h, "predict_mean_var_split2_gated", X, N, D, ls, sf2, W2, w_scales, Np, Xq, M, work2, &k_scale));
+  if (gate) {
+    GPK_CHECK_HIP(h, hipEventSynchronize(h->gate_event));
+    *a2 = h->h_small[GPK_SERVE_A2_OFF];
+    if (!(gate_factor * *a2 <= gate_tol)) return GPK_OK;
+  }
+  void* partial = nullptr;
+  int S = 0;
+  GPK_TRY(split2_variance(h, W2, w_scales, Np, M, work2, k_scale, &partial, &S));
+  GPK_TRY(gpk_colsum_finalize_packed(h, (const double*)partial, S, gpk_padded(M), M, kss, floor_, mean_tmp, P, y_std,
+                                     recheck_below, low_total ? h->d_count + GPK_SERVE_LOW_COUNT : nullptr, out,
+                                     low_total ? 1 : 0));
+  *served = 1;
+  if (low_total) {
+    GPK_CHECK_HIP(h, hipStreamSynchronize(h->stream));
+    *low_total = *reinterpret_cast<const volatile unsigned*>(h->h_small + GPK_SERVE_LOW_OFF);
+  }
+  return GPK_OK;
 }
 
 extern "C" int gpk_predict_var_inv_split(gpk_handle h, const float* X, int64_t N, int D, const double* ls, double sf2,
diff --git a/unmanned_aerial_vehicles_amd/device.py b/unmanned_aerial_vehicles_amd/device.py
--- a/unmanned_aerial_vehicles_amd/device.py
+++ b/unmanned_aerial_vehicles_amd/device.py
@@ -37,7 +37,6 @@
         if os.environ.get("GPK_DEBUG_FILL"):
             self.check(self.lib.gpk_set_option(self.h, b"debug_fill", 1))
         self.bind_stream()
-        self.low_count = torch.zeros((1,), dtype=torch.int32, device=self.device)
         self.low_seen = 0
 
     def bind_stream(self):
@@ -106,6 +105,21 @@
 
 def padded(n):
     return (int(n) + 127) // 128 * 128
+
+
+_gate_rows = {}
+
+
+def gate_rows(M, device, rows=1024):
+    torch = _torch()
+    key = (int(M), int(rows), str(torch.device(device)))
+    with _backends_lock:
+        idx = _gate_rows.get(key)
+        if idx is None:
+            if len(_gate_rows) >= 64:
+                _gate_rows.clear()
+            idx = _gate_rows[key] = torch.linspace(0, int(M) - 1, min(int(M), int(rows)), device=device).round().long()
+        return idx
 
 
 def _p(t):
@@ -148,7 +162,7 @@
         self._f32 = None
         self._Winv = {}
         self._host_args = None
-        self._amp = self._alpha_sq = None
+        self._amp = None
         self._Kinv = None
         self.replica = False
 
@@ -212,13 +226,13 @@
                 be.bind_stream()
                 be.check(be.lib.gpk_potrs(be.h, _p(self.K), self.Np, self.Np, _p(self.winv), _p(self.Yn), self.N,
                                           self.P, _p(self.alpha)))
-        self._amp = self._alpha_sq = None
+        self._amp = None
         if self._f32:
             self._f32.pop("alpha", None)
 
     def set_alpha(self, alpha):
         self.alpha.copy_(self.be.upload(np.asarray(alpha, dtype=np.float64).reshape(self.N, self.P)))
-        self._amp = self._alpha_sq = None
+        self._amp = None
         if self._f32:
             self._f32.pop("alpha", None)
 
@@ -281,7 +295,7 @@
                 g.ctypes.data_as(_lib._dp) if eval_gradient else None, C.byref(info)))
         self.factored = True
         self._Winv["f64"] = W
-        self._amp = self._alpha_sq = None
+        self._amp = None
         return terms[0], terms[1:], g
 
     def release_grad_buffers(self):
@@ -351,7 +365,7 @@
             self._r2 = {key: 0.5 * np.log2(np.e) * float(np.max(np.einsum("ij,ij->i", u, u)))}
         return "mfma" if (self.P <= 8 and self._r2[key] <= self.MFMA_MEAN_R2_MAX) else "valu"
 
-    def predict_mean_dev(self, Xq, y_mean, y_std, dtype="float64", kernel="auto", _alpha=None, _kernel=None):
+    def predict_mean_dev(self, Xq, y_mean, y_std, dtype="float64", kernel="auto", _alpha=None):
         torch = _torch()
         f32 = dtype in ("float32", np.float32, torch.float32)
         if kernel == "auto":
@@ -372,7 +386,6 @@
         ym = np.ascontiguousarray(np.broadcast_to(np.asarray(y_mean, dtype=np.float64), (self.P,)))
         ys = np.ascontiguousarray(np.broadcast_to(np.asarray(y_std, dtype=np.float64), (self.P,)))
         be = self.be
-        ls_, sf2_ = (self.ls, self.sf2) if _kernel is None else (np.ascontiguousarray(_kernel[0]), float(_kernel[1]))
         if kernel == "mfma":
             with be.lock:
                 be.bind_stream()
@@ -384,7 +397,7 @@
         with be.lock:
             be.bind_stream()
             be.check(be.lib.gpk_predict_mean(be.h, GPK_F32 if f32 else GPK_F64, _p(Xd), _p(ad), self.N, self.D,
-                                             self.P, ls_.ctypes.data_as(_lib._dp), sf2_,
+                                             self.P, self.ls.ctypes.data_as(_lib._dp), self.sf2,
                                              ym.ctypes.data_as(_lib._dp), ys.ctypes.data_as(_lib._dp), _p(q), M,
                                              _p(out)))
         return out
@@ -521,7 +534,7 @@
         self._f32 = None
         self._Winv = {"split2": (tensors["W2"], tensors["w_scales"])}
         self._host_args = None
-        self._amp = self._alpha_sq = None
+        self._amp = None
         self._Kinv = None
         self.replica = True
         return self
@@ -532,41 +545,49 @@
     FP32_BATCH_GATE_MARGIN = 1.3
     FP32_VAR_RECHECK_FRACTION = 1e-2
 
-    def _amplification_at(self, q64):
-        zeros, ones = np.zeros(self.P), np.ones(self.P)
-        sq = getattr(self, "_alpha_sq", None)
-        if sq is None:
-            sq = self._alpha_sq = self.alpha ** 2
-        b = self.predict_mean_dev(q64, zeros, ones, "float64", "valu").abs().amax(dim=0)
-        a2 = self.predict_mean_dev(q64, zeros, ones, "float64", "valu", _alpha=sq,
-                                   _kernel=(self.ls / np.sqrt(2.0), self.sf2 ** 2)).amax(dim=0).sqrt()
-        return float((a2 / b.clamp_min(1e-300)).max())
+    def _amplification_at(self, q, idx=None):
+        torch = _torch()
+        M = q.shape[0]
+        R = M if idx is None else int(idx.numel())
+        a2 = C.c_double()
+        be = self.be
+        with be.lock:
+            be.bind_stream()
+            be.check(be.lib.gpk_mean_amplification(be.h, _p(self.X), _p(self.alpha), self.N, self.D, self.P,
+                                                   self.ls.ctypes.data_as(_lib._dp), self.sf2,
+                                                   GPK_F32 if q.dtype == torch.float32 else GPK_F64, _p(q), M,
+                                                   _p(idx) if idx is not None else None, R, C.byref(a2)))
+        return a2.value
+
+    def _gate_source(self, Xq):
+        torch = _torch()
+        M, rows = len(Xq), self.FP32_BATCH_GATE_ROWS
+        if isinstance(Xq, torch.Tensor):
+            if (Xq.device == self.be.device and Xq.dtype in (torch.float32, torch.float64) and Xq.ndim == 2
+                    and Xq.is_contiguous()):
+                return Xq, (gate_rows(M, Xq.device, rows) if M > rows else None)
+            return Xq[gate_rows(M, Xq.device, rows)].to(device=self.be.device, dtype=torch.float64).contiguous(), None
+        idx = np.round(np.linspace(0, M - 1, min(M, rows))).astype(np.int64)
+        return self.be.upload(np.ascontiguousarray(np.asarray(Xq, dtype=np.float64)[idx])), None
 
     def fp32_mean_amplification(self):
-        torch = _torch()
         c = getattr(self, "_amp", None)
         if c is not None and c[0] is self.ls:
             return c[1]
-        idx = torch.linspace(0, self.N - 1, min(self.N, 1024), device=self.be.device).round().long()
-        amp = self._amplification_at(self.X[idx].contiguous())
+        amp = self._amplification_at(self.X, gate_rows(self.N, self.be.device) if self.N > 1024 else None)
         self._amp = (self.ls, amp)
         return amp
 
+    def _fp32_model_ok(self):
+        return self.FP32_MEAN_ERR_PER_AMP[self.mean_kernel_choice()] * self.fp32_mean_amplification() <= self.FP32_MEAN_TOL
+
     def fp32_mean_ok(self, q=None):
-        torch = _torch()
-        c = self.FP32_MEAN_ERR_PER_AMP[self.mean_kernel_choice()]
-        if c * self.fp32_mean_amplification() <= self.FP32_MEAN_TOL:
+        if self._fp32_model_ok():
             return True
         if q is None or len(q) == 0:
             return False
-        M = len(q)
-        if isinstance(q, torch.Tensor):
-            idx = torch.linspace(0, M - 1, min(M, self.FP32_BATCH_GATE_ROWS), device=q.device).round().long()
-            qs = q[idx].to(device=self.be.device, dtype=torch.float64).contiguous()
-        else:
-            idx = np.round(np.linspace(0, M - 1, min(M, self.FP32_BATCH_GATE_ROWS))).astype(np.int64)
-            qs = self.be.upload(np.ascontiguousarray(np.asarray(q, dtype=np.float64)[idx]))
-        return c * self.FP32_BATCH_GATE_MARGIN * self._amplification_at(qs) <= self.FP32_MEAN_TOL
+        c = self.FP32_MEAN_ERR_PER_AMP[self.mean_kernel_choice()]
+        return c * self.FP32_BATCH_GATE_MARGIN * self._amplification_at(*self._gate_source(q)) <= self.FP32_MEAN_TOL
 
     def predict_var_dev(self, Xq, kss, floor=0.0, dtype="float64", method="auto"):
         torch = _torch()
@@ -806,7 +827,9 @@
     def predict_packed_dev(self, Xq, y_mean, y_std, kss, floor=0.0, dtype="float32", var_method="auto", gated=True,
                            mean_gate=None):
         torch = _torch()
-        pd, vm = self._gate_mean(dtype, var_method, gated, Xq, mean_gate)
+        in_call = (gated and mean_gate is None and var_method in ("auto", "inverse_split2") and len(Xq) > 0
+                   and dtype in ("float32", np.float32, torch.float32) and not self._fp32_model_ok())
+        pd, vm = ("float32", var_method) if in_call else self._gate_mean(dtype, var_method, gated, Xq, mean_gate)
         f32 = pd == "float32"
         if vm == "auto":
             vm = "inverse_split2" if f32 else "inverse"
@@ -819,17 +842,7 @@
         ys = np.ascontiguousarray(np.broadcast_to(np.asarray(y_std, dtype=np.float64), (self.P,)))
         be = self.be
         if not (f32 and vm == "inverse_split2"):
-            mean = self.predict_mean_dev(q, ym, ys, pd)
-            var = self.predict_var_dev(q, kss, floor, pd, vm)
-            if gated and f32:
-                low = torch.nonzero(var < self.FP32_VAR_RECHECK_FRACTION * kss).ravel()
-                if low.numel():
-                    var[low] = self.predict_var_dev(self._rows64(Xq, q, low), kss, floor, "float64", self._fp64_var_method())
-            with be.lock:
-                be.bind_stream()
-                be.check(be.lib.gpk_pack_mean_var(be.h, GPK_F32 if f32 else GPK_F64, _p(mean), _p(var), M, self.P,
-                                                  ys.ctypes.data_as(_lib._dp), _p(out)))
-            return out
+            return self._packed_separate(Xq, q, ym, ys, kss, floor, pd, vm, gated, out)
         c = self._f32_data()
         W2, w_scales = self.split2_inverse_factor()
         center = self._xc.ctypes.data_as(_lib._dp) if self.mean_kernel_choice() == "mfma" else None
@@ -838,27 +851,54 @@
         work2 = be.empty((self.Np * panel * 4,), torch.uint8)
         mean_tmp = be.empty((panel * self.P,), torch.float32)
         thr = self.FP32_VAR_RECHECK_FRACTION * kss if gated else 0.0
+        no_gate = (None, None, 0, None, 0, None, 0, 0.0, 0.0)
+        gate = no_gate
+        if in_call:
+            src, idx = self._gate_source(Xq)
+            gate = (_p(self.X), _p(self.alpha), GPK_F32 if src.dtype == torch.float32 else GPK_F64, _p(src), src.shape[0],
+                    _p(idx) if idx is not None else None, src.shape[0] if idx is None else int(idx.numel()),
+                    self.FP32_MEAN_ERR_PER_AMP[self.mean_kernel_choice()] * self.FP32_BATCH_GATE_MARGIN, self.FP32_MEAN_TOL)
+        served, a2, low = C.c_int(0), C.c_double(0.0), C.c_uint(0)
         nlow = 0
         with be.lock:
             be.bind_stream()
-            try:
-                for m0 in range(0, M, panel):
-                    m1 = min(M, m0 + panel)
-                    be.check(be.lib.gpk_predict_mean_var_split2(
-                        be.h, _p(c["X"]), _p(c["alpha"]), self.N, self.D, self.P, self.ls.ctypes.data_as(_lib._dp), self.sf2,
-                        center, ym.ctypes.data_as(_lib._dp), ys.ctypes.data_as(_lib._dp), _p(W2), _p(w_scales), self.Np,
-                        _p(q[m0:m1]), m1 - m0, float(kss), float(floor), _p(work2), _p(mean_tmp), float(thr),
-                        _p(be.low_count) if gated else None, _p(out[m0:m1])))
-            finally:
+            for m0 in range(0, M, panel):
+                m1 = min(M, m0 + panel)
+                be.check(be.lib.gpk_predict_mean_var_split2_gated(
+                    be.h, _p(c["X"]), _p(c["alpha"]), self.N, self.D, self.P, self.ls.ctypes.data_as(_lib._dp), self.sf2,
+                    center, ym.ctypes.data_as(_lib._dp), ys.ctypes.data_as(_lib._dp), _p(W2), _p(w_scales), self.Np,
+                    _p(q[m0:m1]), m1 - m0, float(kss), float(floor), _p(work2), _p(mean_tmp), float(thr), _p(out[m0:m1]),
+                    *(gate if m0 == 0 else no_gate), C.byref(served), C.byref(a2), C.byref(low) if gated else None))
+                if not served.value:
+                    break
                 if gated:
-                    seen = int(be.low_count.item()) & 0xFFFFFFFF
-                    nlow = (seen - be.low_seen) & 0xFFFFFFFF
-                    be.low_seen = seen
+                    nlow += (low.value - be.low_seen) & 0xFFFFFFFF
+                    be.low_seen = low.value
+        if not served.value:
+            return self._packed_separate(Xq, self._as_queries(Xq, torch.float64), ym, ys, kss, floor, "float64", "inverse",
+                                         gated, out)
         if nlow and not self.replica:
             ys2 = torch.as_tensor(ys ** 2, device=be.device)
             low = torch.nonzero(out[:, self.P] <= thr * float(ys[0] ** 2) * (1.0 + 1e-12)).ravel()
             v64 = self.predict_var_dev(self._rows64(Xq, q, low), kss, floor, "float64", self._fp64_var_method())
             out[low, self.P:] = v64[:, None] * ys2[None, :]
+        return out
+
+    def _packed_separate(self, Xq, q, ym, ys, kss, floor, pd, vm, gated, out):
+        torch = _torch()
+        f32 = pd == "float32"
+        M = q.shape[0]
+        be = self.be
+        mean = self.predict_mean_dev(q, ym, ys, pd)
+        var = self.predict_var_dev(q, kss, floor, pd, vm)
+        if gated and f32:
+            low = torch.nonzero(var < self.FP32_VAR_RECHECK_FRACTION * kss).ravel()
+            if low.numel():
+                var[low] = self.predict_var_dev(self._rows64(Xq, q, low), kss, floor, "float64", self._fp64_var_method())
+        with be.lock:
+            be.bind_stream()
+            be.check(be.lib.gpk_pack_mean_var(be.h, GPK_F32 if f32 else GPK_F64, _p(mean), _p(var), M, self.P,
+                                              ys.ctypes.data_as(_lib._dp), _p(out)))
         return out
 
     def gram_host(self, ls, sf2, diag_add):
```

Result: no change. 101,400 predictions/s, median of 2 (+0.1%).
